# microsoft/maro

Hardware: AMD Instinct MI355X
Metric: env-steps/sec (decision events/sec), CIM global_trade.22p (higher is better)
Workload: dtype int32+f64

## Files before the change

maro_amd/cim/engine.py:

```python
from __future__ import annotations

import contextlib
import ctypes
import os
from typing import Optional, Sequence, Union

import numpy as np
import torch

from .. import _lib
from .topology import CimTopology, load_topology

PORT_ATTRS = ["capacity", "empty", "full", "on_shipper", "on_consignee", "shortage", "acc_shortage", "booking",
              "acc_booking", "fulfillment", "acc_fulfillment", "transfer_cost"]
VESSEL_ATTRS = ["capacity", "empty", "full", "remaining_space", "early_discharge", "is_parking", "loc_port_idx",
                "route_idx", "last_loc_idx", "next_loc_idx", "past_stop_list", "past_stop_tick_list",
                "future_stop_list", "future_stop_tick_list"]
MATRIX_ATTRS = ["full_on_ports", "full_on_vessels", "vessel_plans"]
NODE_ATTRS = {"ports": PORT_ATTRS, "vessels": VESSEL_ATTRS, "matrices": MATRIX_ATTRS}
NODE_TYPE = {"ports": 0, "vessels": 1, "matrices": 2}

SEED_KEEP = -1
SEED_REDRAW = -2


class CimBatchEngine:

    def __init__(self, topology: Union[str, CimTopology], n_envs: int, start_tick: int = 0, durations: int = 100,
                 snapshot_resolution: int = 1, max_snapshots: Optional[int] = None, max_actions: int = 1,
                 device: Union[str, torch.device] = "cuda:0", seeds: Optional[Sequence[int]] = None, order_table: int = 0,
                 decision_mode: int = 0, specialize: Union[bool, str, None] = None, step_mode: int = 0):
        if specialize is None:
            specialize = {"1": True, "cached": "cached"}.get(os.environ.get("MARO_AMD_SPECIALIZE", "0"), False)
        self._L = _lib.load()
        if not torch.cuda.is_available():
            raise RuntimeError("maro_amd needs a ROCm GPU (torch.cuda.is_available() is False); there is no CPU path")
        self.topo = topology if isinstance(topology, CimTopology) else load_topology(topology)
        self.device = torch.device(device)
        dev_index = self.device.index if self.device.index is not None else torch.cuda.current_device()
        self.n_envs, self.max_actions = int(n_envs), int(max_actions)
        self.start_tick, self.durations = int(start_tick), int(durations)
        self.max_tick = self.start_tick + self.durations
        self.snapshot_resolution = int(snapshot_resolution)
        self._cs = self.topo.c_struct()
        self._cfg = _lib.MrxCimConfig(self.n_envs, dev_index, self.start_tick, self.durations,
                                      self.snapshot_resolution, int(max_snapshots or 0), self.max_actions, 0, int(decision_mode),
                                      int(order_table))
        self.decision_mode = int(decision_mode)
        nbytes = self._L.mrx_cim_workspace_bytes(ctypes.byref(self._cs), ctypes.byref(self._cfg))
        _lib.check(nbytes, "mrx_cim_workspace_bytes")
        self.workspace = torch.empty(nbytes, dtype=torch.uint8, device=self.device)
        h = ctypes.c_void_p()
        with torch.cuda.device(self.device):
            torch.cuda.synchronize()
            _lib.check(self._L.mrx_cim_create(ctypes.byref(self._cs), ctypes.byref(self._cfg),
                                              self.workspace.data_ptr(), nbytes, ctypes.byref(h)), "mrx_cim_create")
        self._h = h
        self._bound_stream, self._bound_handle = None, None
        self.specialized = False
        self._specialize, self._obs_ids = specialize, ((), ())
        self._step_mode = int(step_mode)
        self._load_specialized()
        self.layout = _lib.MrxCimLayout()
        _lib.check(self._L.mrx_cim_get_layout(self._h, ctypes.byref(self.layout)), "mrx_cim_get_layout")
        lay = self.layout
        self.live = self._view(lay.off_live, torch.int32, (self.n_envs, lay.frame_words))
        self.ring = self._view(lay.off_ring, torch.int32, (self.n_envs, lay.ring_slots, lay.frame_words))
        self.ring_fi = self._view(lay.off_ring_fi, torch.int32, (self.n_envs, lay.ring_slots))
        self.status = self._view(lay.off_status, torch.int32, (self.n_envs,))
        self.ticks = self._view(lay.off_tick, torch.int32, (self.n_envs,))
        self.seeds = self._view(lay.off_seed, torch.int64, (self.n_envs,))
        dshape = (self.n_envs, 8) if self.decision_mode == 0 else (self.n_envs, lay.n_vessels, 8)
        self.decisions = torch.zeros(dshape, dtype=torch.int32, device=self.device)
        self.metrics = torch.zeros((self.n_envs, 3), dtype=torch.int64, device=self.device)
        self.done = torch.zeros((self.n_envs,), dtype=torch.uint8, device=self.device)
        if seeds is not None:
            self.reset(seeds)

    def __del__(self):
        h = getattr(self, "_h", None)
        if h:
            self._L.mrx_cim_destroy(h)
            self._h = None

    def _view(self, off: int, dtype: torch.dtype, shape) -> torch.Tensor:
        n = int(np.prod(shape)) * torch.empty((), dtype=dtype).element_size()
        return self.workspace[off:off + n].view(dtype).view(*shape)

    def _load_specialized(self) -> None:
        self.specialized = False
        if self._specialize:
            from . import specialize as spec
            try:
                spec.load_into(self, spec.plan_defines(self._cs, self._cfg, obs=self._obs_ids), build=self._specialize != "cached")
                self.specialized = True
            except KeyError:
                pass
        self.set_step_mode(self._step_mode)

    def set_step_mode(self, mode: int) -> int:
        self._step_mode = int(mode)
        self.step_mode = _lib.check(self._L.mrx_cim_set_step_mode(self._h, self._step_mode), "mrx_cim_set_step_mode")
        return self.step_mode

    def use_stream(self, stream: Optional[torch.cuda.Stream]) -> None:
        self._bound_stream = stream
        self._bound_handle = None if stream is None else stream.cuda_stream

    def _stream(self) -> int:
        h = self._bound_handle
        return torch.cuda.current_stream(self.device).cuda_stream if h is None else h

    def _dev(self, x, dtype) -> Optional[torch.Tensor]:
        if x is None:
            return None
        if isinstance(x, torch.Tensor) and x.dtype == dtype and x.device == self.device and x.is_contiguous():
            return x
        if not isinstance(x, torch.Tensor):
            x = torch.as_tensor(np.asarray(x), dtype=dtype)
        if self._bound_stream is None:
            return x.to(device=self.device, dtype=dtype).contiguous()
        if x.is_cuda:
            self._bound_stream.wait_stream(torch.cuda.current_stream(self.device))
        with torch.cuda.stream(self._bound_stream):
            return x.to(device=self.device, dtype=dtype).contiguous()

    @staticmethod
    def _p(t: Optional[torch.Tensor]):
        return None if t is None else t.data_ptr()

    def reset(self, seed_cmd=None, mask=None) -> None:
        sc = self._dev(seed_cmd, torch.int64)
        mk = self._dev(mask, torch.uint8)
        _lib.check(self._L.mrx_cim_reset(self._h, self._p(sc), self._p(mk), self._stream()), "mrx_cim_reset")
        self._keep = (sc, mk)

    def step(self, actions=None, n_actions=None, mask=None, n_answered=None):
        a = self._dev(actions, torch.int32)
        na = self._dev(n_actions, torch.int32)
        mk = self._dev(mask, torch.uint8)
        if a is not None:
            assert a.numel() == self.n_envs * self.max_actions * 4, "actions must be [n_envs, max_actions, 4]"
            if na is None:
                na = torch.full((self.n_envs,), self.max_actions, dtype=torch.int32, device=self.device)
        if self.decision_mode == 0:
            _lib.check(self._L.mrx_cim_step(self._h, self._p(a), self._p(na), self._p(mk), self.decisions.data_ptr(),
                                            self.metrics.data_ptr(), self.done.data_ptr(), self._stream()), "mrx_cim_step")
            self._keep = (a, na, mk)
        else:
            nans = self._dev(n_answered, torch.int32)
            _lib.check(self._L.mrx_cim_step_joint(self._h, self._p(a), self._p(na), self._p(nans), self._p(mk), self.decisions.data_ptr(),
                                                  self.metrics.data_ptr(), self.done.data_ptr(), self._stream()), "mrx_cim_step_joint")
            self._keep = (a, na, mk, nans)
        return self.decisions, self.metrics, self.done

    def clear_status_bits(self, envs, bits: int) -> None:
        st = self._bound_stream
        with (torch.cuda.stream(st) if st is not None else contextlib.nullcontext()):
            idx = torch.as_tensor(list(envs), dtype=torch.int64, device=self.status.device)
            self.status[idx] = self.status[idx] & ~int(bits)

    def random_policy(self, step: int, actions: torch.Tensor, n_actions: torch.Tensor,
                      counter: Optional[torch.Tensor] = None) -> None:
        _lib.check(self._L.mrx_cim_random_policy(self._h, self.decisions.data_ptr(), int(step), actions.data_ptr(),
                                                 n_actions.data_ptr(), self._p(counter), self._stream()),
                   "mrx_cim_random_policy")
# ... 75 lines not shown
```

maro_amd/csrc/cim_device.h:

```cpp
#pragma once
#include <math.h>
#include <stdint.h>

#include "cim_params.h"

#ifdef MRX_SPECIALIZED
#define KD(f) (MRXC_##f)
#define OD(f) (MRXC_obs_##f)
#define ODA(f, i) (MRXC_obs_##f(i))
#else
#define KD(f) (K.f)
#define OD(f) (O.f)
#define ODA(f, i) (O.f[i])
#endif

namespace cim {

#ifndef MRX_PROFILE_PHASES
struct Prof {
  MRX_DEV void mark(int) {}
  MRX_DEV void mark(int, long long) {}
  MRX_DEV void flush() {}
};
#endif
// ... 15 lines not shown
  uint32_t* mt_ord;
  uint32_t* mt_buf;
  double* dsrc;
  double* dtgt;
  int32_t* oq;
  int32_t* srcn;
  int32_t* misc;
};

MRX_DEV Lds make_lds(const CimParams& K, int32_t* b) {
  Lds L;
  L.frame = b + KD(l_frame);
  L.priv = b + KD(l_priv);
  L.rfull = b + KD(l_rfull);
  L.mt_ord = (uint32_t*)(b + KD(l_mt0));
  L.mt_buf = (uint32_t*)(b + KD(l_mt1));
  L.dsrc = (double*)(b + KD(l_dsrc));
  L.dtgt = (double*)(b + KD(l_dtgt));
  L.oq = b + KD(l_oq);
  L.srcn = b + KD(l_srcn);
  L.misc = b + KD(l_misc);
  L.tab.tgt_off = K.h_tgt_off; L.tab.route_port = K.h_route_port;
  L.tab.v_route_base = K.h_v_route_base; L.tab.v_route_len = K.h_v_route_len;
  L.tab.leg_off = K.h_leg_off; L.tab.leg_time = K.h_leg_time;
  L.tab.er_delay = K.er_delay; L.tab.fr_delay = K.fr_delay; L.tab.rec_off = K.h_rec_off;
  L.tab.v_cbase = K.h_v_cbase; L.tab.route_cidx = K.h_route_cidx; L.tab.pair_src = K.h_pair_src;
  L.tab.src_base = K.src_base; L.tab.src_noise = K.src_noise; L.tab.er_base = K.er_base; L.tab.er_noise = K.er_noise;
  L.tab.fr_base = K.fr_base; L.tab.fr_noise = K.fr_noise;
  return L;
}

#if defined(MRX_SPECIALIZED)
#if MRXC_lean_ok
#define MRX_LEAN 1
#endif
#endif
#if defined(MRX_LEAN) && !defined(MRX_NO_LEAN2)
#define MRX_LEAN2 1
#endif
#ifdef MRX_LEAN
enum { RR_NB = (MRXC_NT + 63) / 64, RR_H = MRXC_H };
struct RingRegs { int rf[RR_H][RR_NB]; };
#else
struct RingRegs {};
#endif

#ifdef MRX_LEAN2
struct LeanStat {
  int ps[RR_NB];
  int vs0, vs1, vs2;
  int pt;
};
struct VRows {
  int evt, next;
  int w;
};
MRX_DEV int vr_k(const VRows& W) { return W.w & 0xffff; }
MRX_DEV int vr_pos(const VRows& W) { return (W.w >> 16) & 63; }
MRX_DEV int vr_krl(const VRows& W) { return (W.w >> 22) & 63; }
MRX_DEV int vr_park(const VRows& W) { return (W.w >> 28) & 1; }
MRX_DEV void vr_set(VRows& W, int k_, int pos_, int krl_, int park_) { W.w = k_ | (pos_ << 16) | (krl_ << 22) | (park_ << 28); }
struct Lean { LeanStat s; VRows w; };
#else
struct Lean {};
#endif

#define FP(a, p) L.frame[KD(f_ports) + (a) * KD(P) + (p)]
#define FV(a, v) L.frame[KD(f_vessels) + (a) * KD(V) + (v)]
#define FOPK(k) L.frame[KD(f_fop) + (k)]
#define FOVC(v, c) L.frame[KD(f_fov) + T.v_cbase[v] + (c)]
#define PLANC(v, c) L.frame[KD(f_plans) + T.v_cbase[v] + (c)]
#define V_EVT(v) L.priv[KD(pv_evt) + (v)]
#define V_NEXT(v) L.priv[KD(pv_next) + (v)]
#define V_POS(v) L.priv[KD(pv_pos) + (v)]
#define V_KRL(v) L.priv[KD(pv_krl) + (v)]
#define V_PERIOD(v) L.priv[KD(pv_period) + (v)]
#define U(x) wave::uniform(x)
#define MRX_UNALIGNED_FRAMES (KD(resolution) > 1 && KD(start_tick) % KD(resolution) != 0)
#define RING_FULL(slot, k) L.rfull[(slot) * KD(NT) + (k)]
#define RING_EMPTY(slot, p) L.priv[KD(pv_rempty) + (slot) * KD(P) + (p)]

MRX_DEV float bits_f(int32_t x) { union { int32_t i; float f; } u; u.i = x; return u.f; }
MRX_DEV int32_t f_bits(float f) { union { int32_t i; float f; } u; u.f = f; return u.i; }

MRX_DEV void copy_in_async(int32_t* lds_dst, const int32_t* gsrc, int n_words);
MRX_DEV void stage_tables(const CimParams& K, Lds& L, int32_t* c) {
  copy_in_async(c, K.ctab, KD(ctab_words));
#define MRX_HTAB(f) L.tab.f = (const uint16_t*)c + (K.h_##f - (const uint16_t*)K.ctab)
  MRX_HTAB(tgt_off); MRX_HTAB(route_port); MRX_HTAB(v_route_base); MRX_HTAB(v_route_len);
  MRX_HTAB(leg_off); MRX_HTAB(leg_time); MRX_HTAB(rec_off); MRX_HTAB(v_cbase); MRX_HTAB(route_cidx); MRX_HTAB(pair_src);
#undef MRX_HTAB
  L.tab.er_delay = c + (K.er_delay - K.ctab); L.tab.fr_delay = c + (K.fr_delay - K.ctab);
#define MRX_DTAB(f) L.tab.f = (const double*)(c + ((const int32_t*)K.f - K.ctab))
  if (!KD(pregen)) { MRX_DTAB(src_base); MRX_DTAB(src_noise); }
  MRX_DTAB(er_base); MRX_DTAB(er_noise); MRX_DTAB(fr_base); MRX_DTAB(fr_noise);
#undef MRX_DTAB
}

MRX_DEV uint32_t mt_temper(uint32_t y) {
  y ^= (y >> 11);
  y ^= (y << 7) & 0x9d2c5680U;
  y ^= (y << 15) & 0xefc60000U;
  y ^= (y >> 18);
  return y;
}

MRX_DEV void mt_twist(uint32_t* mt) {
  const int l = wave::lane();
  static_assert(MT_WORDS == 3 * 208, "round size");
  for (int k0 = 0; k0 < MT_WORDS; k0 += 208) {
    uint32_t x[4];
#pragma unroll
    for (int j = 0; j < 4; j++) {
      const bool on = j * 64 + l < 208;
      const int k = on ? k0 + j * 64 + l : k0;
      const int k1 = (k + 1 == MT_WORDS) ? 0 : k + 1;
      const int km = (k + 397 >= MT_WORDS) ? k + 397 - MT_WORDS : k + 397;
      const uint32_t y = (mt[k] & 0x80000000U) | (mt[k1] & 0x7fffffffU);
      x[j] = mt[km] ^ (y >> 1) ^ ((y & 1U) ? 0x9908b0dfU : 0U);
    }
    wave::sync();
#pragma unroll
    for (int j = 0; j < 4; j++)
      if (j * 64 + l < 208) mt[k0 + j * 64 + l] = x[j];
    wave::sync();
  }
}

MRX_DEV double mt_draw_batch(uint32_t* mt, int& idx, int rank, int n, bool& twisted) {
  uint32_t a = 0, b = 0;
  const bool has = rank >= 0;
  const int w0 = idx + 2 * rank, w1 = w0 + 1;
  if (has && w0 < MT_WORDS) a = mt_temper(mt[w0]);
  if (has && w1 < MT_WORDS) b = mt_temper(mt[w1]);
  if (idx + 2 * n > MT_WORDS) {
    wave::sync();
    mt_twist(mt);
    twisted = true;
    if (has && w0 >= MT_WORDS) a = mt_temper(mt[w0 - MT_WORDS]);
    if (has && w1 >= MT_WORDS) b = mt_temper(mt[w1 - MT_WORDS]);
    idx = idx + 2 * n - MT_WORDS;
  } else {
    idx += 2 * n;
  }
  return ((double)(a >> 5) * 67108864.0 + (double)(b >> 6)) * (1.0 / 9007199254740992.0);
}

template <int NB>
MRX_DEV void mt_draw_multi(uint32_t* mt, int& idx, const int (&rank)[NB], int n, bool& twisted, double (&r)[NB]) {
  uint32_t a[NB], b[NB];
#pragma unroll
  for (int i = 0; i < NB; i++) {
    const int w0 = idx + 2 * rank[i], w1 = w0 + 1;
    const uint32_t ra = mt[(rank[i] >= 0 && w0 < MT_WORDS) ? w0 : 0], rb = mt[(rank[i] >= 0 && w1 < MT_WORDS) ? w1 : 0];
    a[i] = (rank[i] >= 0 && w0 < MT_WORDS) ? mt_temper(ra) : 0u;
    b[i] = (rank[i] >= 0 && w1 < MT_WORDS) ? mt_temper(rb) : 0u;
  }
  if (idx + 2 * n > MT_WORDS) {
    wave::sync();
    mt_twist(mt);
    twisted = true;
#pragma unroll
    for (int i = 0; i < NB; i++) {
      const int w0 = idx + 2 * rank[i], w1 = w0 + 1;
      const uint32_t ra = mt[(rank[i] >= 0 && w0 >= MT_WORDS) ? w0 - MT_WORDS : 0], rb = mt[(rank[i] >= 0 && w1 >= MT_WORDS) ? w1 - MT_WORDS : 0];
      if (rank[i] >= 0 && w0 >= MT_WORDS) a[i] = mt_temper(ra);
// ... 279 lines not shown
      long long cur = 0;                                                                          \
      if (n_p > 0) {                                                                              \
        const double ts = L.dsrc[sp], x = L.dtgt[k];                                              \
        cur = (long long)ceil((double)n_p * ((ts == 0.0) ? x : x / ts));                          \
        if (cur > 0x7fffffffll) cur = 0x7fffffffll;                                               \
        if (cur < -0x7fffffffll) cur = -0x7fffffffll;                                             \
      }                                                                                           \
      L.oq[k] = (int32_t)cur;                                                                     \
    }                                                                                             \
  }
  if (NTb > 0) MRX_PAIR_BATCH(0, pf.src[0])
  if (NTb > 64) MRX_PAIR_BATCH(64, pf.src[1])
  if (NTb > 128) MRX_PAIR_BATCH(128, pf.src[2])
  for (int k0 = 192; k0 < NTb; k0 += 64) MRX_PAIR_BATCH(k0, K.pair_src[k0 + lane < NT ? k0 + lane : 0])
#undef MRX_PAIR_BATCH
  wave::sync();
  uint64_t negq = 0;
  for (int k0 = 0; k0 < NTb; k0 += 64) negq |= wave::ballot(k0 + lane < NTb && L.oq[k0 + lane] < 0);
  if (!negq) {
    uint32_t* pre = (uint32_t*)L.dtgt;
    uint32_t carry = 0;
#define MRX_HAND_SCAN(k0, SRC)                                                 \
    {                                                                          \
      const int k = (k0) + lane;                                               \
      int v = 0;                                                               \
      if (k < NTb) {                                                           \
        const int n_p = L.srcn[(SRC)];                                         \
        const int q = L.oq[k];                                                 \
        v = q < n_p ? q : (n_p > 0 ? n_p : 0);  \
      }                                                                        \
      const uint32_t incl = (uint32_t)wave::scan_incl_add(v) + carry;          \
      carry = (uint32_t)wave::bcast((int)incl, 63);                            \
      if (k < NTb) pre[k] = incl;                                              \
    }
    if (NTb > 0) MRX_HAND_SCAN(0, pf.src[0])
    if (NTb > 64) MRX_HAND_SCAN(64, pf.src[1])
    if (NTb > 128) MRX_HAND_SCAN(128, pf.src[2])
    for (int k0 = 192; k0 < NTb; k0 += 64) MRX_HAND_SCAN(k0, K.pair_src[k0 + lane < NT ? k0 + lane : 0])
#undef MRX_HAND_SCAN
    wave::sync();
#define MRX_HAND_OUT(k0, SRC)                                                                   \
    {                                                                                           \
      const int k = (k0) + lane;                                                                \
      if (k < NTb) {                                                                            \
        const int sp = (SRC);                                                                   \
        const int n_p = L.srcn[sp], q = L.oq[k], off = T.tgt_off[sp];                           \
        const int v = q < n_p ? q : (n_p > 0 ? n_p : 0);                                        \
        const int before = (int)(pre[k] - (uint32_t)v - (off > 0 ? pre[off - 1] : 0u));         \
        const int rem = n_p - before;                                                           \
        const int cur = rem <= 0 ? 0 : (q < rem ? q : rem);                                     \
        L.oq[k] = cur > 0 ? cur : 0;                                                            \
      }                                                                                         \
    }
    if (NTb > 0) MRX_HAND_OUT(0, pf.src[0])
    if (NTb > 64) MRX_HAND_OUT(64, pf.src[1])
    if (NTb > 128) MRX_HAND_OUT(128, pf.src[2])
    for (int k0 = 192; k0 < NTb; k0 += 64) MRX_HAND_OUT(k0, K.pair_src[k0 + lane < NT ? k0 + lane : 0])
#undef MRX_HAND_OUT
  } else if (lane < brk) {
    const long long n_p = L.srcn[lane];
    if (n_p > 0) {
      const int off = T.tgt_off[lane], cnt = T.tgt_off[lane + 1] - off;
      long long rem = n_p;
      for (int j = 0; j < cnt; j++) {
        long long cur = L.oq[off + j];
        if (cur > rem) cur = rem;
        rem -= cur;
        L.oq[off + j] = cur > 0 ? (int32_t)cur : 0;
      }
    }
  }
}

MRX_DEV void reset_env(const CimParams& K, int env, int32_t* lds, long long cmd) {
  Lds L = make_lds(K, lds);
  uint32_t* mt_route = (uint32_t*)(lds + KD(l_mt2));
  uint32_t* mt_oinit = (uint32_t*)(lds + KD(l_mt3));
  L.mt_ord = (uint32_t*)(lds + KD(r_mt0));
  L.mt_buf = (uint32_t*)(lds + KD(r_mt1));
  const int lane = wave::lane();
  const int P = KD(P), V = KD(V), TT = KD(T);
  uint32_t* g_mt = K.mt + (size_t)env * MTS_COUNT * MT_WORDS;
  int32_t* g_priv = K.priv + (size_t)env * KD(PW);
  int32_t* g_live = K.live + (size_t)env * KD(FW);
  const Tabs& T = L.tab;

  long long base;
  if (KD(data_mode)) {
    base = K.data_seed;
  } else if (cmd >= 0) {
    base = cmd;
  } else if (cmd == -1) {
    base = K.seed[env];
  } else {
    int idx = g_priv[PH_IDX_ROUTE];
    copy_words((int32_t*)mt_route, (const int32_t*)(g_mt + MTS_ROUTE * MT_WORDS), MT_WORDS);
    wave::sync();
    uint32_t r = mt_next_u32(mt_route, idx) >> (32 - 13);
    while (r >= 4096u) r = mt_next_u32(mt_route, idx) >> (32 - 13);
    base = (long long)r;
    wave::sync();
  }

  {
    uint32_t* arr = lane == 0 ? L.mt_ord : lane == 1 ? L.mt_buf : lane == 2 ? mt_route : mt_oinit;
    const int sidx = lane == 0 ? KD(idx_order_num) : lane == 1 ? KD(idx_buffer) : lane == 2 ? KD(idx_route) : KD(idx_order_init);
    if (lane < 3 || (lane == 3 && KD(has_order_init))) mt_seed_serial(arr, base + sidx);
  }
  wave::sync();
  int idx_route = MT_WORDS, idx_oi = MT_WORDS;

  int32_t* g_prop = K.order_prop + (size_t)env * TT;
  int status = 0;
  uint32_t* g_stops = K.stops + (size_t)env * V * KD(SMAX);
  if (KD(data_mode)) {
    for (int t = lane; t < TT; t += 64) g_prop[t] = (KD(data_mode) == 1 && t < KD(data_T)) ? K.fx_order_prop[t] : 0;
    for (int i = lane; i < V * KD(SMAX); i += 64) g_stops[i] = K.fx_stops[i];
    if (lane < V) { K.nstops[(size_t)env * V + lane] = K.fx_nstops[lane]; K.vperiod[(size_t)env * V + lane] = K.fx_vperiod[lane]; }
    __atomic_thread_fence(__ATOMIC_SEQ_CST);
    wave::sync();
  } else {
  for (int t0 = 0; t0 < TT; t0 += 64) {
    const int t = t0 + lane;
    double orders = t < TT ? K.order_dist[t % KD(period)] : 0.0;
    const bool nz = t < TT && orders != 0.0;
    if (KD(has_order_init)) {
      const uint64_t m = wave::ballot(nz);
      const int rank = nz ? __builtin_popcountll(m & ((1ull << lane) - 1ull)) : -1;
      bool tw = false;
      const double r = mt_draw_batch(mt_oinit, idx_oi, rank, __builtin_popcountll(m), tw);
      if (nz) orders = apply_noise(orders, K.sample_noise, r);
    }
    if (t < TT) {
      int32_t val = 0;
      if (nz) {
        double c = orders < 1.0 ? orders : 1.0;
        if (c < 0.0) c = 0.0;
        val = (int32_t)floor(c * (double)KD(total_containers));
      }
      g_prop[t] = val;
    }
  }

  for (int v = 0; v < V; v++) {
    const int Lr = K.v_route_len[v], rb = K.v_route_base[v], start = K.v_start[v];
    const double speed = K.v_speed[v], sn = K.v_speed_noise[v], dur = K.v_dur[v], dn = K.v_dur_noise[v];
    union { double d; int w[2]; } my_dist;
    my_dist.d = lane < Lr ? K.route_dist[rb + lane] : 0.0;
    const int my_leg = lane < Lr ? K.leg_time[K.leg_off[v] + lane] : 0;
    int tick = 0, extra = 0, k = 0;
    bool have_park = false, done = false;
    int park_carry = 0;
    while (!done) {
      const int left = (MT_WORDS - idx_route) / 2;
      const int nd = (idx_route >= MT_WORDS - 1 || left > 126) ? 126 : left;
      const int c = have_park ? 1 : 0;
      const int pi = 2 * lane - c, si = pi + 1;
      const int rank[2] = {(pi >= 0 && pi < nd) ? pi : -1, si < nd ? si : -1};
      double r[2];
      bool tw = false;
      mt_draw_multi<2>(mt_route, idx_route, rank, nd, tw, r);
      const int n_full = (nd + c) / 2;
      const bool half = ((nd + c) & 1) != 0;
      int parking = (int)ceil(apply_noise(dur, dn, r[0]));
      if (c && lane == 0) parking = park_carry;
      const double noised_speed = apply_noise(speed, sn, r[1]);
      int loc = start + k + lane;
// ... 12 lines not shown
      if (k + n_run >= 4 * KD(SMAX) + 1) {
        n_run = 4 * KD(SMAX) + 1 - k;
        run = run && lane < n_run;
        status |= 2;
        done = true;
      }
      if (wave::ballot(run && (parking <= 0 || parking > 255))) status |= 8;
      if (wave::ballot(run && k + lane >= KD(SMAX))) status |= 2;
      if (run && k + lane < KD(SMAX)) g_stops[(size_t)v * KD(SMAX) + k + lane] = ((uint32_t)t_before << 8) | (uint32_t)(parking & 0xff);
      if (extra + __builtin_popcountll(over & ((1ull << n_run) - 1ull)) > KD(future_n)) done = true;
      if (done) {
        idx_route -= 2 * (nd - (2 * n_run - c));
      } else {
        have_park = half;
        park_carry = wave::bcast(parking, n_full < 64 ? n_full : 0);
        tick += wave::bcast(incl, 63);
        extra += __builtin_popcountll(over);
      }
      k += n_run;
    }
    const int n_per = k < Lr ? k : Lr;
    int ploc = start + lane;
    ploc = ploc % Lr;
    const int leg_l = wave::shfl(my_leg, ploc);
    const int period = wave::bcast(wave::scan_incl_add(lane < n_per ? leg_l : 0), 63);
    if (lane == 0) { K.nstops[(size_t)env * V + v] = k < KD(SMAX) ? k : KD(SMAX); K.vperiod[(size_t)env * V + v] = period; }
  }
  __atomic_thread_fence(__ATOMIC_SEQ_CST);
  }
  wave::sync();

  copy_words((int32_t*)(g_mt + MTS_ORDER * MT_WORDS), (const int32_t*)L.mt_ord, MT_WORDS);
  copy_words((int32_t*)(g_mt + MTS_BUFFER * MT_WORDS), (const int32_t*)L.mt_buf, MT_WORDS);
  copy_words((int32_t*)(g_mt + MTS_ROUTE * MT_WORDS), (const int32_t*)mt_route, MT_WORDS);
  wave::sync();

  for (int i = lane; i < KD(FW); i += 64) L.frame[i] = (i >= KD(f_plans) && i < KD(f_plans) + KD(NC)) ? -1 : 0;
  for (int i = lane; i < KD(PWH); i += 64) L.priv[i] = 0;
  wave::sync();
  if (lane < P) {
    FP(PA_CAPACITY, lane) = K.p_cap[lane];
    FP(PA_EMPTY, lane) = K.p_init_empty[lane];
  }
  if (lane < V) {
    const int v = lane;
    FV(VA_CAPACITY, v) = K.v_cap[v];
    FV(VA_ROUTE_IDX, v) = K.v_route[v];
    FV(VA_EMPTY, v) = K.v_init_empty[v];
    FV(VA_REMAINING_SPACE, v) = K.v_total_space[v] - K.v_init_empty[v];
    FV(VA_IS_PARKING, v) = 1;
    FV(VA_LOC_PORT_IDX, v) = K.route_port[K.v_route_base[v] + K.v_start[v]];
    write_plans(K, L, v, K.v_start[v], 0);
    V_EVT(v) = stop_parking(g_stops[(size_t)v * KD(SMAX)]);
    V_POS(v) = K.v_start[v];
    V_KRL(v) = 0;
    V_PERIOD(v) = K.vperiod[(size_t)env * V + v];
    V_NEXT(v) = K.nstops[(size_t)env * V + v] > 1 ? stop_arrival(g_stops[(size_t)v * KD(SMAX) + 1]) : 0x7fffffff;
  }
  bool zombie = false;
  if (KD(start_tick) > 0 && lane < V) {
    const int v = lane, ns = K.nstops[(size_t)env * V + v];
    int ks = 0;
    while (ks < ns && stop_arrival(g_stops[(size_t)v * KD(SMAX) + ks]) + stop_parking(g_stops[(size_t)v * KD(SMAX) + ks]) < KD(start_tick)) ks++;
    if (ks > 0) {
      zombie = true;
      const uint32_t st = g_stops[(size_t)v * KD(SMAX) + (ks < ns ? ks : 0)];
      V_EVT(v) = ks < ns ? stop_arrival(st) + stop_parking(st) : 0x7fffffff;
      V_NEXT(v) = ks;
    }
  }
  const uint64_t zm = wave::ballot(zombie);
  if (lane == 0) {
    L.priv[PH_TICK] = KD(start_tick);
    L.priv[PH_FLAGS] = FL_FRESH;
    L.priv[PH_IDX_ORDER] = MT_WORDS;
    L.priv[PH_IDX_BUFFER] = MT_WORDS;
    L.priv[PH_IDX_ROUTE] = idx_route;
    L.priv[PH_ZOMBIE_LO] = (int32_t)(uint32_t)(zm & 0xffffffffull);
    L.priv[PH_ZOMBIE_HI] = (int32_t)(uint32_t)(zm >> 32);
    K.seed[env] = base;
    K.status[env] = status;
    K.tick[env] = KD(start_tick);
    K.hint[env] = 1;
  }
  wave::sync();
  copy_words(g_live, L.frame, KD(FW));
  copy_words(g_priv, L.priv, KD(PWH));
  for (int i = KD(PWH) + lane; i < KD(PW); i += 64) g_priv[i] = 0;
  for (int i = lane; i < KD(S); i += 64) K.ring_fi[(size_t)env * KD(S) + i] = -1;
  int32_t* g_rec0 = K.rec + (size_t)env * KD(REC_W);
  for (int i = lane; i < KD(REC_W); i += 64) g_rec0[i] = 0;
}

MRX_DEV double of_recip(double d) {
#if defined(__HIP_DEVICE_COMPILE__)
  double y = __builtin_amdgcn_rcp(d);
  y = fma(y, fma(-d, y, 1.0), y);
  y = fma(y, fma(-d, y, 1.0), y);
  return y;
#else
  return d;
#endif
}
MRX_DEV double of_div(double n, double d, double y) {
#if defined(__HIP_DEVICE_COMPILE__)
  const double q0 = n * y;
  return fma(fma(-d, q0, n), y, q0);
#else
  (void)y;
  return n / d;
#endif
}

MRX_DEV void of_next_block(uint32_t* win, int cur, int nxt) {
  const int l = wave::lane();
#define MRX_OF_ROUND(K0, N)                                                                                  \
  _Pragma("unroll") for (int j = 0; j < ((N) + 63) / 64; j++) {                                              \
    const int k = (K0) + j * 64 + l;                                                                         \
    const bool on = (j + 1) * 64 <= (N) || l < (N) - j * 64;         \
    const int kc = on ? k : (K0);                                                                            \
    const uint32_t a = win[cur + kc], b = win[kc + 1 == MT_WORDS ? nxt : cur + kc + 1];                      \
    const uint32_t m = win[kc < 227 ? cur + kc + 397 : nxt + kc - 227];                                      \
    const uint32_t y = (a & 0x80000000U) | (b & 0x7fffffffU);                                                \
    x[j] = m ^ (y >> 1) ^ ((uint32_t)(-(int32_t)(y & 1U)) & 0x9908b0dfU);                                    \
  }                                                                                                          \
  wave::sync();                                                                                              \
  _Pragma("unroll") for (int j = 0; j < ((N) + 63) / 64; j++)                                                \
    if ((j + 1) * 64 <= (N) || l < (N) - j * 64) win[nxt + (K0) + j * 64 + l] = x[j];                        \
  wave::sync();
  uint32_t x[3];
  MRX_OF_ROUND(0, 192)
  MRX_OF_ROUND(192, 192)
  MRX_OF_ROUND(384, 192)
  MRX_OF_ROUND(576, 48)
#undef MRX_OF_ROUND
}

MRX_DEV void gen_order_table_fast(const CimParams& K, int env, int32_t* lds) {
  const int lane = wave::lane();
  const int P = KD(P), NT = KD(NT), ND = P + NT;
  uint32_t* win = (uint32_t*)(lds + KD(gf_win));
  double* val = (double*)(lds + KD(gf_val));
  int32_t* rec = lds + KD(gf_rec);
  int32_t* pre1 = lds + KD(gf_pre);
  uint16_t* row16 = (uint16_t*)(lds + KD(gf_row));
  int32_t* seg = lds + KD(gf_seg);
  const int ZERO = KD(gf_slots), TRASH = KD(gf_slots) + 4;
  copy_in_async((int32_t*)win, (const int32_t*)(K.mt + ((size_t)env * MTS_COUNT + MTS_ORDER) * MT_WORDS), MT_WORDS);

  const int cnt_p = lane < P ? K.tgt_off[lane + 1] - K.tgt_off[lane] : 0;
  const int pad_p = (cnt_p + 3) & ~3;
  const int Ppad = (P + 3) & ~3;
  const int incl_p = wave::scan_incl_add(pad_p);
  const int sum_seg = lane < P ? Ppad + incl_p - pad_p : 0;
  const int sum_len = lane < P ? pad_p : lane == P ? Ppad : 0;
  const int toff_l = K.tgt_off[lane <= P ? lane : P];
  int max_len = 4;
  for (int len = 8; len <= 64; len += 4)
    if (wave::ballot(sum_len >= len)) max_len = len;
  if (lane < P) seg[lane] = sum_seg;
  for (int i = lane; i < KD(gf_slots) + 6; i += 64) val[i] = 0.0;
  for (int i = lane; i < KD(NTP) / 2; i += 64) ((uint32_t*)row16)[i] = 0u;
  if (lane == 0) {
    pre1[0] = 0;
    double* r = (double*)(rec + P * 8);
    r[0] = 1.0; r[1] = 1.0;
// ... 820 lines not shown
      tick_prefetch_arrivals(K, env, L, arr_mask, pf);
      tick_prefetch_land(pf);
    }
    const int lvv = lane < V ? lane : 0;
    const int r_k = FV(VA_NEXT_LOC_IDX, lvv), r_pos = V_POS(lvv), r_krl = V_KRL(lvv), r_cap = FV(VA_CAPACITY, lvv),
              r_full = FV(VA_FULL, lvv), r_empty = FV(VA_EMPTY, lvv), r_len = T.v_route_len[lvv], r_rb = T.v_route_base[lvv];
    for (uint64_t m = arr_mask; m; m &= m - 1, a_idx++) {
      if (a_idx == 4) {
        tick_prefetch_arrivals(K, env, L, m, pf);
        tick_prefetch_land(pf);
        a_idx = 0;
      }
      const int v = __builtin_ctzll(m);
      const int k = wave::readlane(r_k, v), pos = wave::readlane(r_pos, v), krl = wave::readlane(r_krl, v),
                cap = wave::readlane(r_cap, v);
      int full = wave::readlane(r_full, v), empty = wave::readlane(r_empty, v);
      const int full0 = full, empty0 = empty;
      const int Lr = wave::readlane(r_len, v), rb = wave::readlane(r_rb, v), RL = Lr + 1;
      const int p = T.route_port[rb + pos];
      const int ns = wave::bcast(pf.ns, a_idx);
      const uint32_t st_k = (uint32_t)wave::bcast((int)pf.stk, a_idx);
      const uint32_t st_k1 = (uint32_t)wave::bcast((int)pf.stk1, a_idx);
      prof.mark(10);
      const bool act = lane < Lr;
      int xi = pos + lane, xn = pos + 1 + lane;
      xi = act ? (xi >= Lr ? xi - Lr : xi) : 0;
      xn = act ? (xn >= Lr ? xn - Lr : xn) : 0;
      const int leg = act ? T.leg_time[T.leg_off[v] + xi] : 0;
      const int tick_i = t + wave::scan_incl_add(leg);
      const int port_i = T.route_port[rb + xn], c_i = T.route_cidx[rb + xn];
      bool dup_later = false, dup_earlier = false;
      const int n_distinct = (v + 1 < V ? (int)T.v_cbase[v + 1] : KD(NC)) - (int)T.v_cbase[v];
      if (n_distinct != Lr) {
        for (int j = 0; j < Lr; j++) {
          const int cj = wave::bcast(c_i, j);
          dup_later = dup_later || (j > lane && cj == c_i);
          dup_earlier = dup_earlier || (j < lane && cj == c_i);
        }
      }
      if (lane < Lr && !dup_later) PLANC(v, c_i) = tick_i;
      prof.mark(11);
      const int acceptable = (int)floor((double)(cap - full * KD(vol)) / (double)KD(vol));
      const bool lv = lane < Lr && (k + 1 + lane) < ns && !dup_earlier;
      const int kk = a_idx == 0 ? pf.kk[0] : a_idx == 1 ? pf.kk[1] : a_idx == 2 ? pf.kk[2] : pf.kk[3];
      const int pend = (lv && kk >= 0) ? FOPK(kk) : 0;
      const int incl = wave::scan_incl_add(pend);
      int l = 0;
      if (acceptable > 0 && pend > 0) { const int room = acceptable - (incl - pend); l = room <= 0 ? 0 : (pend < room ? pend : room); }
      const int loaded_total = wave::bcast(incl < acceptable ? incl : (acceptable > 0 ? acceptable : 0), 63);
      if (l > 0) {
        FOPK(kk) = pend - l;
        FOVC(v, c_i) += l;
        int row = krl + 1 + lane;
        if (row >= RL) row -= RL;
        g_rec[T.rec_off[v] + row * RL + krl] = l;
      }
      full += loaded_total;
      int early = 0;
      if ((long long)(full + empty) * KD(vol) > (long long)cap) {
        early = (full + empty) - (int)ceil((double)cap / (double)KD(vol));
        empty -= early;
      }
      wave::sync();
      if (lane == 0) {
        FV(VA_LAST_LOC_IDX, v) = k;
        FV(VA_IS_PARKING, v) = 1;
        FV(VA_LOC_PORT_IDX, v) = p;
        FP(PA_FULL, p) -= loaded_total;
        FP(PA_EMPTY, p) += early;
        FV(VA_FULL, v) = full;
        FV(VA_EMPTY, v) = empty;
        FV(VA_EARLY_DISCHARGE, v) = early;
        FV(VA_REMAINING_SPACE, v) += (full0 + empty0) - (full + empty);
        V_EVT(v) = t + stop_parking(st_k);
        V_NEXT(v) = k + 1 < ns ? stop_arrival(st_k1) : 0x7fffffff;
      }
      wave::sync();
    }
  }
  prof.mark(PF_ARRIVALS);
  return arr_mask;
}

MRX_DEV void take_snapshot(const CimParams& K, const CimObs& O, int env, Lds& L, int fi) {
  const int s = fi % KD(S);
  copy_words(K.ring + ((size_t)env * KD(S) + s) * KD(FW), L.frame, KD(FW));
  if (wave::lane() == 0) K.ring_fi[(size_t)env * KD(S) + s] = fi;
  if (O.hist_n > 0 && fi < O.hist_frames) {
    int32_t* row = O.hist + ((size_t)env * O.hist_frames + fi) * O.hist_n * KD(P);
    for (int a = 0; a < O.hist_n; a++)
      if (wave::lane() < KD(P)) row[a * KD(P) + wave::lane()] = FP(O.hist_attr[a], wave::lane());
  }
}

MRX_DEV unsigned long long mix64(unsigned long long seed, unsigned long long step) {
  unsigned long long x = seed * 0x9E3779B97F4A7C15ull + step * 0xBF58476D1CE4E5B9ull + 0x94D049BB133111EBull;
  x ^= x >> 30; x *= 0xBF58476D1CE4E5B9ull;
  x ^= x >> 27; x *= 0x94D049BB133111EBull;
  x ^= x >> 31;
  return x;
}
MRX_DEV void agent_answer(const CimParams& K, const CimObs& O, int env, long long seed, int t, int port, int vessel, int load, int dis) {
  const unsigned long long key = O.agent_key >= 0 ? (unsigned long long)O.agent_key : (((unsigned long long)(unsigned)t << 8) | (unsigned)vessel) + 0x100000000ull;
  const unsigned long long x = mix64((unsigned long long)seed, key), r = x >> 1;
  int32_t* a = O.agent_actions + (size_t)env * KD(max_actions) * 4;
  a[0] = vessel; a[1] = port;
  if ((x & 1ull) == 0 && load > 0) { a[2] = (int)(r % (unsigned long long)(load + 1)); a[3] = 0; }
  else { a[2] = (int)(r % (unsigned long long)(dis + 1)); a[3] = 1; }
  O.agent_n_actions[env] = 1;
  if (O.agent_count) wave::global_add_nr(&O.agent_count[env], 1);
}
MRX_DEV void agent_none(const CimObs& O, int env) { O.agent_n_actions[env] = 0; }

struct FastRows {
  int hdr;
  int pe, tc;
  int ve, rs, ed, lp, per;
  int pl[4];
  int vo[8];
};

template <bool OBS>
MRX_DEV void fast_rows_request(const CimParams& K, const CimObs& O, int env, FastRows& R) {
  const int lane = wave::lane();
  const int32_t* g_live = K.live + (size_t)env * KD(FW);
  const int32_t* g_priv = K.priv + (size_t)env * KD(PW);
  const int p = lane < KD(P) ? lane : 0, v = lane < KD(V) ? lane : 0;
  R.hdr = lane < PH_COUNT ? g_priv[lane] : 0;
  R.pe = g_live[KD(f_ports) + PA_EMPTY * KD(P) + p];
  R.tc = g_live[KD(f_ports) + PA_TRANSFER_COST * KD(P) + p];
  R.ve = g_live[KD(f_vessels) + VA_EMPTY * KD(V) + v];
  R.rs = g_live[KD(f_vessels) + VA_REMAINING_SPACE * KD(V) + v];
  R.ed = g_live[KD(f_vessels) + VA_EARLY_DISCHARGE * KD(V) + v];
  R.lp = g_live[KD(f_vessels) + VA_LOC_PORT_IDX * KD(V) + v];
  R.per = g_priv[KD(pv_period) + v];
  for (int k = 0; k < 4; k++) R.pl[k] = (KD(NC) <= 256 && lane + 64 * k < KD(NC)) ? g_live[KD(f_plans) + lane + 64 * k] : 0;
  if constexpr (OBS) {
#pragma unroll
    for (int a = 0; a < 8; a++) R.vo[a] = a < OD(nv) ? g_live[KD(f_vessels) + ODA(va, a) * KD(V) + v] : 0;
  }
}

MRX_DEV double port_attr_value(int attr, int raw) { return attr == PA_TRANSFER_COST ? (double)bits_f(raw) : (double)raw; }

template <bool OBS>
MRX_DEV bool fast_step(const CimParams& K, const CimObs& O, int env, const FastRows& R, int n_act, int a0v, int a0p, int a0q, int a0t,
                       int32_t* dec_out, long long* met_out, uint8_t* done_out) {
  const int lane = wave::lane();
  const int P = KD(P), V = KD(V);
  const int hdr = R.hdr;
  const int flags = wave::bcast(hdr, PH_FLAGS);
  if (flags & FL_FINISHED) {
    if (lane < 8) dec_out[lane] = lane == 7 ? -1 : 0;
    if (lane < 3) met_out[lane] = 0;
    if (lane == 0) { *done_out = 1; if (O.agent_mode) agent_none(O, env); }
    return true;
  }
  if ((flags & FL_FRESH) || MRX_UNALIGNED_FRAMES) return false;
  const long long agent_seed = O.agent_mode ? K.seed[env] : 0;
  const uint64_t pend = ((uint64_t)(uint32_t)wave::bcast(hdr, PH_PEND_HI) << 32) | (uint32_t)wave::bcast(hdr, PH_PEND_LO);
  const int cur = wave::bcast(hdr, PH_CUR_VESSEL);
  const uint64_t pend_after = pend & ~(1ull << (cur & 63));
  if (!pend_after || n_act > 1) return false;
  int32_t* g_live = K.live + (size_t)env * KD(FW);
  int32_t* g_priv = K.priv + (size_t)env * KD(PW);
  const int t = wave::bcast(hdr, PH_TICK);
  long long opnum = ((long long)wave::bcast(hdr, PH_OPNUM_HI) << 32) | (uint32_t)wave::bcast(hdr, PH_OPNUM_LO);
  const long long acc_b = ((long long)wave::bcast(hdr, PH_ACCB_HI) << 32) | (uint32_t)wave::bcast(hdr, PH_ACCB_LO);
  const long long acc_s = ((long long)wave::bcast(hdr, PH_ACCS_HI) << 32) | (uint32_t)wave::bcast(hdr, PH_ACCS_LO);
  int status = 0;
  const int v2 = __builtin_ctzll(pend_after);
#define GP(a, p) g_live[KD(f_ports) + (a) * P + (p)]
#define GV(a, v) g_live[KD(f_vessels) + (a) * V + (v)]
  bool act = n_act == 1;
  const int av = a0v, ap = a0p, q = a0q, ty = a0t;
  if (act && (av < 0 || av >= V || ap < 0 || ap >= P || q < 0 || (ty != 0 && ty != 1))) { status |= 1; act = false; }
  const int sv = act ? av : 0, sp = act ? ap : 0;
  const int c = act ? K.cidx_dense[sv * P + sp] : -1;
  const int pe = wave::bcast(R.pe, sp), tc = wave::bcast(R.tc, sp);
  const int ve = wave::bcast(R.ve, sv), rs = wave::bcast(R.rs, sv);
  const int period = wave::bcast(R.per, sv);
  const int lp2 = wave::bcast(R.lp, v2);
  int ve2 = wave::bcast(R.ve, v2), rs2 = wave::bcast(R.rs, v2);
  const int ed2 = wave::bcast(R.ed, v2);
  int pe2 = wave::bcast(R.pe, lp2);
  int pl;
  {
    const int cc = c >= 0 ? c : 0;
    const int p0 = wave::bcast(R.pl[0], cc & 63), p1 = wave::bcast(R.pl[1], cc & 63), p2 = wave::bcast(R.pl[2], cc & 63),
              p3 = wave::bcast(R.pl[3], cc & 63);
    pl = cc < 64 ? p0 : cc < 128 ? p1 : cc < 192 ? p2 : p3;
    if (KD(NC) > 256) pl = g_live[KD(f_plans) + cc];
  }
  bool applied = false;
  int o_pe = 0, o_tc = 0, o_ve = 0, o_rs = 0;
  if (act) {
    int npe = pe, nve = ve;
    bool ok = true;
    if (ty == 1) { if (q > ve) ok = false; else { npe = pe + q; nve = ve - q; } }
    else { if (q > (pe < rs ? pe : rs)) ok = false; else { npe = pe - q; nve = ve + q; } }
    if (!ok) status |= 1;
    else {
      const int nrs = rs - (nve - ve);
      applied = true; o_pe = npe; o_tc = f_bits((float)((double)bits_f(tc) + (double)q)); o_ve = nve; o_rs = nrs;
      if (lane == 0) {
        GP(PA_EMPTY, ap) = npe;
        GP(PA_TRANSFER_COST, ap) = f_bits((float)((double)bits_f(tc) + (double)q));
        GV(VA_EMPTY, av) = nve;
        GV(VA_REMAINING_SPACE, av) = nrs;
        if (c >= 0) g_live[KD(f_plans) + c] = pl + period;
      }
      if (c < 0) status |= 32;
      opnum += q;
      if (ap == lp2) pe2 = npe;
      if (av == v2) { ve2 = nve; rs2 = nrs; }
    }
  }
#undef GP
#undef GV
  if constexpr (OBS) {
    if (applied && lane == 0) {
      if (OD(i_empty) >= 0) O.ports[((size_t)env * P + ap) * OD(np) + OD(i_empty)] = (double)o_pe;
      if (OD(i_tc) >= 0) O.ports[((size_t)env * P + ap) * OD(np) + OD(i_tc)] = (double)bits_f(o_tc);
    }
#pragma unroll
    for (int a = 0; a < 8; a++) {
      if (a < OD(nv)) {
        int raw = wave::bcast(R.vo[a], v2);
        if (applied && av == v2) { if (ODA(va, a) == VA_EMPTY) raw = o_ve; else if (ODA(va, a) == VA_REMAINING_SPACE) raw = o_rs; }
        if (lane == 0) O.vessel[(size_t)env * OD(nv) + a] = (double)raw;
      }
    }
  }
  if (lane == 0) {
    dec_out[0] = t; dec_out[1] = lp2; dec_out[2] = v2;
    dec_out[3] = pe2 < rs2 ? pe2 : rs2;
    dec_out[4] = ve2; dec_out[5] = ed2;
    dec_out[6] = (t - KD(start_tick)) / KD(resolution); dec_out[7] = 1;
    if (O.agent_mode) agent_answer(K, O, env, agent_seed, t, lp2, v2, pe2 < rs2 ? pe2 : rs2, ve2);
    met_out[0] = acc_b; met_out[1] = acc_s; met_out[2] = opnum;
    *done_out = 0;
    g_priv[PH_PEND_LO] = (int32_t)(uint32_t)(pend_after & 0xffffffffull);
    g_priv[PH_PEND_HI] = (int32_t)(uint32_t)(pend_after >> 32);
    g_priv[PH_CUR_VESSEL] = v2;
    g_priv[PH_OPNUM_LO] = (int32_t)(uint32_t)((unsigned long long)opnum & 0xffffffffull);
    g_priv[PH_OPNUM_HI] = (int32_t)(opnum >> 32);
    K.hint[env] = (pend_after & ~(1ull << v2)) ? 0 : ((flags & FL_LONG) ? 2 : 1);
    if (status) wave::global_or(&K.status[env], status);
  }
  return true;
}

template <bool OBS>
MRX_DEV bool fast_step_lane(const CimParams& K, const CimObs& O, int env, const int32_t* act, int n_act, int32_t* dec_out,
                            long long* met_out, uint8_t* done_out) {
  const int P = KD(P), V = KD(V);
  int32_t* g_live = K.live + (size_t)env * KD(FW);
  int32_t* g_priv = K.priv + (size_t)env * KD(PW);
  const wave::v4i h0 = wave::ld16(g_priv), h1 = wave::ld16(g_priv + 4), h3 = wave::ld16(g_priv + 12);
  wave::v4i a4 = {0, 0, 0, 0};
  if (act) a4 = wave::ld16(act);
  const int flags = h0.y;
  if (flags & FL_FINISHED) {
    for (int j = 0; j < 8; j++) dec_out[j] = j == 7 ? -1 : 0;
    for (int j = 0; j < 3; j++) met_out[j] = 0;
    *done_out = 1;
    if (O.agent_mode) agent_none(O, env);
    return true;
  }
  if ((flags & FL_FRESH) || MRX_UNALIGNED_FRAMES) return false;
  const long long agent_seed = O.agent_mode ? K.seed[env] : 0;
  const uint64_t pend = ((uint64_t)(uint32_t)h0.w << 32) | (uint32_t)h0.z;
  const int cur = h1.x;
  const uint64_t pend_after = pend & ~(1ull << (cur & 63));
  if (!pend_after || n_act > 1) return false;
  const int t = h0.x;
  long long opnum = ((long long)h1.z << 32) | (uint32_t)h1.y;
  const long long acc_b = ((long long)h3.y << 32) | (uint32_t)h3.x, acc_s = ((long long)h3.w << 32) | (uint32_t)h3.z;
  int status = 0;
  const int v2 = __builtin_ctzll(pend_after);
#define GP(a, p) g_live[KD(f_ports) + (a) * P + (p)]
#define GV(a, v) g_live[KD(f_vessels) + (a) * V + (v)]
  bool do_act = n_act == 1;
  const int av = a4.x, ap = a4.y, q = a4.z, ty = a4.w;
  if (do_act && (av < 0 || av >= V || ap < 0 || ap >= P || q < 0 || (ty != 0 && ty != 1))) { status |= 1; do_act = false; }
  const int sv = do_act ? av : 0, sp = do_act ? ap : 0;
  const int c = do_act ? K.cidx_dense[sv * P + sp] : -1;
  const int pe = GP(PA_EMPTY, sp), tc = GP(PA_TRANSFER_COST, sp);
  const int ve = GV(VA_EMPTY, sv), rs = GV(VA_REMAINING_SPACE, sv);
  const int period = g_priv[KD(pv_period) + sv];
  const int lp2 = GV(VA_LOC_PORT_IDX, v2), ed2 = GV(VA_EARLY_DISCHARGE, v2);
  int ve2 = GV(VA_EMPTY, v2), rs2 = GV(VA_REMAINING_SPACE, v2);
  int vo[8];
  if constexpr (OBS) {
#pragma unroll
    for (int a = 0; a < 8; a++) vo[a] = a < OD(nv) ? GV(ODA(va, a), v2) : 0;
  }
  int pe2 = GP(PA_EMPTY, lp2 >= 0 ? lp2 : 0);
  const int pl = c >= 0 ? g_live[KD(f_plans) + c] : 0;
  bool applied = false;
  int o_pe = 0, o_tc = 0, o_ve = 0, o_rs = 0;
  if (do_act) {
    int npe = pe, nve = ve;
    bool ok = true;
    if (ty == 1) { if (q > ve) ok = false; else { npe = pe + q; nve = ve - q; } }
    else { if (q > (pe < rs ? pe : rs)) ok = false; else { npe = pe - q; nve = ve + q; } }
    if (!ok) status |= 1;
    else {
      const int nrs = rs - (nve - ve);
      applied = true; o_pe = npe; o_tc = f_bits((float)((double)bits_f(tc) + (double)q)); o_ve = nve; o_rs = nrs;
      GP(PA_EMPTY, ap) = npe;
      GP(PA_TRANSFER_COST, ap) = o_tc;
      GV(VA_EMPTY, av) = nve;
      GV(VA_REMAINING_SPACE, av) = nrs;
      if (c >= 0) g_live[KD(f_plans) + c] = pl + period;
      else status |= 32;
      opnum += q;
      if (ap == lp2) pe2 = npe;
      if (av == v2) { ve2 = nve; rs2 = nrs; }
    }
  }
#undef GP
#undef GV
  if constexpr (OBS) {
    if (applied) {
      if (OD(i_empty) >= 0) O.ports[((size_t)env * P + ap) * OD(np) + OD(i_empty)] = (double)o_pe;
      if (OD(i_tc) >= 0) O.ports[((size_t)env * P + ap) * OD(np) + OD(i_tc)] = (double)bits_f(o_tc);
    }
#pragma unroll
    for (int a = 0; a < 8; a++) {
      if (a < OD(nv)) {
        int raw = vo[a];
        if (applied && av == v2) { if (ODA(va, a) == VA_EMPTY) raw = o_ve; else if (ODA(va, a) == VA_REMAINING_SPACE) raw = o_rs; }
        O.vessel[(size_t)env * OD(nv) + a] = (double)raw;
      }
    }
  }
  dec_out[0] = t; dec_out[1] = lp2; dec_out[2] = v2;
  dec_out[3] = pe2 < rs2 ? pe2 : rs2;
  dec_out[4] = ve2; dec_out[5] = ed2;
  dec_out[6] = (t - KD(start_tick)) / KD(resolution); dec_out[7] = 1;
  if (O.agent_mode) agent_answer(K, O, env, agent_seed, t, lp2, v2, pe2 < rs2 ? pe2 : rs2, ve2);
  met_out[0] = acc_b; met_out[1] = acc_s; met_out[2] = opnum;
  *done_out = 0;
  g_priv[PH_PEND_LO] = (int32_t)(uint32_t)(pend_after & 0xffffffffull);
  g_priv[PH_PEND_HI] = (int32_t)(uint32_t)(pend_after >> 32);
  g_priv[PH_CUR_VESSEL] = v2;
  g_priv[PH_OPNUM_LO] = (int32_t)(uint32_t)((unsigned long long)opnum & 0xffffffffull);
  g_priv[PH_OPNUM_HI] = (int32_t)(opnum >> 32);
  K.hint[env] = (pend_after & ~(1ull << v2)) ? 0 : ((flags & FL_LONG) ? 2 : 1);
  if (status) wave::global_or(&K.status[env], status);
  return true;
}

MRX_DEV uint64_t consume_decisions(const CimParams& K, uint64_t pend, int cur, int n_answered) {
  if (KD(decision_mode) == 0) return pend & ~(1ull << (cur & 63));
  if (KD(decision_mode) == 1 || n_answered < 0) return 0ull;
  for (int k = 0; k < n_answered && pend; k++) pend &= pend - 1;
  return pend;
}

struct StepIO {
  const int32_t* actions;
  int n_act, n_answered;
  int32_t* dec_out;
  long long* met_out;
  uint8_t* done_out;
};
struct StepBatch {
  const int32_t *actions, *n_actions, *n_answered;
  int32_t* decisions;
  long long* metrics;
  uint8_t* done;
};
MRX_DEV StepIO step_io(const CimParams& K, const StepBatch& B, int env, bool counts = true) {
  StepIO io;
  io.actions = B.actions ? B.actions + (size_t)env * KD(max_actions) * 4 : nullptr;
  io.n_act = (counts && B.actions && B.n_actions) ? B.n_actions[env] : 0;
  io.n_answered = (counts && B.n_answered) ? B.n_answered[env] : -1;
  io.dec_out = B.decisions + (size_t)env * (KD(decision_mode) ? (size_t)KD(V) * 8 : 8);
  io.met_out = B.metrics + (size_t)env * 3;
  io.done_out = B.done + env;
  return io;
}
struct StepEnd { bool store, ord_dirty, buf_dirty; };

template <bool PG>
MRX_DEV void state_load_async(const CimParams& K, Lds& L, int env) {
  const uint32_t* g_mt = K.mt + (size_t)env * MTS_COUNT * MT_WORDS;
  copy_in_async(L.frame, K.live + (size_t)env * KD(FW), KD(FW));
  copy_in_async(L.priv, K.priv + (size_t)env * KD(PW), KD(PWH));
#ifndef MRX_LEAN
  copy_in_async(L.rfull, K.priv + (size_t)env * KD(PW) + KD(pv_rfull), KD(PW) - KD(pv_rfull));
#endif
  if (!PG && KD(use_order_rng)) copy_in_async((int32_t*)L.mt_ord, (const int32_t*)(g_mt + MTS_ORDER * MT_WORDS), MT_WORDS);
  if (KD(use_buffer_rng)) copy_in_async((int32_t*)L.mt_buf, (const int32_t*)(g_mt + MTS_BUFFER * MT_WORDS), MT_WORDS);
}
template <bool PG>
MRX_DEV void state_store(const CimParams& K, Lds& L, int env, const StepEnd& e) {
  uint32_t* g_mt = K.mt + (size_t)env * MTS_COUNT * MT_WORDS;
  copy_words(K.live + (size_t)env * KD(FW), L.frame, KD(FW));
  copy_words(K.priv + (size_t)env * KD(PW), L.priv, KD(PWH));
#ifndef MRX_LEAN
  copy_words(K.priv + (size_t)env * KD(PW) + KD(pv_rfull), L.rfull, KD(PW) - KD(pv_rfull));
#endif
  if (!PG && KD(use_order_rng) && e.ord_dirty) copy_words((int32_t*)(g_mt + MTS_ORDER * MT_WORDS), (const int32_t*)L.mt_ord, MT_WORDS);
  if (KD(use_buffer_rng) && e.buf_dirty) copy_words((int32_t*)(g_mt + MTS_BUFFER * MT_WORDS), (const int32_t*)L.mt_buf, MT_WORDS);
}

MRX_DEV void ring_load(const CimParams& K, int env, RingRegs& rr) {
#ifdef MRX_LEAN
  const int lane = wave::lane();
  const int32_t* g = K.priv + (size_t)env * KD(PW) + KD(pv_rfull);
#pragma unroll
  for (int h = 0; h < RR_H; h++)
#pragma unroll
    for (int b = 0; b < RR_NB; b++) {
      const int k = b * 64 + lane;
      const int x = g[h * KD(NT) + (k < KD(NT) ? k : 0)];
      rr.rf[h][b] = k < KD(NT) ? x : 0;
    }
#endif
}
MRX_DEV void ring_store(const CimParams& K, int env, const RingRegs& rr) {
#ifdef MRX_LEAN
  const int lane = wave::lane();
  int32_t* g = K.priv + (size_t)env * KD(PW) + KD(pv_rfull);
#pragma unroll
  for (int h = 0; h < RR_H; h++)
#pragma unroll
    for (int b = 0; b < RR_NB; b++) {
      const int k = b * 64 + lane;
      if (k < KD(NT)) g[h * KD(NT) + k] = rr.rf[h][b];
    }
#endif
}

struct StepCtx {
  int t;
  bool fresh;
  uint64_t pend;
  int idx_ord, idx_buf;
  long long opnum;
  int status;
  int a0v, a0p, a0q, a0t, n_act, n_answered;
  TickPf pf;
};
struct StepOut {
  int kind;
  int dec[8];
  long long met[3];
  int done, hint, tick, status;
  bool obs_on;
  double obs[8];
  double vobs[8];
};

MRX_DEV int plan_cell(const Lds& L, int v, int p) {
  const Tabs& T = L.tab;
  const int lane = wave::lane();
  const int Lr = T.v_route_len[v], rb = T.v_route_base[v];
  const bool hit = lane < Lr && (int)T.route_port[rb + (lane < Lr ? lane : 0)] == p;
  const uint64_t m = wave::ballot(hit);
  if (!m) return -1;
  return (int)T.v_cbase[v] + (int)T.route_cidx[rb + __builtin_ctzll(m)];
}

template <bool PG>
MRX_DEV bool body_open(const CimParams& K, int env, Lds& L, StepCtx& c, StepOut& out, Lean& Z) {
#ifdef MRX_LEAN2
  vrows_load(K, L, Z.w);
#endif
  const int flags0 = U(L.priv[PH_FLAGS]);
  out.kind = 0;
  out.obs_on = false;
  c.pf = TickPf{};
  if (flags0 & FL_FINISHED) {
    out.kind = 2;
    return false;
  }
  if (c.n_act > KD(max_actions)) c.n_act = KD(max_actions);
  c.t = L.priv[PH_TICK];
  c.fresh = (flags0 & FL_FRESH) != 0;
  c.pend = ((uint64_t)(uint32_t)L.priv[PH_PEND_HI] << 32) | (uint32_t)L.priv[PH_PEND_LO];
  c.idx_ord = L.priv[PH_IDX_ORDER];
  c.idx_buf = L.priv[PH_IDX_BUFFER];
  c.opnum = ((long long)L.priv[PH_OPNUM_HI] << 32) | (uint32_t)L.priv[PH_OPNUM_LO];
  c.status = 0;
  const uint64_t pend_after = c.fresh ? 0ull : consume_decisions(K, c.pend, L.priv[PH_CUR_VESSEL], c.n_answered);
  const int tn = c.fresh ? c.t : c.t + 1;
  if (!pend_after && tn < KD(T)) {
#ifdef MRX_LEAN2
    tick_prefetch_lean(K, env, L, tn, c.pf, Z);
#else
    if constexpr (!PG) tick_prefetch_static(K, c.pf, true);
    tick_prefetch<PG>(K, env, L, tn, c.pf);
#endif
  }
  return true;
}

MRX_DEV void body_act(const CimParams& K, Lds& L, const int32_t* actions, StepCtx& c, const Lean& Z) {
  const int P = KD(P), V = KD(V);
  if (c.fresh) return;
  for (int i = 0; i < c.n_act; i++) {
    const int32_t* a = actions + 4 * i;
    const int v = U(i == 0 ? c.a0v : a[0]), p = U(i == 0 ? c.a0p : a[1]), q = U(i == 0 ? c.a0q : a[2]), ty = U(i == 0 ? c.a0t : a[3]);
    if (v < 0 || v >= V || p < 0 || p >= P || q < 0 || (ty != 0 && ty != 1)) { c.status |= 1; continue; }
#ifdef MRX_LEAN2
    const Tabs& T = L.tab;
    const int a_vs0 = wave::readlane(Z.s.vs0, v), a_Lr = a_vs0 & 63, a_rb = (int)((unsigned)a_vs0 >> 12), a_cb = wave::readlane(Z.s.vs2, v);
    const int a_lr = wave::lane() < a_Lr ? wave::lane() : 0;
    const int a_rp = T.route_port[a_rb + a_lr], a_rc = T.route_cidx[a_rb + a_lr], a_per = V_PERIOD(v);
#endif
    const int pe_v = FP(PA_EMPTY, p), ve_v = FV(VA_EMPTY, v), rs_v = FV(VA_REMAINING_SPACE, v), tc_v = FP(PA_TRANSFER_COST, p);
    const int pe = U(pe_v), ve = U(ve_v), rs = U(rs_v), tc = U(tc_v);
    int npe, nve;
    if (ty == 1) {
      if (q > ve) { c.status |= 1; continue; }
      npe = pe + q; nve = ve - q;
    } else {
      if (q > (pe < rs ? pe : rs)) { c.status |= 1; continue; }
      npe = pe - q; nve = ve + q;
    }
    FP(PA_EMPTY, p) = npe;
    FV(VA_EMPTY, v) = nve;
    FV(VA_REMAINING_SPACE, v) = rs - (nve - ve);
    c.opnum += q;
    FP(PA_TRANSFER_COST, p) = f_bits((float)((double)bits_f(tc) + (double)q));
    {
#ifdef MRX_LEAN2
      const uint64_t hit = wave::ballot(wave::lane() < a_Lr && a_rp == p);
      const int cc = hit ? a_cb + wave::readlane(a_rc, __builtin_ctzll(hit)) : -1;
      if (cc >= 0) { const int pl = U(L.frame[KD(f_plans) + cc]); L.frame[KD(f_plans) + cc] = pl + U(a_per); }
#else
      const int cc = plan_cell(L, v, p);
      if (cc >= 0) { const int pl = U(L.frame[KD(f_plans) + cc]); L.frame[KD(f_plans) + cc] = pl + U(V_PERIOD(v)); }
#endif
      else c.status |= 32;
    }
  }
  c.pend = consume_decisions(K, c.pend, L.priv[PH_CUR_VESSEL], c.n_answered);
  wave::sync();
}

template <bool PG, bool OBS>
MRX_DEV StepEnd body_run(const CimParams& K, const CimObs& O, int env, Lds& L, const StepIO& io, StepCtx& c, StepOut& out, Prof& prof, RingRegs& rr, Lean& Z) {
  const int lane = wave::lane();
  const int P = KD(P), V = KD(V);
  StepEnd end = {true, false, false};
  int t = c.t;
  bool fresh = c.fresh, finished = false;
  uint64_t pend = c.pend;
  int dec_v = -1;
  for (;;) {
    if (pend) {
      dec_v = __builtin_ctzll(pend);
      break;
    }
    if (!fresh) {
      if ((t + 1) % KD(resolution) == 0) {
        if (lane < P) FP(PA_ACC_FULFILLMENT, lane) = FP(PA_ACC_BOOKING, lane) - FP(PA_ACC_SHORTAGE, lane);
        wave::sync();
        take_snapshot(K, O, env, L, (t - KD(start_tick)) / KD(resolution));
        wave::sync();
        if (lane < P) { FP(PA_SHORTAGE, lane) = 0; FP(PA_BOOKING, lane) = 0; FP(PA_FULFILLMENT, lane) = 0; FP(PA_TRANSFER_COST, lane) = 0; }
        wave::sync();
      }
      if (t + 1 == KD(T)) {
        if ((t + 1) % KD(resolution) != 0) take_snapshot(K, O, env, L, (t - KD(start_tick)) / KD(resolution));
        finished = true;
        break;
      }
      t += 1;
    }
    prof.mark(PF_POST_STEP);
    fresh = false;
#ifdef MRX_LEAN2
    pend = run_tick_lean(K, env, L, t, c.pf, c.idx_buf, c.status, prof, end.buf_dirty, rr, Z);
#else
    pend = run_tick<PG>(K, env, L, t, c.pf, c.idx_ord, c.idx_buf, c.status, prof, end.ord_dirty, end.buf_dirty, rr);
#endif
    if (!pend && t + 1 < KD(T)) {
#ifdef MRX_LEAN2
      tick_prefetch_lean(K, env, L, t + 1, c.pf, Z);
#else
      tick_prefetch<PG>(K, env, L, t + 1, c.pf);
#endif
      tick_prefetch_land(c.pf);
    }
  }

  if (MRX_UNALIGNED_FRAMES && !finished) {
    const int fi0 = (t - KD(start_tick)) / KD(resolution), lo = KD(start_tick) + fi0 * KD(resolution);
    if (t > lo + (KD(resolution) - 1 - lo % KD(resolution))) {
      wave::sync();
      take_snapshot(K, O, env, L, fi0);
      wave::sync();
    }
  }
  long long acc_b = 0, acc_s = 0;
  if (lane < P) { acc_b = FP(PA_ACC_BOOKING, lane); acc_s = FP(PA_ACC_SHORTAGE, lane); }
  acc_b = wave::reduce_add(acc_b);
  acc_s = wave::reduce_add(acc_s);
  const int fi = (t - KD(start_tick)) / KD(resolution);
  out.kind = 1;
  if (KD(decision_mode) != 0) {
    int32_t* dec_out = io.dec_out;
    const uint64_t pm = finished ? 0ull : pend;
    const bool mine = lane < V && ((pm >> lane) & 1ull);
    if (mine) {
      const int r = __builtin_popcountll(pm & ((1ull << lane) - 1ull));
      const int v = lane, p = FV(VA_LOC_PORT_IDX, v);
      const int pe = FP(PA_EMPTY, p), rs = FV(VA_REMAINING_SPACE, v);
      int32_t* d = dec_out + 8 * r;
      d[0] = t; d[1] = p; d[2] = v; d[3] = pe < rs ? pe : rs; d[4] = FV(VA_EMPTY, v); d[5] = FV(VA_EARLY_DISCHARGE, v);
      d[6] = fi; d[7] = 1;
    }
    const int cnt = __builtin_popcountll(pm);
    if (lane < V && lane >= cnt) {
      int32_t* d = dec_out + 8 * lane;
      for (int j = 0; j < 8; j++) d[j] = 0;
      if (lane == 0) { d[0] = t; d[6] = fi; }
    }
  } else if (!finished) {
    {
      const int v = dec_v, p = FV(VA_LOC_PORT_IDX, v);
      const int pe = FP(PA_EMPTY, p), rs = FV(VA_REMAINING_SPACE, v);
      out.dec[0] = t; out.dec[1] = p; out.dec[2] = v;
      out.dec[3] = pe < rs ? pe : rs;
      out.dec[4] = FV(VA_EMPTY, v);
      out.dec[5] = FV(VA_EARLY_DISCHARGE, v);
      out.dec[6] = fi; out.dec[7] = 1;
    }
    if constexpr (OBS) {
      out.obs_on = true;
      const int tot = P * OD(np), npd = OD(np) > 0 ? OD(np) : 1;
#pragma unroll
      for (int j = 0; j < 8; j++) {
        const int i = lane + 64 * j;
        out.obs[j] = 0.0;
        if (i < tot) {
          const int p = i / npd, a = i - p * npd;
          const int attr = (int)((OD(pa_packed) >> (4 * a)) & 15u);
          out.obs[j] = port_attr_value(attr, FP(attr, p));
        }
      }
#pragma unroll
      for (int a = 0; a < 8; a++) out.vobs[a] = a < OD(nv) ? (double)FV(ODA(va, a), dec_v) : 0.0;
    }
  } else {
    out.dec[0] = t; out.dec[1] = 0; out.dec[2] = 0; out.dec[3] = 0; out.dec[4] = 0; out.dec[5] = 0;
    out.dec[6] = fi; out.dec[7] = 0;
  }
  out.met[0] = acc_b; out.met[1] = acc_s; out.met[2] = c.opnum;
  out.done = finished ? 1 : 0;
  out.tick = t;
  out.status = c.status;
  out.hint = (KD(decision_mode) == 0 && !MRX_UNALIGNED_FRAMES && (finished || (pend & ~(1ull << (dec_v & 63))))) ? 0 : 1;
  bool long_next = false;
  if (KD(start_tick) == 0 && !finished) {
#ifdef MRX_LEAN2
    const bool soon = lane < V && (vr_park(Z.w) ? Z.w.next : Z.w.evt) <= t + 1;
#else
    const bool soon = lane < V && (FV(VA_IS_PARKING, lane) ? V_NEXT(lane) : V_EVT(lane)) <= t + 1;
#endif
    long_next = wave::ballot(soon) == 0ull;
  }
  if (long_next && out.hint) out.hint = 2;
  if (lane == 0) {
    L.priv[PH_TICK] = t;
    L.priv[PH_FLAGS] = finished ? FL_FINISHED : (long_next ? FL_LONG : 0);
    L.priv[PH_PEND_LO] = (int32_t)(uint32_t)(pend & 0xffffffffull);
    L.priv[PH_PEND_HI] = (int32_t)(uint32_t)(pend >> 32);
    L.priv[PH_CUR_VESSEL] = dec_v;
    L.priv[PH_OPNUM_LO] = (int32_t)(uint32_t)((unsigned long long)c.opnum & 0xffffffffull);
    L.priv[PH_OPNUM_HI] = (int32_t)(c.opnum >> 32);
    L.priv[PH_IDX_ORDER] = c.idx_ord;
    L.priv[PH_IDX_BUFFER] = c.idx_buf;
    L.priv[PH_ACCB_LO] = (int32_t)(uint32_t)((unsigned long long)acc_b & 0xffffffffull); L.priv[PH_ACCB_HI] = (int32_t)(acc_b >> 32);
    L.priv[PH_ACCS_LO] = (int32_t)(uint32_t)((unsigned long long)acc_s & 0xffffffffull); L.priv[PH_ACCS_HI] = (int32_t)(acc_s >> 32);
  }
  wave::sync();
  prof.mark(PF_OUTPUT);
  return end;
}

template <bool OBS>
MRX_DEV void body_emit(const CimParams& K, const CimObs& O, int env, const StepIO& io, const StepOut& out, long long agent_seed) {
  const int lane = wave::lane();
  if (out.kind == 0) return;
  if (out.kind == 2) {
    if (lane < 8) io.dec_out[lane] = lane == 7 ? -1 : 0;
    if (lane < 3) io.met_out[lane] = 0;
    if (lane == 0) { *io.done_out = 1; if (O.agent_mode) agent_none(O, env); }
    return;
  }
  if (O.agent_mode && KD(decision_mode) == 0 && lane == 0) {
    if (out.dec[7] == 1 && !out.done) agent_answer(K, O, env, agent_seed, out.dec[0], out.dec[1], out.dec[2], out.dec[3], out.dec[4]);
    else agent_none(O, env);
  }
  if (KD(decision_mode) == 0) {
    if (lane == 0) {
#pragma unroll
      for (int j = 0; j < 8; j++) io.dec_out[j] = out.dec[j];
    }
    if constexpr (OBS) {
      if (out.obs_on) {
        const int tot = KD(P) * OD(np);
        double* op = O.ports + (size_t)env * tot;
#pragma unroll
        for (int j = 0; j < 8; j++) {
          const int i = lane + 64 * j;
          if (i < tot) op[i] = out.obs[j];
        }
#pragma unroll
        for (int a = 0; a < 8; a++)
          if (a < OD(nv) && lane == 0) O.vessel[(size_t)env * OD(nv) + a] = out.vobs[a];
      }
    }
  }
  if (lane == 0) {
    io.met_out[0] = out.met[0]; io.met_out[1] = out.met[1]; io.met_out[2] = out.met[2];
    *io.done_out = (uint8_t)out.done;
    K.tick[env] = out.tick;
    K.hint[env] = (uint8_t)out.hint;
    if (out.status) wave::global_or(&K.status[env], out.status);
  }
}

template <bool PG, bool OBS>
MRX_DEV StepEnd full_body(const CimParams& K, const CimObs& O, int env, Lds& L, const StepIO& io, int a0v, int a0p, int a0q, int a0t, Prof& prof, RingRegs& rr, Lean& Z) {
  StepCtx c;
  StepOut out;
  c.a0v = a0v; c.a0p = a0p; c.a0q = a0q; c.a0t = a0t;
  c.n_act = io.n_act; c.n_answered = io.n_answered;
  StepEnd end = {false, false, false};
  const long long agent_seed = O.agent_mode ? K.seed[env] : 0;
  if (body_open<PG>(K, env, L, c, out, Z)) {
    prof.mark(PF_LOAD);
    body_act(K, L, io.actions, c, Z);
    prof.mark(PF_ACTION);
    tick_prefetch_land(c.pf);
    prof.mark(PF_MT_LOAD);
    end = body_run<PG, OBS>(K, O, env, L, io, c, out, prof, rr, Z);
  }
  body_emit<OBS>(K, O, env, io, out, agent_seed);
  return end;
}

enum { PATH_PROBE = 0,
       PATH_FAST = 1,
       PATH_FULL = 2 };

template <bool PG, bool OBS>
MRX_DEV void step_env(const CimParams& K, const CimObs& O, int env, int32_t* lds, const StepIO& io, int path, int32_t* lds_ctab = nullptr) {
  Lds L = make_lds(K, lds);
  Prof prof;
  if (KD(decision_mode) == 0 && path != PATH_FULL) {
    FastRows rows;
    fast_rows_request<OBS>(K, O, env, rows);
    int hint = 0;
    if (path == PATH_PROBE) hint = K.hint[env];
    int f0v = 0, f0p = 0, f0q = 0, f0t = 0;
    if (io.actions) { f0v = io.actions[0]; f0p = io.actions[1]; f0q = io.actions[2]; f0t = io.actions[3]; }
    if (!U(hint) && fast_step<OBS>(K, O, env, rows, io.n_act > KD(max_actions) ? KD(max_actions) : io.n_act, f0v, f0p, f0q, f0t, io.dec_out,
                                   io.met_out, io.done_out)) {
#ifdef MRX_PROFILE_FAST_PATH
      prof.mark(13); prof.mark(14, 1);
      prof.flush();
#endif
      return;
    }
    prof.mark(12);
  }
  state_load_async<PG>(K, L, env);
  stage_tables(K, L, lds_ctab ? lds_ctab : lds + KD(l_ctab));
  RingRegs rr;
  ring_load(K, env, rr);
  Lean Z;
#ifdef MRX_LEAN2
  lean_stat_load(K, Z.s);
#endif
  int a0v = 0, a0p = 0, a0q = 0, a0t = 0;
  if (io.actions) { a0v = io.actions[0]; a0p = io.actions[1]; a0q = io.actions[2]; a0t = io.actions[3]; }
  wave::lds_dma_wait();
  const StepEnd e = full_body<PG, OBS>(K, O, env, L, io, a0v, a0p, a0q, a0t, prof, rr, Z);
  if (e.store) { state_store<PG>(K, L, env, e); ring_store(K, env, rr); }
  prof.mark(PF_STORE);
  prof.flush();
}

template <bool OBS>
MRX_DEV void fast_lanes_env(const CimParams& K, const CimObs& O, const StepBatch& B, const uint8_t* mask, int env) {
  if (env >= K.n_envs || (mask && !mask[env]) || K.hint[env]) return;
  const StepIO io = step_io(K, B, env);
  const int n_act = io.n_act > KD(max_actions) ? KD(max_actions) : io.n_act;
  if (KD(decision_mode) == 0 && fast_step_lane<OBS>(K, O, env, io.actions, n_act, io.dec_out, io.met_out, io.done_out)) return;
  K.order[wave::global_add(&K.sched[0], 1)] = env | MRX_ORDER_TICK;
}

template <bool PG, bool OBS>
MRX_DEV void step_loop(const CimParams& K, const CimObs& O, int32_t* lds, int w, int W, const StepBatch& B) {
  const int n_tick = U(wave::ld_uniform_v(K.sched + 0));
  for (int i = w; i < n_tick; i += W) {
    const int env = U(wave::ld_uniform_v(K.order + i)) & (MRX_ORDER_TICK - 1);
    step_env<PG, OBS>(K, O, env, lds, step_io(K, B, env), PATH_FULL);
    wave::sync();
  }
}

MRX_DEV int attr_slots(const CimParams& K, int node_type, int a) {
  if (node_type == 0) return 1;
  if (node_type == 1) {
    if (a == VA_PAST_STOP_LIST || a == VA_PAST_STOP_TICK_LIST) return KD(past_n);
    if (a == VA_FUTURE_STOP_LIST || a == VA_FUTURE_STOP_TICK_LIST) return KD(future_n);
    return 1;
  }
  return a == MA_FULL_ON_PORTS ? KD(P) * KD(P) : KD(V) * KD(P);
}

MRX_DEV int frame_word(const CimParams& K, int node_type, int a, int node, int s) {
  if (node_type == 0) return KD(f_ports) + a * KD(P) + node;
  if (node_type == 1) return KD(f_vessels) + a * KD(V) + node;
  if (a == MA_FULL_ON_PORTS) {
    const int k = K.pair_dense[s];
    return k < 0 ? -1 : KD(f_fop) + k;
  }
  const int c = K.cidx_dense[s];
  if (c < 0) return -1;
  return (a == MA_FULL_ON_VESSELS ? KD(f_fov) : KD(f_plans)) + c;
}

MRX_DEV int stop_list_value(const CimParams& K, int env, const int32_t* frame, int a, int v, int s) {
  const int Lr = K.v_route_len[v], rb = K.v_route_base[v], start = K.v_start[v];
  const uint32_t* srow = K.stops + ((size_t)env * KD(V) + v) * KD(SMAX);
  if (a == VA_PAST_STOP_LIST || a == VA_PAST_STOP_TICK_LIST) {
    const int j = frame[KD(f_vessels) + VA_NEXT_LOC_IDX * KD(V) + v] - KD(past_n) + s;
    if (j < 0) return -1;
    if (a == VA_PAST_STOP_LIST) return K.route_port[rb + (start + j) % Lr];
    if (j == 0) {
      const int32_t* hdr = K.priv + (size_t)env * KD(PW);
      const uint64_t zm = ((uint64_t)(uint32_t)hdr[PH_ZOMBIE_HI] << 32) | (uint32_t)hdr[PH_ZOMBIE_LO];
      if (!((zm >> v) & 1ull)) return 0;
    }
    return stop_arrival(srow[j < KD(SMAX) ? j : KD(SMAX) - 1]);
  }
  const int k = frame[KD(f_vessels) + VA_LAST_LOC_IDX * KD(V) + v];
  int tick = k == 0 ? 0 : stop_arrival(srow[k < KD(SMAX) ? k : KD(SMAX) - 1]);
  int x = (start + k) % Lr;
  const int lo = K.leg_off[v];
  for (int i = 0; i <= s; i++) {
    tick += K.leg_time[lo + x];
    x = (x + 1 == Lr) ? 0 : x + 1;
  }
  return a == VA_FUTURE_STOP_LIST ? K.route_port[rb + x] : tick;
}

MRX_DEV const int32_t* frame_of(const CimParams& K, int env, int fi) {
  const int s = (fi < 0 ? 0 : fi) % KD(S);
  const int32_t* hdr = K.priv + (size_t)env * KD(PW);
  const int flags = hdr[PH_FLAGS], tick = hdr[PH_TICK], held = K.ring_fi[(size_t)env * KD(S) + s];
  const bool paused = (flags & (FL_FRESH | FL_FINISHED)) == 0;
  const int cur_fi = (tick - KD(start_tick)) / KD(resolution);
  const int32_t* frame = nullptr;
  if (held == fi) frame = K.ring + ((size_t)env * KD(S) + s) * KD(FW);
  if (paused && s == cur_fi % KD(S)) frame = fi == cur_fi ? K.live + (size_t)env * KD(FW) : nullptr;
  return fi < 0 ? nullptr : frame;
}

MRX_DEV double query_elem(const CimParams& K, int node_type, const int32_t* ticks, int nt, int ticks_per_env,
                          const int32_t* nodes, int nn, int nodes_per_env, const int32_t* attrs, int na, long long row, int col) {
  const int ni = (int)(row % nn);
  const int ti = (int)((row / nn) % nt);
  const int env = (int)(row / ((long long)nn * nt));
  const int fi = ticks[(size_t)env * ticks_per_env + ti];
  const int32_t* frame = frame_of(K, env, fi);
  if (!frame) return 0.0;
  int a = 0, slot = col;
  for (int i = 0; i < na; i++) {
    const int ns = attr_slots(K, node_type, attrs[i]);
    if (slot < ns) { a = attrs[i]; break; }
    slot -= ns;
  }
  const int node = nodes[(size_t)env * nodes_per_env + ni];
  const int n_nodes = node_type == 0 ? KD(P) : node_type == 1 ? KD(V) : 1;
  if (node < 0 || node >= n_nodes) return 0.0;
  if (node_type == 1 && a >= VA_PAST_STOP_LIST) return (double)stop_list_value(K, env, frame, a, node, slot);
  const int w = frame_word(K, node_type, a, node, slot);
  if (w < 0) return a == MA_VESSEL_PLANS ? -1.0 : 0.0;
  const int32_t raw = frame[w];
  return (node_type == 0 && a == PA_TRANSFER_COST) ? (double)bits_f(raw) : (double)raw;
}

#undef FP
#undef FV
#undef FOPK
#undef FOVC
#undef PLANC
#undef V_EVT
#undef V_NEXT
#undef V_POS
#undef V_KRL
#undef V_PERIOD
#undef U
#undef RING_FULL
#undef RING_EMPTY

}
```

maro_amd/csrc/cim_dqn.h:

```cpp
#pragma once
#include <hip/hip_runtime.h>

#include "cim_device.h"

namespace cim {

enum { DQ_MAX_LAYERS = 8, DQ_MAX_WIDTH = 256, DQ_TILE_MAX = 32, DQ_LD = DQ_MAX_WIDTH + 4, DQ_MAX_TICKS = 16, DQ_MAX_NODES = 8,
       DQ_PASS = 8 ,
       DQ_SLOTS = 2 * DQ_PASS  };

struct DqnParams {
  int n_layers, dueling, state_dim, look_back, n_nodes, n_pa, n_va, n_actions;
  int xcd_runs;
  int pa[8], va[8];
  int kpad[DQ_MAX_LAYERS], npad[DQ_MAX_LAYERS], n_out[DQ_MAX_LAYERS];
  long long s_off[4][DQ_MAX_LAYERS];
  long long b_off[DQ_MAX_LAYERS], net_floats;
  float slope, epsilon;
  const float* weights;
  double action_space[32];
};

struct SamplerRec {
  int on, cap, D, f64, A, P;
// ... 40 lines not shown
__device__ __forceinline__ dq_f4 dq_ldw(__amdgpu_buffer_rsrc_t rs, int soff_bytes, unsigned lane_off) {
  return __builtin_bit_cast(dq_f4, __builtin_amdgcn_raw_buffer_load_b128(rs, (int)lane_off, soff_bytes, 0));
}

__device__ __forceinline__ void dq_barrier() { asm volatile("s_waitcnt lgkmcnt(0)\n\ts_barrier" ::: "memory"); }

template <int MT, int NT, int H, bool FULL>
__device__ __forceinline__ void dq_pass(dq_f4 (&ring)[DQ_SLOTS], dq_f4 (&acc)[DQ_TILE_MAX / 16][4], dq_f4 (&acur)[DQ_TILE_MAX / 16], const float* xk, int nvalid,
                                        __amdgpu_buffer_rsrc_t rs, int refill, unsigned lane_off) {
  dq_f4 an_[MT];
#pragma unroll
  for (int p = 0; p < DQ_PASS; p++) {
    const int kbl = p / NT, nt = p % NT;
    if (nt == 0) {
#pragma unroll
      for (int mt = 0; mt < MT; mt++) an_[mt] = *(const dq_f4*)(xk + mt * 16 * DQ_LD + (kbl + 1) * 16);
    }
    const dq_f4 b_ = ring[H * DQ_PASS + p];
    ring[H * DQ_PASS + p] = dq_ldw(rs, refill + p * 1024, lane_off);
    if (FULL || p < nvalid) {
#pragma unroll
      for (int s = 0; s < 4; s++)
#pragma unroll
        for (int mt = 0; mt < MT; mt++) acc[mt][nt] = __builtin_amdgcn_mfma_f32_16x16x4f32(b_[s], acur[mt][s], acc[mt][nt], 0, 0, 0);
    }
    if (nt == NT - 1) {
#pragma unroll
      for (int mt = 0; mt < MT; mt++) acur[mt] = an_[mt];
    }
  }
}

template <int MT, int NT, int H>
__device__ __forceinline__ void dq_pass_any(dq_f4 (&ring)[DQ_SLOTS], dq_f4 (&acc)[DQ_TILE_MAX / 16][4], dq_f4 (&acur)[DQ_TILE_MAX / 16], const float* xk, int nvalid,
                                            __amdgpu_buffer_rsrc_t rs, int refill, unsigned lane_off) {
  if (nvalid >= DQ_PASS) dq_pass<MT, NT, H, true>(ring, acc, acur, xk, nvalid, rs, refill, lane_off);
  else dq_pass<MT, NT, H, false>(ring, acc, acur, xk, nvalid, rs, refill, lane_off);
}

template <int MT, int NT>
__device__ __forceinline__ void dq_epilogue(dq_f4 (&acc)[DQ_TILE_MAX / 16][4], const dq_f4 (&bv)[4], float* __restrict__ Xout, int col0, int colstep, bool act, float slope) {
  const int lane = threadIdx.x & 63, r = lane & 15, g = lane >> 4;
#pragma unroll
  for (int nt = 0; nt < NT; nt++) {
    const int col = col0 + nt * colstep + g * 4;
#pragma unroll
    for (int mt = 0; mt < MT; mt++) {
      dq_f4 v = acc[mt][nt] + bv[nt];
      if (act) {
#pragma unroll
        for (int e = 0; e < 4; e++) v[e] = v[e] > 0.f ? v[e] : v[e] * slope;
      }
      *(dq_f4*)(Xout + (mt * 16 + r) * DQ_LD + col) = v;
      acc[mt][nt] = dq_f4{0.f, 0.f, 0.f, 0.f};
    }
  }
}

__device__ __forceinline__ void dq_bias(dq_f4 (&bv)[4], const float* bias, int Npad, int w, int g) {
  const int sh = dq_sh(Npad), col0 = (Npad == 16 ? 0 : Npad == 32 ? (w & 1) : w) * 16, colstep = Npad <= 32 ? 16 : 64;
#pragma unroll
  for (int nt = 0; nt < 4; nt++) bv[nt] = *(const dq_f4*)(bias + col0 + min(nt, (1 << sh) - 1) * colstep + g * 4);
}

__device__ __forceinline__ unsigned long long dq_mix64(unsigned long long seed, unsigned long long key) {
  unsigned long long x = seed * 0x9E3779B97F4A7C15ull + key * 0xBF58476D1CE4E5B9ull + 0x94D049BB133111EBull;
  x ^= x >> 30; x *= 0xBF58476D1CE4E5B9ull;
  x ^= x >> 27; x *= 0x94D049BB133111EBull;
  x ^= x >> 31;
  return x;
}

__device__ __forceinline__ const int32_t* dq_shfl_ptr(const int32_t* p, int src) {
  const unsigned long long u = (unsigned long long)p;
  const unsigned lo = (unsigned)__shfl((int)(unsigned)u, src), hi = (unsigned)__shfl((int)(unsigned)(u >> 32), src);
  return (const int32_t*)(((unsigned long long)hi << 32) | lo);
}

__device__ __forceinline__ void dq_state_wave(const CimParams& K, const DqnParams& M, int env, const int32_t* __restrict__ decisions,
                                              const int* c_info, float* __restrict__ xrows, float* __restrict__ state_out, const SamplerRec& R) {
  const int lane = threadIdx.x & 63;
  const int dl = lane < 8 ? decisions[(size_t)env * 8 + lane] : 0;
  const int32_t* hdr = K.priv + (size_t)env * K.PW;
  const int flags = hdr[PH_FLAGS], htick = hdr[PH_TICK];
  int over = 0, pact = 0, pj = 0;
  long long head = 0;
  if (R.on) {
    over = (int)R.eoe[env] | (int)R.done[env];
    head = R.head[env];
    pact = R.prev_active[env];
    pj = (int)R.prev_j[env];
  }
  const int tick = __builtin_amdgcn_readlane(dl, 0), port = __builtin_amdgcn_readlane(dl, 1), vessel = __builtin_amdgcn_readlane(dl, 2);
  if (over || __builtin_amdgcn_readlane(dl, 7) != 1 || (unsigned)port >= (unsigned)K.P) return;
  const int32_t* livef = K.live + (size_t)env * K.FW;
  const int vv = (unsigned)vessel < (unsigned)K.V ? vessel : 0;
  const int kw = K.f_vessels + VA_LAST_LOC_IDX * K.V + vv;
  const int k_live = livef[kw];
  const int Lr = K.v_route_len[vv], rb = K.v_route_base[vv], start = K.v_start[vv];
  long long last = -1;
  if (R.on) last = R.last[(size_t)env * R.P + port];
  const int n_ticks = M.look_back - 1;
  const int fi = max(0, tick - lane);
  const int slot = fi % K.S;
  const int held = lane < n_ticks ? K.ring_fi[(size_t)env * K.S + slot] : -1;
  const bool paused = (flags & (FL_FRESH | FL_FINISHED)) == 0;
  const int cur_fi = (htick - K.start_tick) / K.resolution;
  const int32_t* fptr = nullptr;
  if (held == fi) fptr = K.ring + ((size_t)env * K.S + slot) * K.FW;
  if (paused && slot == cur_fi % K.S) fptr = fi == cur_fi ? livef : nullptr;
  if (lane >= n_ticks) fptr = nullptr;
  const int32_t* now = dq_shfl_ptr(fptr, 0);
  now = (const int32_t*)(((unsigned long long)(unsigned)__builtin_amdgcn_readfirstlane((int)((unsigned long long)now >> 32)) << 32) |
                         (unsigned)__builtin_amdgcn_readfirstlane((int)(unsigned long long)now));
  const int k = now == livef ? k_live : now ? now[kw] : 0;
  const int x0 = (start + k) % Lr;
  int node = port;
  if (lane >= 1 && lane < M.n_nodes) node = now ? (int)K.route_port[rb + (x0 + lane) % Lr] : 0;
  const int kp0 = M.kpad[0];
  const size_t cbase = (size_t)env * R.cap;
  const int s0 = (int)(head & ((long long)R.cap - 1)), s1 = pact ? pj : -1, s2 = last >= 0 ? (int)(last & ((long long)R.cap - 1)) : -1;
  int32_t raw[4];
  int inf[4];
  unsigned okm = 0;
#pragma unroll
  for (int i = 0; i < 4; i++) {
    const int c = lane + 64 * i;
    const int info = c < kp0 ? c_info[c] : -1;
    inf[i] = info;
    const int ti = info & 0xff, ni = (info >> 8) & 0x7f, word = info >> 16;
    const bool vessel_col = ni == 0x7f;
    const int32_t* f = dq_shfl_ptr(fptr, ti & 63);
    const int nd = vessel_col ? vessel : __shfl(node, ni & 63);
    const bool ok = info >= 0 && f != nullptr && (unsigned)nd < (unsigned)(vessel_col ? K.V : K.P);
    const int w = vessel_col ? K.f_vessels + word * K.V + nd : word + nd;
    raw[i] = *(ok ? f + w : K.live);
    okm |= (unsigned)ok << i;
  }
#pragma unroll
  for (int i = 0; i < 4; i++) {
    const int c = lane + 64 * i;
    if (c < kp0) {
      const float v = !((okm >> i) & 1) ? 0.f : ((inf[i] >> 15) & 1) ? bits_f(raw[i]) : (float)raw[i];
      xrows[(size_t)env * kp0 + c] = v;
      if (inf[i] >= 0) {
        if (state_out) state_out[(size_t)env * M.state_dim + c] = v;
        if (R.on) {
          rec_store(R.c_state, (cbase + s0) * R.D + c, v, R.f64);
          if (s1 >= 0) rec_store(R.c_next_state, (cbase + s1) * R.D + c, v, R.f64);
          if (s2 >= 0) rec_store(R.c_nas, (cbase + s2) * R.D + c, v, R.f64);
        }
      }
    }
  }
}

}

extern "C" __global__ void __launch_bounds__(256)
mrx_k_cim_dqn_prep(CimParams K, cim::DqnParams M, int n_bin, const int32_t* __restrict__ decisions, int32_t* __restrict__ cnt,
                   int32_t* __restrict__ lists, int32_t* __restrict__ n_actions, unsigned long long* __restrict__ counter, int sched_per,
                   float* __restrict__ xrows, float* __restrict__ state_out, cim::SamplerRec R) {
  using namespace cim;
  const int n_envs = K.n_envs, P = K.P;
  const int first_state = n_bin + (sched_per > 0 ? 1 : 0);
  if ((int)blockIdx.x >= first_state) {
    __shared__ int c_info[DQ_MAX_WIDTH];
    const int t = threadIdx.x, kp0 = M.kpad[0];
    const int per_tick = M.n_nodes * M.n_pa, n_port_feats = (M.look_back - 1) * per_tick;
    if (t < kp0) {
      int info = -1;
      if (t < n_port_feats) {
        const int ti = t / per_tick, rem = t - ti * per_tick, ni = rem / M.n_pa, a = M.pa[rem - ni * M.n_pa];
        info = ti | (ni << 8) | ((a == PA_TRANSFER_COST ? 1 : 0) << 15) | ((K.f_ports + a * K.P) << 16);
      } else if (t < M.state_dim) {
        info = 0 | (0x7f << 8) | (M.va[t - n_port_feats] << 16);
      }
      c_info[t] = info;
    }
    __syncthreads();
    const int env = __builtin_amdgcn_readfirstlane(((int)blockIdx.x - first_state) * 4 + (t >> 6));
    if (env < n_envs) dq_state_wave(K, M, env, decisions, c_info, xrows, state_out, R);
    return;
  }
  if (sched_per > 0 && (int)blockIdx.x == n_bin) {
    mrx_schedule_block((const uint8_t*)K.hint, nullptr, 0, n_envs, sched_per & 0xffffff, K.order, K.sched, sched_per >> 24);
    return;
  }
  __shared__ int lcnt[64], base[64];
  const int t = threadIdx.x, e = blockIdx.x * blockDim.x + t;
  if (t < 64) lcnt[t] = 0;
  __syncthreads();
  int port = -1, rank = 0;
  if (e < n_envs) {
    const int32_t* d = decisions + (size_t)e * 8;
    bool over = false;
    if (R.on) {
      const bool was_over = R.eoe[e] != 0;
      over = was_over || R.done[e] != 0;
      if (over) {
        if (!was_over) R.eoe[e] = 1;
        if (R.prev_active[e]) {
          const size_t row = ((size_t)e * R.cap + (size_t)R.prev_j[e]) * R.D;
          if (R.f64) for (int k = 0; k < R.D; k++) ((double*)R.c_next_state)[row + k] = ((const double*)R.c_state)[row + k];
          else for (int k = 0; k < R.D; k++) ((float*)R.c_next_state)[row + k] = ((const float*)R.c_state)[row + k];
          R.prev_active[e] = 0;
        }
      }
    }
    if (!over && d[7] == 1 && (unsigned)d[1] < (unsigned)P) {
      port = d[1];
      rank = atomicAdd(&lcnt[port], 1);
    }
    n_actions[e] = port >= 0 ? 1 : 0;
  }
  __syncthreads();
  if (t < P && lcnt[t] > 0) {
    base[t] = atomicAdd(&cnt[t], lcnt[t]);
    if (counter) atomicAdd(counter, (unsigned long long)lcnt[t]);
  }
  __syncthreads();
  if (port >= 0) lists[(size_t)port * n_envs + base[port] + rank] = e;
}

template <int DQ_TILE>
__device__ __forceinline__ void mrx_dqn_mlp_body(const CimParams& K, const cim::DqnParams& M, const int32_t* __restrict__ decisions, int32_t* __restrict__ cnt,
                                                 const int32_t* __restrict__ lists, const float* __restrict__ xrows, int32_t* __restrict__ actions,
                                                 float* __restrict__ q_out, int32_t* __restrict__ choice_out, const cim::SamplerRec& R) {
  using namespace cim;
  __shared__ __attribute__((aligned(16))) float X[2][DQ_TILE * DQ_LD + 16];
  const int t = threadIdx.x, lane = t & 63;
  const int w = __builtin_amdgcn_readfirstlane(t >> 6);

  int port, rows, first;
  {
    const int c = lane < K.P ? cnt[lane] : 0;
    const int nt = (c + DQ_TILE - 1) / DQ_TILE;
    int incl = nt;
    for (int o = 1; o < 64; o <<= 1) {
      const int up = __shfl_up(incl, o);
      if (lane >= o) incl += up;
    }
    const int total = __builtin_amdgcn_readlane(incl, 63);
    int tile_idx = (int)blockIdx.x;
    if (M.xcd_runs) {
      const int run = (total + 7) >> 3, x = (int)blockIdx.x & 7, slot = (int)blockIdx.x >> 3;
      tile_idx = slot < run ? x * run + slot : total;
    }
    const int b = tile_idx - (incl - nt);
    const unsigned long long hit = __ballot(tile_idx < total && b >= 0 && b < nt);
    port = hit ? __builtin_amdgcn_readfirstlane((int)__builtin_ctzll(hit)) : -1;
    const int src = port < 0 ? 0 : port;
    first = __builtin_amdgcn_readfirstlane(__shfl(b * DQ_TILE, src));
    rows = __builtin_amdgcn_readfirstlane(__shfl(min(DQ_TILE, c - b * DQ_TILE), src));
  }
  if (port < 0) {
    dq_barrier();
    if (t == 0) {
      int32_t* done = cnt + 64;
      if (atomicAdd(done, 1) == (int)gridDim.x - 1) {
        for (int p = 0; p < 64; p++) cnt[p] = 0;
        *done = 0;
      }
    }
    return;
  }
  const int32_t* list = lists + (size_t)port * K.n_envs + first;
  const float* net = M.weights + (size_t)port * M.net_floats;
  constexpr int MT = DQ_TILE / 16;
  const int r16 = lane & 15, g4 = lane >> 4;
  const unsigned lane_off = (unsigned)lane * 16;
  dq_f4 ring[DQ_SLOTS], bv[4], bvn[4];
  const __amdgpu_buffer_rsrc_t rs = dq_rsrc(net);
  int soff = (int)M.s_off[w][0] * 4;
#pragma unroll
  for (int p = 0; p < DQ_SLOTS; p++) ring[p] = dq_ldw(rs, soff + p * 1024, lane_off);
  int lw = 0;
  while (lw < M.n_layers && dq_idle(M.npad[lw], w)) lw++;
  dq_bias(bv, net + M.b_off[lw < M.n_layers ? lw : 0], M.npad[lw < M.n_layers ? lw : 0], w, g4);
#ifdef MRX_DQN_PROFILE
  long long tm[12]; int tmi = 0;
  const long long rt0 = (long long)__builtin_amdgcn_s_memrealtime();
#define DQ_MARK() do { dq_barrier(); tm[tmi++] = (long long)__builtin_amdgcn_s_memtime(); } while (0)
  __shared__ long long dq_tl[4][64];
  int tli = 0;
#ifdef MRX_DQN_PROFILE_T
#define DQ_T() do { if (lane == 0 && tli < 64) dq_tl[w][tli] = (long long)__builtin_amdgcn_s_memtime(); tli++; } while (0)
#else
#define DQ_T() do {} while (0)
#endif
#else
#define DQ_MARK() do {} while (0)
#define DQ_T() do {} while (0)
#endif
  DQ_MARK();

  int32_t dq_d[5] = {0, 0, 0, 0, 0};
  int32_t dq_space = 0, dq_early = 0, dq_env = -1;
  long long dq_head = 0, dq_seed = 0, dq_last = -1;
  if (t < rows) {
    const int env = list[t];
    dq_env = env;
    const int32_t* d = decisions + (size_t)env * 8;
#pragma unroll
    for (int i = 0; i < 5; i++) dq_d[i] = d[i];
    const int32_t* live = K.live + (size_t)env * K.FW;
    const int v = (unsigned)dq_d[2] < (unsigned)K.V ? dq_d[2] : 0;
    dq_space = live[K.f_vessels + VA_REMAINING_SPACE * K.V + v];
    dq_early = live[K.f_vessels + VA_EARLY_DISCHARGE * K.V + v];
    if (R.on) {
      dq_head = R.head[env];
      const int agent = dq_d[1] < 0 ? 0 : (dq_d[1] >= R.P ? R.P - 1 : dq_d[1]);
      dq_last = R.last[(size_t)env * R.P + agent];
    }
    if (M.epsilon > 0.f) dq_seed = K.seed[env];
  }
  {
    const int kp0 = M.kpad[0], q4 = kp0 >> 2;
    for (int i = t; i < DQ_TILE * q4; i += 256) {
      const int r = i / q4, c4 = i - r * q4;
      dq_f4 v = dq_f4{0.f, 0.f, 0.f, 0.f};
      if (r < rows) v = *(const dq_f4*)(xrows + (size_t)list[r] * kp0 + c4 * 4);
      *(dq_f4*)(&X[0][r * DQ_LD + c4 * 4]) = v;
    }
  }
  dq_barrier();
  DQ_MARK();

  int cur = 0, half = 0;
  dq_f4 acc[DQ_TILE_MAX / 16][4], acur[DQ_TILE_MAX / 16];
#pragma unroll
  for (int mt = 0; mt < DQ_TILE_MAX / 16; mt++) {
    acur[mt] = dq_f4{0.f, 0.f, 0.f, 0.f};
#pragma unroll
    for (int nt = 0; nt < 4; nt++) acc[mt][nt] = dq_f4{0.f, 0.f, 0.f, 0.f};
  }
  for (int l = 0; l < M.n_layers; l++) {
    DQ_T();
    if (l == lw) {
      const int Npad = M.npad[l], sh = dq_sh(Npad), F = (M.kpad[l] >> 4) << sh;
      int ln = l + 1;
      while (ln < M.n_layers && dq_idle(M.npad[ln], w)) ln++;
      const int lb = ln < M.n_layers ? ln : l;
      dq_bias(bvn, net + M.b_off[lb], M.npad[lb], w, g4);
      const float* xlane = X[cur] + r16 * DQ_LD + g4 * 4;
#pragma unroll
      for (int mt = 0; mt < MT; mt++) acur[mt] = *(const dq_f4*)(xlane + mt * 16 * DQ_LD);
      DQ_T();
      for (int f0 = 0; f0 < F; f0 += DQ_PASS) {
        const int nvalid = F - f0;
        const float* xk = xlane + (f0 >> sh) * 16;
        const int refill = soff + DQ_SLOTS * 1024;
        if (half == 0) {
          if (sh == 0) dq_pass_any<MT, 1, 0>(ring, acc, acur, xk, nvalid, rs, refill, lane_off);
          else if (sh == 1) dq_pass_any<MT, 2, 0>(ring, acc, acur, xk, nvalid, rs, refill, lane_off);
          else dq_pass_any<MT, 4, 0>(ring, acc, acur, xk, nvalid, rs, refill, lane_off);
        } else {
          if (sh == 0) dq_pass_any<MT, 1, 1>(ring, acc, acur, xk, nvalid, rs, refill, lane_off);
          else if (sh == 1) dq_pass_any<MT, 2, 1>(ring, acc, acur, xk, nvalid, rs, refill, lane_off);
          else dq_pass_any<MT, 4, 1>(ring, acc, acur, xk, nvalid, rs, refill, lane_off);
        }
        half ^= 1;
        soff += DQ_PASS * 1024;
        DQ_T();
      }
      const bool act = l + 1 < M.n_layers;
      const int col0 = (Npad == 16 ? 0 : Npad == 32 ? (w & 1) : w) * 16, colstep = Npad <= 32 ? 16 : 64;
      if (sh == 0) dq_epilogue<MT, 1>(acc, bv, X[cur ^ 1], col0, colstep, act, M.slope);
      else if (sh == 1) dq_epilogue<MT, 2>(acc, bv, X[cur ^ 1], col0, colstep, act, M.slope);
      else dq_epilogue<MT, 4>(acc, bv, X[cur ^ 1], col0, colstep, act, M.slope);
      DQ_T();
      lw = ln;
#pragma unroll
      for (int nt = 0; nt < 4; nt++) bv[nt] = bvn[nt];
    }
    dq_barrier();
    DQ_T();
    cur ^= 1;
    DQ_MARK();
  }
  if (t == 0) {
    int32_t* done = cnt + 64;
    if (atomicAdd(done, 1) == (int)gridDim.x - 1) {
      for (int p = 0; p < 64; p++) cnt[p] = 0;
      *done = 0;
    }
  }

  if (t < rows) {
// ... 88 lines not shown
```

maro_amd/csrc/cim_engine.hip:

```cpp
#include <hip/hip_runtime.h>
#include <stdio.h>
#include <stdlib.h>
#include <string.h>

#include <mutex>
#include <new>
#include <string>
#include <vector>

#include "wave.h"
#include "cim_prof.h"
#include "cim_device.h"
#include "cim_layout.h"

#include "cim_step_kernels.h"


__device__ __forceinline__ unsigned mrx_nz16(uint4 v, unsigned m = 0xffffffffu) {
  auto nib = [m](unsigned w) { w &= m; return ((((w | ((w & 0x7f7f7f7fu) + 0x7f7f7f7fu)) >> 7) & 0x01010101u) * 0x01020408u) >> 24; };
  return nib(v.x) | (nib(v.y) << 4) | (nib(v.z) << 8) | (nib(v.w) << 12);
}

__device__ __forceinline__ void mrx_schedule_block(const uint8_t* __restrict__ hint, const uint8_t* __restrict__ mask, int mask_vec, int n, int per,
                                                   int32_t* __restrict__ order, int32_t* __restrict__ sched, int lpt) {
  __shared__ int s_l[16], s_t[16], s_f[16];
  const int tid = threadIdx.x, lane = tid & 63, wid = tid >> 6;
  const int lo = tid * per, hi = lo + per < n ? lo + per : n;
  auto piece = [&](int p0, unsigned& l, unsigned& t, unsigned& f) {
    const unsigned valid = p0 + 16 <= n ? 0xffffu : ((1u << (n - p0)) - 1u);
    const uint4 hv = *(const uint4*)(hint + p0);
    const unsigned tk = mrx_nz16(hv), lg = lpt ? mrx_nz16(hv, 0x02020202u) : 0u;
    unsigned on = 0xffffu;
    if (mask) {
      if (mask_vec && p0 + 16 <= n) on = mrx_nz16(*(const uint4*)(mask + p0));
      else { on = 0; for (int b = 0; b < 16 && p0 + b < n; b++) on |= mask[p0 + b] ? (1u << b) : 0u; }
    }
    l = lg & on & valid;
    t = tk & ~lg & on & valid;
    f = ~tk & on & valid;
  };
  int cl = 0, ct = 0, cf = 0;
  unsigned long long bl = 0, bt = 0, bf = 0;
  const bool small = per <= 64;
  for (int p0 = lo; p0 < hi; p0 += 16) {
    unsigned l, t, f;
    piece(p0, l, t, f);
    cl += __builtin_popcount(l); ct += __builtin_popcount(t); cf += __builtin_popcount(f);
    if (small) { bl |= (unsigned long long)l << (p0 - lo); bt |= (unsigned long long)t << (p0 - lo); bf |= (unsigned long long)f << (p0 - lo); }
  }
  int il = cl, it = ct, jf = cf;
  for (int d = 1; d < 64; d <<= 1) {
    const int w = __shfl_up(il, d, 64), u = __shfl_up(it, d, 64), v = __shfl_up(jf, d, 64);
    if (lane >= d) { il += w; it += u; jf += v; }
  }
  if (lane == 63) { s_l[wid] = il; s_t[wid] = it; s_f[wid] = jf; }
  __syncthreads();
  int base_l = 0, base_t = 0, base_f = 0, tot_l = 0, tot_t = 0, tot_f = 0;
  const int n_waves = (int)(blockDim.x >> 6);
  for (int w = 0; w < n_waves; w++) {
    if (w < wid) { base_l += s_l[w]; base_t += s_t[w]; base_f += s_f[w]; }
    tot_l += s_l[w]; tot_t += s_t[w]; tot_f += s_f[w];
  }
  int ol = base_l + il - cl, ot = tot_l + base_t + it - ct, of = tot_l + tot_t + base_f + jf - cf;
  if (small) {
    for (unsigned long long m = bl; m; m &= m - 1) order[ol++] = (lo + __builtin_ctzll(m)) | MRX_ORDER_TICK;
    for (unsigned long long m = bt; m; m &= m - 1) order[ot++] = (lo + __builtin_ctzll(m)) | MRX_ORDER_TICK;
    for (unsigned long long m = bf; m; m &= m - 1) order[of++] = lo + __builtin_ctzll(m);
  } else {
    for (int p0 = lo; p0 < hi; p0 += 16) {
      unsigned l, t, f;
      piece(p0, l, t, f);
      for (; l; l &= l - 1) order[ol++] = (p0 + __builtin_ctz(l)) | MRX_ORDER_TICK;
      for (; t; t &= t - 1) order[ot++] = (p0 + __builtin_ctz(t)) | MRX_ORDER_TICK;
      for (; f; f &= f - 1) order[of++] = p0 + __builtin_ctz(f);
    }
  }
  const int n_full = tot_l + tot_t;
  for (int i = n_full + tot_f + tid; i < n; i += (int)blockDim.x) order[i] = -1;
  if (tid < 16) sched[tid] = tid == 0 ? n_full : tid == 1 ? n_full + tot_f : tid >= 8 ? -1 : 0;
}

extern "C" __global__ void __launch_bounds__(1024)
mrx_k_cim_schedule(const uint8_t* __restrict__ hint, const uint8_t* __restrict__ mask, int mask_vec, int n, int per, int32_t* __restrict__ order,
                   int32_t* __restrict__ sched, int lpt) {
  mrx_schedule_block(hint, mask, mask_vec, n, per, order, sched, lpt);
}

#ifndef MRX_DQN_TILE_DEFAULT
#define MRX_DQN_TILE_DEFAULT 16
#endif
#include "cim_dqn.h"
#include "cim_sampler.h"

struct AttrList { int n; int32_t id[16]; };

extern "C" __global__ void __launch_bounds__(256)
mrx_k_cim_query(CimParams K, int node_type, const int32_t* __restrict__ ticks, int nt, int ticks_per_env,
                const int32_t* __restrict__ nodes, int nn, int nodes_per_env, AttrList al, int row_slots, long long total,
                double* __restrict__ out) {
  const long long rt = blockIdx.x;
  const int per_row = nn * row_slots;
  for (int j = threadIdx.x; j < per_row; j += blockDim.x) {
    const int ni = j / row_slots;
    out[rt * per_row + j] = cim::query_elem(K, node_type, ticks, nt, ticks_per_env, nodes, nn, nodes_per_env, al.id, al.n, rt * nn + ni, j - ni * row_slots);
  }
}

__device__ __forceinline__ unsigned long long mrx_mix64(unsigned long long seed, unsigned long long step) {
  unsigned long long x = seed * 0x9E3779B97F4A7C15ull + step * 0xBF58476D1CE4E5B9ull + 0x94D049BB133111EBull;
  x ^= x >> 30; x *= 0xBF58476D1CE4E5B9ull;
  x ^= x >> 27; x *= 0x94D049BB133111EBull;
  x ^= x >> 31;
  return x;
}

extern "C" __global__ void __launch_bounds__(256)
mrx_k_cim_random_policy(CimParams K, const int32_t* __restrict__ decisions, long long step, int32_t* __restrict__ actions,
                        int32_t* __restrict__ n_actions, unsigned long long* __restrict__ counter, int sched_per) {
  if (sched_per > 0 && blockIdx.x == 0) {
    mrx_schedule_block((const uint8_t*)K.hint, nullptr, 0, K.n_envs, sched_per & 0xffffff, K.order, K.sched, sched_per >> 24);
    return;
  }
  const int env = (int)((blockIdx.x - (sched_per > 0 ? 1 : 0)) * blockDim.x + threadIdx.x);
  bool valid = false;
  if (env < K.n_envs) {
    const int32_t* d = decisions + (size_t)env * 8;
    valid = d[7] == 1;
    int32_t* a = actions + (size_t)env * K.max_actions * 4;
    if (valid) {
      const unsigned long long key = step >= 0 ? (unsigned long long)step : (((unsigned long long)(unsigned)d[0] << 8) | (unsigned)d[2]) + 0x100000000ull;
      const unsigned long long x = mrx_mix64((unsigned long long)K.seed[env], key);
      const unsigned long long r = x >> 1;
      const int load = d[3], dis = d[4];
      a[0] = d[2]; a[1] = d[1];
      if ((x & 1ull) == 0 && load > 0) { a[2] = (int)(r % (unsigned long long)(load + 1)); a[3] = MRX_ACTION_LOAD; }
      else { a[2] = (int)(r % (unsigned long long)(dis + 1)); a[3] = MRX_ACTION_DISCHARGE; }
    }
    n_actions[env] = valid ? 1 : 0;
  }
  if (counter) {
    const unsigned long long m = __ballot(valid);
    if ((threadIdx.x & 63) == 0 && m) atomicAdd(counter, (unsigned long long)__builtin_popcountll(m));
  }
}

template <class T>
__global__ void __launch_bounds__(64)
mrx_k_cim_sampler_record(int n, int P, int D, int cap, int A, int first, const int32_t* __restrict__ dec, const float* __restrict__ state,
                         const int32_t* __restrict__ choice, const int32_t* __restrict__ acts, int32_t* __restrict__ nact, uint8_t* __restrict__ eoe,
                         const uint8_t* __restrict__ done, long long* __restrict__ head, long long* __restrict__ last, long long* __restrict__ prev_j, uint8_t* __restrict__ prev_active,
                         int32_t* __restrict__ c_tick, long long* __restrict__ c_agent, T* __restrict__ c_state, long long* __restrict__ c_action,
                         int32_t* __restrict__ c_env_action, uint8_t* __restrict__ c_terminal, T* __restrict__ c_next_state, T* __restrict__ c_nas,
                         long long* __restrict__ steps_env) {
  const int e = (int)blockIdx.x, lane = (int)threadIdx.x;
  const bool was_over = eoe[e] != 0;
  const bool over = was_over || (done && done[e] != 0);
  if (over && !was_over && lane == 0) eoe[e] = 1;
  const float* st = state + (size_t)e * D;
  const long long ring = (long long)cap - 1;
  if (!first && prev_active[e]) {
    const long long pj = prev_j[e];
    T* ns = c_next_state + ((size_t)e * cap + pj) * D;
    const T* own = c_state + ((size_t)e * cap + pj) * D;
    for (int d = lane; d < D; d += 64) ns[d] = over ? own[d] : (T)st[d];
  }
  if (over) {
    if (lane == 0) { nact[e] = 0; prev_active[e] = 0; }
    return;
  }
  const long long q = head[e], j = q & ring;
  int agent = dec[(size_t)e * 8 + 1];
  agent = agent < 0 ? 0 : (agent >= P ? P - 1 : agent);
  const long long prev = last[(size_t)e * P + agent], pslot = prev & ring;
  T* cs = c_state + ((size_t)e * cap + j) * D;
  for (int d = lane; d < D; d += 64) cs[d] = (T)st[d];
  if (prev >= 0) {
    T* na = c_nas + ((size_t)e * cap + pslot) * D;
    for (int d = lane; d < D; d += 64) na[d] = (T)st[d];
  }
  if (lane < 4) c_env_action[((size_t)e * cap + j) * 4 + lane] = acts[(size_t)e * A * 4 + lane];
  if (lane == 0) {
    c_tick[(size_t)e * cap + j] = dec[(size_t)e * 8];
    c_agent[(size_t)e * cap + j] = agent;
    c_action[(size_t)e * cap + j] = choice[e];
    c_terminal[(size_t)e * cap + j] = 0;
    if (prev >= 0) c_terminal[(size_t)e * cap + pslot] = 0;
    last[(size_t)e * P + agent] = q;
    head[e] = q + 1;
    prev_j[e] = j;
    prev_active[e] = 1;
    steps_env[e] += 1;
  }
}

template <class T>
__global__ void __launch_bounds__(256)
mrx_k_cim_sampler_emit(int P, int D, int cap, int frames, int window, double ff, double sf, const double* __restrict__ decay,
                       const long long* __restrict__ rows, const long long* __restrict__ tail, const long long* __restrict__ n_emit,
                       const long long* __restrict__ out_off, const int32_t* __restrict__ hist, const int32_t* __restrict__ c_tick,
                       const long long* __restrict__ c_agent, const T* __restrict__ c_state, const long long* __restrict__ c_action,
                       const int32_t* __restrict__ c_env_action, const uint8_t* __restrict__ c_terminal, const T* __restrict__ c_next_state,
                       const T* __restrict__ c_nas, T* __restrict__ o_state, long long* __restrict__ o_action, int32_t* __restrict__ o_env_action,
                       float* __restrict__ o_reward, T* __restrict__ o_next_state, T* __restrict__ o_nas, uint8_t* __restrict__ o_terminal,
// ... 227 lines not shown
int mrx_cim_get_layout(mrx_handle h, mrx_cim_layout* out) {
  if (!h || !out) return set_err(MRX_ERR_INVALID_ARG, "null handle/out");
  *out = h->plan.layout;
  return MRX_OK;
}

int mrx_cim_reset(mrx_handle h, const int64_t* d_seed_cmd, const uint8_t* d_env_mask, void* stream) {
  if (!h) return set_err(MRX_ERR_INVALID_ARG, "null handle");
  h->order_ready = false;
  int rc = use_device(h->device);
  if (rc != MRX_OK) return rc;
  const CimParams& K = h->plan.kp;
  const bool table = K.pregen && K.orders_stride && d_seed_cmd && !K.data_mode;
  if (h->spec_module) {
    CimParams Kc = K;
    const long long* cmd = (const long long*)d_seed_cmd;
    long long dflt = -1;
    void* params[] = {&Kc, &cmd, &d_env_mask, &dflt};
    HIP_TRY(hipModuleLaunchKernel(h->spec_reset, (unsigned)K.n_envs, 1, 1, 64, 1, 1, (unsigned)((size_t)K.lds_words_reset * 4), (hipStream_t)stream, params, nullptr));
    if (table)
      HIP_TRY(hipModuleLaunchKernel(h->spec_order_table, (unsigned)K.n_envs, 1, 1, 64, 1, 1, (unsigned)((size_t)K.lds_words_gen * 4), (hipStream_t)stream, params, nullptr));
    return MRX_OK;
  }
  hipLaunchKernelGGL(mrx_k_cim_reset, dim3(K.n_envs), dim3(64), (size_t)K.lds_words_reset * 4, (hipStream_t)stream, K,
                     (const long long*)d_seed_cmd, d_env_mask, (long long)-1);
  if (table)
    hipLaunchKernelGGL(mrx_k_cim_order_table, dim3(K.n_envs), dim3(64), (size_t)K.lds_words_gen * 4, (hipStream_t)stream, K,
                       (const long long*)d_seed_cmd, d_env_mask, (long long)-1);
  HIP_TRY(hipGetLastError());
  return MRX_OK;
}

static int launch_step(mrx_handle h, const int32_t* d_actions, const int32_t* d_n_actions, const int32_t* d_n_answered,
                       const uint8_t* d_env_mask, int32_t* d_decisions, int64_t* d_metrics, uint8_t* d_done, void* stream);

int mrx_cim_step(mrx_handle h, const int32_t* d_actions, const int32_t* d_n_actions, const uint8_t* d_env_mask,
                 int32_t* d_decisions, int64_t* d_metrics, uint8_t* d_done, void* stream) {
  if (h && h->plan.kp.decision_mode != 0) return set_err(MRX_ERR_INVALID_ARG, "engine was created in a Joint decision mode: use mrx_cim_step_joint");
  return launch_step(h, d_actions, d_n_actions, nullptr, d_env_mask, d_decisions, d_metrics, d_done, stream);
}

int mrx_cim_step_joint(mrx_handle h, const int32_t* d_actions, const int32_t* d_n_actions, const int32_t* d_n_answered,
                       const uint8_t* d_env_mask, int32_t* d_decisions, int64_t* d_metrics, uint8_t* d_done, void* stream) {
  if (h && h->plan.kp.decision_mode == 0) return set_err(MRX_ERR_INVALID_ARG, "engine was created in Sequential decision mode: use mrx_cim_step");
  return launch_step(h, d_actions, d_n_actions, d_n_answered, d_env_mask, d_decisions, d_metrics, d_done, stream);
}

static int effective_step_mode(mrx_handle h) {
  static const int env_mode = getenv("MRX_CIM_STEP_MODE") ? atoi(getenv("MRX_CIM_STEP_MODE")) : 0;
  int m = h->step_mode ? h->step_mode : env_mode;
  if (m < 1 || m > 5) m = 2;
  if (m == 3) m = 2;
  if (m == 4 && h->spec_module && !(h->spec_fast && h->spec_loop)) m = 2;
  if (m == 5 && h->spec_module && !h->spec_fast) m = 2;
  return m;
}

static int resident_waves(const void* kern, size_t lds_bytes, int device) {
  int per_cu = 0, cus = 0;
  if (hipOccupancyMaxActiveBlocksPerMultiprocessor(&per_cu, kern, 64, lds_bytes) != hipSuccess || per_cu <= 0) per_cu = 8;
  if (hipDeviceGetAttribute(&cus, hipDeviceAttributeMultiprocessorCount, device) != hipSuccess || cus <= 0) cus = 256;
  if (getenv("MRX_CIM_LOOP_WAVES_PER_CU")) per_cu = atoi(getenv("MRX_CIM_LOOP_WAVES_PER_CU"));
  return per_cu * cus;
}

static int launch_step(mrx_handle h, const int32_t* d_actions, const int32_t* d_n_actions, const int32_t* d_n_answered,
                       const uint8_t* d_env_mask, int32_t* d_decisions, int64_t* d_metrics, uint8_t* d_done, void* stream) {
  if (!h || !d_decisions || !d_metrics || !d_done) return set_err(MRX_ERR_INVALID_ARG, "null handle/output pointer");
  int rc = use_device(h->device);
  if (rc != MRX_OK) return rc;
  const CimParams& K = h->plan.kp;
  static const size_t lds_pad = getenv("MRX_DEBUG_LDS_PAD_BYTES") ? (size_t)atoi(getenv("MRX_DEBUG_LDS_PAD_BYTES")) : 0;
  const bool obs = h->obs.np > 0 || h->obs.nv > 0;
  const int mode = effective_step_mode(h);
  cim::StepBatch B = {d_actions, d_n_actions, d_n_answered, d_decisions, (long long*)d_metrics, d_done};
  if (h->obs.agent_mode) {
    h->obs.agent_key = h->agent_key;
    if (h->agent_key >= 0) h->agent_key++;
  }
  const bool have_order = h->order_ready && !d_env_mask && stream == h->order_stream;
  h->order_ready = false;
  if (mode >= 2 && !have_order) {
    const int per = ((K.n_envs + 1023) / 1024 + 15) / 16 * 16;
    hipLaunchKernelGGL(mrx_k_cim_schedule, dim3(1), dim3(1024), 0, (hipStream_t)stream, (const uint8_t*)K.hint, d_env_mask,
                       ((uintptr_t)d_env_mask & 15) ? 0 : 1, K.n_envs, per, K.order, K.sched, h->lpt);
  }
  const int sorted = mode == 5 ? 2 : mode >= 2 ? 1 : 0;
  const size_t lds_bytes = (size_t)K.lds_words * 4 + lds_pad;
  if (mode == 4) {
    const unsigned fast_blocks = (unsigned)((K.n_envs + 63) / 64);
    if (h->spec_module) {
      CimParams Kc = K;
      CimObs Oc = h->obs;
      void* pf[] = {&Kc, &Oc, &B, &d_env_mask};
      HIP_TRY(hipModuleLaunchKernel(h->spec_fast, fast_blocks, 1, 1, 64, 1, 1, 0, (hipStream_t)stream, pf, nullptr));
      void* pl[] = {&Kc, &Oc, &B};
      const int W = h->loop_waves < K.n_envs ? h->loop_waves : K.n_envs;
      HIP_TRY(hipModuleLaunchKernel(h->spec_loop, (unsigned)W, 1, 1, 64, 1, 1, (unsigned)lds_bytes, (hipStream_t)stream, pl, nullptr));
      return MRX_OK;
    }
#define MRX_LAUNCH_SPLIT(SUFFIX)                                                                                                    \
    {                                                                                                                              \
      if (!h->loop_waves) h->loop_waves = resident_waves((const void*)mrx_k_cim_step_loop##SUFFIX, lds_bytes, h->device);                       \
      const int W = h->loop_waves < K.n_envs ? h->loop_waves : K.n_envs;                                                           \
      hipLaunchKernelGGL(mrx_k_cim_fast_lanes##SUFFIX, dim3(fast_blocks), dim3(64), 0, (hipStream_t)stream, K, h->obs, B, d_env_mask); \
      hipLaunchKernelGGL(mrx_k_cim_step_loop##SUFFIX, dim3(W), dim3(64), lds_bytes, (hipStream_t)stream, K, h->obs, B);            \
    }
    if (K.pregen) { if (obs) MRX_LAUNCH_SPLIT(_tab_obs) else MRX_LAUNCH_SPLIT(_tab) }
    else { if (obs) MRX_LAUNCH_SPLIT(_obs) else MRX_LAUNCH_SPLIT() }
#undef MRX_LAUNCH_SPLIT
    HIP_TRY(hipGetLastError());
    return MRX_OK;
  }
  if (mode == 5) {
    const unsigned fast_blocks = (unsigned)((K.n_envs + 63) / 64);
    if (h->spec_module) {
      CimParams Kc = K;
      CimObs Oc = h->obs;
      void* pf[] = {&Kc, &Oc, &B, &d_env_mask};
      HIP_TRY(hipModuleLaunchKernel(h->spec_fast, fast_blocks, 1, 1, 64, 1, 1, 0, (hipStream_t)stream, pf, nullptr));
    } else if (K.pregen) {
      if (obs) hipLaunchKernelGGL(mrx_k_cim_fast_lanes_tab_obs, dim3(fast_blocks), dim3(64), 0, (hipStream_t)stream, K, h->obs, B, d_env_mask);
      else hipLaunchKernelGGL(mrx_k_cim_fast_lanes_tab, dim3(fast_blocks), dim3(64), 0, (hipStream_t)stream, K, h->obs, B, d_env_mask);
    } else {
      if (obs) hipLaunchKernelGGL(mrx_k_cim_fast_lanes_obs, dim3(fast_blocks), dim3(64), 0, (hipStream_t)stream, K, h->obs, B, d_env_mask);
      else hipLaunchKernelGGL(mrx_k_cim_fast_lanes, dim3(fast_blocks), dim3(64), 0, (hipStream_t)stream, K, h->obs, B, d_env_mask);
    }
  }
  if (h->spec_module) {
    CimParams Kc = K;
    CimObs Oc = h->obs;
    int srt = sorted;
    void* params[] = {&Kc, &Oc, &B, &d_env_mask, &srt};
    const int kw = K.wg_waves > 0 ? K.wg_waves : 1;
    HIP_TRY(hipModuleLaunchKernel(h->spec_fn[(K.pregen ? 2 : 0) + (obs ? 1 : 0)], (unsigned)((K.n_envs + kw - 1) / kw), 1, 1, (unsigned)(64 * kw), 1, 1,
                                  (unsigned)((K.lean_ok ? ((size_t)kw * K.l_ctab + K.ctab_words + 3) / 4 * 16 : (size_t)K.lds_words * 4) + lds_pad), (hipStream_t)stream, params, nullptr));
    return MRX_OK;
  }
  auto kern = K.pregen ? (obs ? mrx_k_cim_step_tab_obs : mrx_k_cim_step_tab) : (obs ? mrx_k_cim_step_obs : mrx_k_cim_step);
  hipLaunchKernelGGL(kern, dim3(K.n_envs), dim3(64), (size_t)K.lds_words * 4 + lds_pad, (hipStream_t)stream, K, h->obs, B, d_env_mask, sorted);
  HIP_TRY(hipGetLastError());
  return MRX_OK;
}

int mrx_cim_set_device_agent(mrx_handle h, int mode, int32_t* d_actions, int32_t* d_n_actions, int32_t* d_counts, int64_t next_key) {
  if (!h) return set_err(MRX_ERR_INVALID_ARG, "null handle");
  if (mode != 0 && mode != 1) return set_err(MRX_ERR_INVALID_ARG, "device agent mode must be 0 (off) or 1 (random legal)");
  if (mode && (!d_actions || !d_n_actions)) return set_err(MRX_ERR_INVALID_ARG, "null action buffers");
  if (mode && h->plan.kp.decision_mode != 0) return set_err(MRX_ERR_UNSUPPORTED, "the device agent answers Sequential decisions only");
  h->obs.agent_mode = mode;
  h->obs.agent_actions = mode ? d_actions : nullptr;
  h->obs.agent_n_actions = mode ? d_n_actions : nullptr;
  h->obs.agent_count = mode ? d_counts : nullptr;
  h->agent_key = next_key;
  return MRX_OK;
}

int mrx_cim_set_step_mode(mrx_handle h, int mode) {
  if (!h) return set_err(MRX_ERR_INVALID_ARG, "null handle");
  if (mode < 0 || mode > 5) return set_err(MRX_ERR_INVALID_ARG, "step mode must be 0 (automatic), 1, 2, 4 or 5");
  h->step_mode = mode;
  return effective_step_mode(h);
}

static std::string plan_defines(const CimParams& K, const CimObs& O);
static int make_obs(const int32_t* port_attrs, int n_port_attrs, const int32_t* vessel_attrs, int n_vessel_attrs, CimObs* out);

// ... 512 lines not shown
```

maro_amd/csrc/cim_layout.h:

```cpp
#pragma once
#include <math.h>
#include <stdint.h>
#include <stdlib.h>
#include <string.h>

#include <string>
#include <utility>
#include <vector>

#include "../../include/maro_amd.h"
#include "cim_params.h"

struct CimHostPlan {
  CimParams kp;
  mrx_cim_layout layout;
  std::vector<uint8_t> const_blob;
  int64_t const_off = 0;
  int64_t workspace_bytes = 0;
  int64_t o_live, o_ring, o_ring_fi, o_priv, o_rec, o_status, o_tick, o_nstops, o_order_prop, o_mt, o_stops, o_seed, o_vperiod, o_orders, o_hint, o_order, o_sched;
  std::vector<std::pair<size_t, int64_t>> binds;
  int64_t ctab_rel = 0;
  int64_t shared_orders_rel = -1;
};

namespace cim_layout_detail {
inline int64_t align_up(int64_t x, int64_t a) { return (x + a - 1) / a * a; }
struct Arena {
  int64_t top = 0;
  int64_t take(int64_t bytes) { int64_t o = align_up(top, 256); top = o + bytes; return o; }
};
template <class T>
inline int64_t blob_put(std::vector<uint8_t>& blob, const T* src, size_t n, size_t align = 64) {
  size_t off = (blob.size() + align - 1) / align * align;
  blob.resize(off + sizeof(T) * (n ? n : 1), 0);
  if (n) memcpy(blob.data() + off, src, sizeof(T) * n);
  return (int64_t)off;
}
}

inline int cim_stop_bound(const mrx_cim_topology* t, int v, int max_tick) {
  int r = t->vessel_route[v];
  int L = t->route_offset[r + 1] - t->route_offset[r];
  double cyc = 0;
  for (int i = 0; i < L; i++) {
    double park = ceil(t->vessel_duration[v] - t->vessel_duration_noise[v]);
    if (park < 1) park = 1;
    double sp = t->vessel_speed[v] + t->vessel_speed_noise[v];
    double sail = sp > 0 ? ceil(t->route_dist[t->route_offset[r] + i] / sp) : 1;
    if (sail < 0) sail = 0;
    cyc += park + sail;
  }
  if (cyc < 1) cyc = 1;
  double cycles = ceil((double)(max_tick + 1) / cyc) + 1;
  return (int)(cycles * L) + t->future_stop_number + 2;
}

typedef int (*order_fast_probe_fn)();
inline order_fast_probe_fn& order_fast_probe() {
  static order_fast_probe_fn f = nullptr;
  return f;
}

inline int cim_plan(const mrx_cim_topology* t, const mrx_cim_config* c, CimHostPlan* pl, std::string* err) {
  using namespace cim_layout_detail;
  auto fail = [&](const char* m) { if (err) *err = m; return (int)MRX_ERR_UNSUPPORTED; };
  if (!t || !c) { if (err) *err = "null topology/config"; return MRX_ERR_INVALID_ARG; }
  if (c->n_envs <= 0 || c->durations <= 0 || c->snapshot_resolution <= 0) { if (err) *err = "n_envs, durations and snapshot_resolution must be positive"; return MRX_ERR_INVALID_ARG; }
  if (t->n_ports <= 0 || t->n_ports > 64) return fail("engine limit: 1..64 ports (one lane per port)");
  if (t->n_vessels <= 0 || t->n_vessels > 64) return fail("engine limit: 1..64 vessels (one lane per vessel)");
  if (t->container_volume <= 0) return fail("container_volume must be positive");
  if (c->n_envs >= (1 << 30)) return fail("engine limit: n_envs < 2^30");
  {
    auto bad = [&](const char* m) { if (err) *err = m; return (int)MRX_ERR_INVALID_ARG; };
    if (t->period < 1 || !t->order_dist) return bad("topology: period must be >= 1 (order_dist[period])");
    if (t->n_routes <= 0 || t->n_targets < 0 || t->n_route_points <= 0) return bad("topology: n_routes / n_route_points must be positive, n_targets >= 0");
    if (!t->route_offset || !t->route_port || !t->target_offset || !t->vessel_route || !t->vessel_start_offset) return bad("topology: null index array");
    if (t->n_targets > 0 && !t->target_port) return bad("topology: null target_port");
    if (t->route_offset[0] != 0 || t->route_offset[t->n_routes] != t->n_route_points) return bad("topology: route_offset must run from 0 to n_route_points");
    for (int r = 0; r < t->n_routes; r++) if (t->route_offset[r + 1] < t->route_offset[r]) return bad("topology: route_offset must be non-decreasing");
    for (int i = 0; i < t->n_route_points; i++) if (t->route_port[i] < 0 || t->route_port[i] >= t->n_ports) return bad("topology: route_port out of range");
    if (t->target_offset[0] != 0 || t->target_offset[t->n_ports] != t->n_targets) return bad("topology: target_offset must run from 0 to n_targets");
    for (int p = 0; p < t->n_ports; p++) if (t->target_offset[p + 1] < t->target_offset[p]) return bad("topology: target_offset must be non-decreasing");
    for (int i = 0; i < t->n_targets; i++) if (t->target_port[i] < 0 || t->target_port[i] >= t->n_ports) return bad("topology: target_port out of range");
    for (int v = 0; v < t->n_vessels; v++) {
      const int r = t->vessel_route[v];
      if (r < 0 || r >= t->n_routes) return bad("topology: vessel_route out of range");
      const int L = t->route_offset[r + 1] - t->route_offset[r];
      if (t->vessel_start_offset[v] < 0 || t->vessel_start_offset[v] >= (L > 0 ? L : 1)) return bad("topology: vessel_start_offset out of range");
    }
  }
  CimParams& k = pl->kp;
  memset(&k, 0, sizeof(k));
  const int P = t->n_ports, V = t->n_vessels, R = t->n_routes, NT = t->n_targets, NRP = t->n_route_points;
  k.n_envs = c->n_envs; k.P = P; k.V = V; k.R = R; k.NT = NT; k.NRP = NRP;
  k.past_n = t->past_stop_number; k.future_n = t->future_stop_number;
  if (k.past_n < 0 || k.future_n < 0 || k.past_n > 16 || k.future_n > 16) return fail("stop_number out of range (0..16)");
  k.vrows = 10;
  k.start_tick = c->start_tick; k.T = c->start_tick + c->durations; k.resolution = c->snapshot_resolution;
  k.max_actions = c->max_actions > 0 ? c->max_actions : 1;
  if (c->decision_mode < 0 || c->decision_mode > 2) { if (err) *err = "decision_mode must be 0, 1 or 2"; return MRX_ERR_INVALID_ARG; }
  k.decision_mode = c->decision_mode;
  k.period = t->period; k.vol = t->container_volume; k.total_containers = t->total_containers; k.order_mode = t->order_mode;
// ... 235 lines not shown
  k.l_ctab = (k.lds_words + 3) / 4 * 4;
  k.lds_words_lean = (k.l_ctab + k.ctab_words + 3) / 4 * 4;
  k.l_rfull = k.lds_words_lean;
  k.l_oq = k.l_rfull + (H * NT + 3) / 4 * 4;
  k.l_odelay = k.l_oq;
  k.lds_words = (k.l_oq + NT + 1 + 3) / 4 * 4;
  k.lean_ok = (k.pregen && NT <= 192 && H <= 4) ? 1 : 0;
  if (NRP >= (1 << 19) || rec_w >= (1 << 15)) k.lean_ok = 0;
  if (k.SMAX >= (1 << 16)) k.lean_ok = 0;
  {
    int best_k = 1, best_waves = 0;
    for (int kk = 1; kk <= 4; kk++) {
      const long long bytes = ((long long)kk * k.l_ctab + k.ctab_words + 3) / 4 * 4 * 4;
      const long long gran = (bytes + 1279) / 1280;
      const int waves = gran > 128 ? 0 : (int)(128 / gran) * kk;
      if (waves > best_waves) { best_waves = waves; best_k = kk; }
    }
    best_k = 1;
    if (const char* ev = getenv("MRX_CIM_WG_WAVES")) { const int v = atoi(ev); if (v >= 1 && v <= 16 && k.lean_ok) best_k = v; }
    k.wg_waves = best_k;
  }
  k.l_mt2 = 0; k.l_mt3 = MT_WORDS; k.r_mt0 = 2 * MT_WORDS; k.r_mt1 = 3 * MT_WORDS;
  k.lds_words_reset = 4 * MT_WORDS > k.FW + k.PWH ? 4 * MT_WORDS : (k.FW + k.PWH + 3) / 4 * 4;
  if (k.pregen) {
    int g = 0;
    k.g_mt0 = g; g += MT_WORDS;
    k.g_dsrc = g; g += dsrc_w;
    k.g_dtgt = g; g += dtgt_w;
    k.g_oq = g; g += NT + 1;
    k.g_srcn = g; g += P;
    g = (g + 1) / 2 * 2;
    k.g_srctab = g; g += 4 * P;
    k.g_ctab = (g + 3) / 4 * 4;
    k.lds_words_gen = (k.g_ctab + k.ctab_words + 3) / 4 * 4;
    k.order_fast = 0;
    {
      const char* ev = getenv("MRX_ORDER_FAST");
      bool ok = k.order_half && k.use_order_rng && P <= 63 && P + NT <= 192 && !(ev && atoi(ev) == 0);
      if (ok && order_fast_probe()) {
        static const int veto = order_fast_probe()();
        if (veto) ok = false;
      }
      const double margin = 9.094947017729282e-13, cap = 1048576.0;
      auto entry_ok = [&](double b, double n) { return (b == 0.0 && n == 0.0) || b - fabs(n) >= margin; };
      double tot = 0, tot_min = 0;
      for (int p = 0; p < P && ok; p++) {
        if (!entry_ok(t->source_base[p], t->source_noise[p])) ok = false;
        tot += t->source_base[p] + fabs(t->source_noise[p]);
        tot_min += t->source_base[p] - fabs(t->source_noise[p]);
      }
      if (!(tot <= cap && tot_min >= margin)) ok = false;
      for (int p = 0; p < P && ok; p++) {
        double ts = 0, ts_min = 0;
        for (int i = t->target_offset[p]; i < t->target_offset[p + 1]; i++) {
          if (!entry_ok(t->target_base[i], t->target_noise[i])) ok = false;
          ts += t->target_base[i] + fabs(t->target_noise[i]);
          ts_min += t->target_base[i] - fabs(t->target_noise[i]);
        }
        if (t->target_offset[p + 1] > t->target_offset[p] && !(ts <= cap && ts_min >= margin)) ok = false;
      }
      if (ok) {
        int slots = (P + 3) / 4 * 4;
        for (int p = 0; p < P; p++) slots += (t->target_offset[p + 1] - t->target_offset[p] + 3) / 4 * 4;
        k.gf_slots = slots;
        int f = 0;
        k.gf_win = f; f += 2 * MT_WORDS;
        k.gf_val = f; f += 2 * (slots + 6);
        f = (f + 3) / 4 * 4;
        k.gf_rec = f; f += 8 * (P + 1);
        k.gf_pre = f; f += NT + 2;
        f = (f + 3) / 4 * 4;
        k.gf_row = f; f += k.NTP / 2;
        k.gf_seg = f; f += P + 1;
        k.order_fast = 1;
        k.lds_words_gen = (f + 3) / 4 * 4;
      }
    }
  }
  if ((int64_t)k.lds_words_reset * 4 > 160 * 1024 || (int64_t)k.lds_words * 4 > 160 * 1024) return fail("engine limit: per-env state exceeds 160 KiB of LDS");

  Arena A;
  const int64_t N = c->n_envs;
  pl->const_off = A.take((int64_t)B.size());
  pl->o_live = A.take(N * k.FW * 4);
  pl->o_ring = A.take(N * (int64_t)k.S * k.FW * 4);
  pl->o_ring_fi = A.take(N * k.S * 4);
  pl->o_priv = A.take(N * k.PW * 4);
  pl->o_rec = A.take(N * (int64_t)k.REC_W * 4);
  pl->o_status = A.take(N * 4);
  pl->o_tick = A.take(N * 4);
  pl->o_nstops = A.take(N * V * 4);
  pl->o_order_prop = A.take(N * (int64_t)k.T * 4);
  pl->o_mt = A.take(N * MTS_COUNT * MT_WORDS * 4);
  pl->o_stops = A.take(N * (int64_t)V * k.SMAX * 4);
  pl->o_seed = A.take(N * 8);
  pl->o_vperiod = A.take(N * V * 4);
  pl->o_hint = A.take(N + 64);
  pl->o_order = A.take(N * 4);
  pl->o_sched = A.take(64 + 64 * MRX_PIPE_MAX_WAVES);
  pl->shared_orders_rel = shared_orders_rel;
  k.orders_stride = shared_orders_rel >= 0 ? 0 : (long long)c->durations * k.NTP;
  pl->o_orders = (k.pregen && shared_orders_rel < 0) ? A.take(N * (int64_t)c->durations * k.NTP * (k.order_half ? 2 : 4)) : 0;
  pl->workspace_bytes = align_up(A.top, 256);

  mrx_cim_layout& Lo = pl->layout;
  memset(&Lo, 0, sizeof(Lo));
  Lo.n_envs = c->n_envs; Lo.n_ports = P; Lo.n_vessels = V; Lo.frame_words = k.FW; Lo.ring_slots = k.S;
  Lo.max_stops = k.SMAX; Lo.horizon = k.H;
  Lo.frame_off_ports = k.f_ports; Lo.frame_off_vessels = k.f_vessels; Lo.frame_off_full_on_ports = k.f_fop;
  Lo.frame_off_full_on_vessels = k.f_fov; Lo.frame_off_vessel_plans = k.f_plans;
  Lo.off_live = pl->o_live; Lo.off_ring = pl->o_ring; Lo.off_ring_fi = pl->o_ring_fi; Lo.off_status = pl->o_status;
  Lo.off_tick = pl->o_tick; Lo.off_seed = pl->o_seed; Lo.off_stops = pl->o_stops; Lo.off_nstops = pl->o_nstops;
  Lo.off_order_prop = pl->o_order_prop; Lo.off_vessel_period = pl->o_vperiod;
  Lo.off_orders = shared_orders_rel >= 0 ? pl->const_off + shared_orders_rel : pl->o_orders; Lo.order_row_words = k.NTP; Lo.order_table_on = k.pregen; Lo.order_elem_bytes = k.pregen ? (k.order_half ? 2 : 4) : 0;
  Lo.workspace_bytes = pl->workspace_bytes;
  return MRX_OK;
}

inline void cim_plan_bind(CimHostPlan* pl, void* base_) {
  uint8_t* base = (uint8_t*)base_;
  CimParams& k = pl->kp;
  uint8_t* cb = base + pl->const_off;
  for (auto& bd : pl->binds) *(const void**)((char*)&k + bd.first) = cb + bd.second;
  k.ctab = (const int32_t*)(cb + pl->ctab_rel);
  k.live = (int32_t*)(base + pl->o_live); k.ring = (int32_t*)(base + pl->o_ring); k.ring_fi = (int32_t*)(base + pl->o_ring_fi);
  k.priv = (int32_t*)(base + pl->o_priv); k.rec = (int32_t*)(base + pl->o_rec); k.status = (int32_t*)(base + pl->o_status);
  k.tick = (int32_t*)(base + pl->o_tick); k.nstops = (int32_t*)(base + pl->o_nstops);
  k.order_prop = (int32_t*)(base + pl->o_order_prop); k.mt = (uint32_t*)(base + pl->o_mt);
  k.stops = (uint32_t*)(base + pl->o_stops); k.seed = (int64_t*)(base + pl->o_seed);
  k.vperiod = (int32_t*)(base + pl->o_vperiod);
  k.hint = base + pl->o_hint; k.order = (int32_t*)(base + pl->o_order); k.sched = (int32_t*)(base + pl->o_sched);
  k.orders = !k.pregen ? nullptr : pl->shared_orders_rel >= 0 ? (int32_t*)(cb + pl->shared_orders_rel) : (int32_t*)(base + pl->o_orders);
}
```

maro_amd/csrc/cim_params.h:

```cpp
#pragma once
#include <stdint.h>

enum { PA_CAPACITY, PA_EMPTY, PA_FULL, PA_ON_SHIPPER, PA_ON_CONSIGNEE, PA_SHORTAGE, PA_ACC_SHORTAGE,
       PA_BOOKING, PA_ACC_BOOKING, PA_FULFILLMENT, PA_ACC_FULFILLMENT, PA_TRANSFER_COST, PA_COUNT };
enum { VA_CAPACITY, VA_EMPTY, VA_FULL, VA_REMAINING_SPACE, VA_EARLY_DISCHARGE, VA_IS_PARKING, VA_LOC_PORT_IDX,
       VA_ROUTE_IDX, VA_LAST_LOC_IDX, VA_NEXT_LOC_IDX, VA_PAST_STOP_LIST, VA_PAST_STOP_TICK_LIST,
       VA_FUTURE_STOP_LIST, VA_FUTURE_STOP_TICK_LIST, VA_COUNT };
enum { MA_FULL_ON_PORTS, MA_FULL_ON_VESSELS, MA_VESSEL_PLANS, MA_COUNT };

enum { PH_TICK, PH_FLAGS, PH_PEND_LO, PH_PEND_HI, PH_CUR_VESSEL, PH_OPNUM_LO, PH_OPNUM_HI, PH_IDX_ORDER,
       PH_IDX_BUFFER, PH_IDX_ROUTE, PH_ZOMBIE_LO, PH_ZOMBIE_HI ,
       PH_ACCB_LO, PH_ACCB_HI, PH_ACCS_LO, PH_ACCS_HI , PH_COUNT = 16 };
enum { FL_FRESH = 1, FL_FINISHED = 2, FL_LONG = 4  };

#define MT_WORDS 624
enum { MTS_ORDER = 0, MTS_BUFFER = 1, MTS_ROUTE = 2, MTS_COUNT = 3 };

struct CimParams {
  int n_envs, P, V, R, NT, NRP, past_n, future_n, vrows, FW, S, H, SMAX, T, start_tick, resolution,
      max_actions, period;
  int vol, total_containers, order_mode;
  int use_order_rng, use_buffer_rng, has_order_init;
  int idx_order_init, idx_route, idx_order_num, idx_buffer;
  double sample_noise;
  int f_ports, f_vessels, f_fop, f_fov, f_plans;
  int misc_cap;
  int NC;
  int PW, PWH , pv_evt, pv_next, pv_pos, pv_krl, pv_period, pv_rfull, pv_rempty;
  int REC_W;
  int l_frame, l_priv, l_mt0, l_mt1, l_dsrc, l_dtgt, l_oq, l_odelay, l_srcn, l_misc, lds_words;
  int l_ctab, ctab_words;
  int wg_waves;
  int l_mt2, l_mt3, r_mt0, r_mt1, lds_words_reset;
  int l_rfull, lds_words_lean, lean_ok;
  int decision_mode;
  int data_mode;
  int data_T;
  long long data_seed;
  long long orders_stride;
  int order_half;
  const uint32_t* fx_stops;
  const int32_t *fx_nstops, *fx_vperiod, *fx_order_prop;
  int pregen, NTP;
  int g_mt0, g_dsrc, g_dtgt, g_oq, g_srcn, g_srctab, g_ctab, lds_words_gen;
  int order_fast, gf_win, gf_val, gf_rec, gf_pre, gf_row, gf_seg, gf_slots;
  const double *src_base, *src_noise, *tgt_base, *tgt_noise, *er_base, *er_noise, *fr_base, *fr_noise,
      *v_speed, *v_speed_noise, *v_dur, *v_dur_noise, *route_dist, *order_dist;
  const int32_t *tgt_off, *tgt_port, *pair_src, *route_port, *v_route_base, *v_route_len, *v_start, *v_cap,
      *v_init_empty, *v_total_space, *p_cap, *p_init_empty, *leg_off, *leg_time, *v_period, *er_delay,
      *fr_delay, *rec_off, *v_route, *v_cbase, *route_cidx, *cidx_dense, *pair_dense;
  const int32_t* lean_tab;
  const int32_t* ctab;
  const uint16_t *h_tgt_off, *h_route_port, *h_v_route_base, *h_v_route_len, *h_leg_off, *h_leg_time,
      *h_rec_off, *h_v_cbase, *h_route_cidx, *h_pair_src;
  int32_t *live, *ring, *ring_fi, *priv, *rec, *status, *tick, *nstops, *order_prop, *vperiod, *orders;
  uint32_t *mt, *stops;
  int64_t* seed;
  uint8_t* hint;
  int32_t* order;
  int32_t* sched;
};
#define MRX_ORDER_TICK 0x40000000
#define MRX_PIPE_MAX_WAVES 4096

#define MRX_CIM_DIM_FIELDS(X) \
  X(P) \
  X(V) \
  X(R) \
  X(NT) \
  X(NRP) \
  X(past_n) \
  X(future_n) \
  X(vrows) \
  X(FW) \
  X(S) \
  X(H) \
  X(SMAX) \
  X(T) \
  X(start_tick) \
  X(resolution) \
  X(max_actions) \
  X(period) \
  X(vol) \
  X(total_containers) \
  X(order_mode) \
  X(use_order_rng) \
  X(use_buffer_rng) \
  X(has_order_init) \
  X(idx_order_init) \
  X(idx_route) \
  X(idx_order_num) \
  X(idx_buffer) \
  X(f_ports) \
  X(f_vessels) \
  X(f_fop) \
  X(f_fov) \
  X(f_plans) \
  X(misc_cap) \
  X(NC) \
  X(PW) \
  X(PWH) \
  X(pv_evt) \
  X(pv_next) \
  X(pv_pos) \
  X(pv_krl) \
  X(pv_period) \
  X(pv_rfull) \
  X(pv_rempty) \
  X(REC_W) \
  X(l_frame) \
  X(l_priv) \
  X(l_mt0) \
  X(l_mt1) \
  X(l_dsrc) \
  X(l_dtgt) \
  X(l_oq) \
  X(l_odelay) \
  X(l_srcn) \
  X(l_misc) \
  X(lds_words) \
  X(l_ctab) \
  X(ctab_words) \
  X(wg_waves) \
  X(decision_mode) \
  X(data_mode) \
  X(data_T) \
  X(pregen) \
  X(order_half) \
  X(NTP) \
  X(l_mt2) \
  X(l_mt3) \
  X(r_mt0) \
  X(r_mt1) \
  X(l_rfull) \
  X(lds_words_lean) \
  X(lean_ok) \
  X(lds_words_reset) \
  X(g_mt0) \
  X(g_dsrc) \
  X(g_dtgt) \
  X(g_oq) \
  X(g_srcn) \
  X(g_srctab) \
  X(g_ctab) \
  X(lds_words_gen) \
// ... 24 lines not shown
```

maro_amd/csrc/cim_sampler.h:

```cpp
#pragma once
#include <hip/hip_runtime.h>

#include "cim_dqn.h"

namespace cim {

struct SamplerEnd {
  SamplerRec R;
  long long* tail;
  int window, frames;
  double ff, sf;
  const double* decay;
  int32_t* hist;
};

}

extern "C" __global__ void __launch_bounds__(64)
mrx_k_cim_sampler_finalize(CimParams K, cim::SamplerEnd E, long long* __restrict__ n_emit) {
  const cim::SamplerRec& R = E.R;
  const int e = (int)blockIdx.x, lane = (int)threadIdx.x;
  const bool was_over = R.eoe[e] != 0;
  const bool over = was_over || R.done[e] != 0;
  if (over && !was_over && lane == 0) R.eoe[e] = 1;
  const int tick_now = K.tick[e];
  if (over && R.prev_active[e]) {
    const size_t row = ((size_t)e * R.cap + (size_t)R.prev_j[e]) * R.D;
    if (R.f64) for (int k = lane; k < R.D; k += 64) ((double*)R.c_next_state)[row + k] = ((const double*)R.c_state)[row + k];
    else for (int k = lane; k < R.D; k += 64) ((float*)R.c_next_state)[row + k] = ((const float*)R.c_state)[row + k];
  }
  if (!over && tick_now >= 0 && tick_now < E.frames) {
    const int32_t* live = K.live + (size_t)e * K.FW + K.f_ports;
    int32_t* row = E.hist + ((size_t)e * E.frames + (size_t)tick_now) * 2 * K.P;
    if (lane < K.P) { row[lane] = live[PA_FULFILLMENT * K.P + lane]; row[K.P + lane] = live[PA_SHORTAGE * K.P + lane]; }
  }
  const long long head = R.head[e], tail = E.tail[e], ring = (long long)R.cap - 1;
  const long long bound = (long long)tick_now - E.window;
  long long cnt = 0;
  for (long long q0 = tail; q0 < head; q0 += 64) {
    const long long q = q0 + lane;
    const bool ok = q < head && (long long)R.c_tick[(size_t)e * R.cap + (size_t)(q & ring)] <= bound;
    const unsigned long long m = __ballot(ok);
    if (m == ~0ull) { cnt += 64; continue; }
    cnt += __builtin_ctzll(~m);
    break;
  }
  __syncthreads();
  if (lane == 0) {
    n_emit[e] = cnt;
    if (over) R.prev_active[e] = 0;
  }
}

extern "C" __global__ void __launch_bounds__(1024)
mrx_k_cim_sampler_scan(int n, const long long* __restrict__ n_emit, const long long* __restrict__ head, const long long* __restrict__ tail,
                       const uint8_t* __restrict__ eoe, const uint8_t* __restrict__ prev_active, long long* __restrict__ out_off,
                       long long* __restrict__ info) {
  __shared__ long long part[1024], pmax[1024], pover[1024], ppend[1024];
  const int t = (int)threadIdx.x, per = (n + 1023) / 1024, lo = t * per, hi = min(n, lo + per);
  long long s = 0, mx = 0, ov = 0, pe = 0;
  for (int e = lo; e < hi; e++) {
    s += n_emit[e];
    const long long left = head[e] - tail[e] - n_emit[e];
    mx = left > mx ? left : mx;
    ov += eoe[e] != 0;
    pe += (n_emit[e] > 0 && left == 0 && eoe[e] == 0 && prev_active[e] != 0) ? 1 : 0;
  }
  part[t] = s; pmax[t] = mx; pover[t] = ov; ppend[t] = pe;
  __syncthreads();
  for (int o = 1; o < 1024; o <<= 1) {
    const long long v = t >= o ? part[t - o] : 0;
    const long long m2 = t >= o ? pmax[t - o] : 0, o2 = t >= o ? pover[t - o] : 0, p2 = t >= o ? ppend[t - o] : 0;
    __syncthreads();
    part[t] += v; pmax[t] = m2 > pmax[t] ? m2 : pmax[t]; pover[t] += o2; ppend[t] += p2;
    __syncthreads();
  }
  long long run = part[t] - s;
  for (int e = lo; e < hi; e++) { out_off[e] = run; run += n_emit[e]; }
  if (t == 1023) { info[0] = part[t]; info[1] = pmax[t]; info[2] = pover[t]; info[3] = ppend[t]; }
}

template <class T>
__global__ void __launch_bounds__(256)
mrx_k_cim_sampler_emit_all(cim::SamplerEnd E, int rows_cap, const long long* __restrict__ n_emit, const long long* __restrict__ out_off,
                           T* __restrict__ o_state, long long* __restrict__ o_action, int32_t* __restrict__ o_env_action,
                           float* __restrict__ o_reward, T* __restrict__ o_next_state, T* __restrict__ o_nas, uint8_t* __restrict__ o_terminal,
                           int32_t* __restrict__ o_env_id, int32_t* __restrict__ o_tick, int32_t* __restrict__ o_agent) {
  extern __shared__ int32_t hrows[];
  const cim::SamplerRec& R = E.R;
  const int e = (int)blockIdx.x, t = (int)threadIdx.x, w = t >> 6, lane = t & 63;
  const long long ne = n_emit[e];
  if (ne <= 0) return;
  const long long t0 = E.tail[e], o0 = out_off[e], ring = (long long)R.cap - 1;
  const int P = R.P, D = R.D;
  const size_t base = (size_t)e * R.cap;
  const T* cs = (const T*)R.c_state;
  const T* cn = (const T*)R.c_next_state;
  const T* ca = (const T*)R.c_nas;
  const bool eoe = R.eoe[e] != 0;
  const long long s0 = t0 & ring;
  const long long n1 = (s0 + ne <= (long long)R.cap) ? ne : (long long)R.cap - s0;
  for (int piece = 0; piece < 2; piece++) {
    const long long cnt = piece == 0 ? n1 : ne - n1;
    if (cnt <= 0) continue;
    const size_t src = (base + (size_t)(piece == 0 ? s0 : 0)) * D, dst = (size_t)(o0 + (piece == 0 ? 0 : n1)) * D;
    const size_t words = (size_t)cnt * D;
    for (size_t i = t; i < words; i += 256) {
      o_state[dst + i] = cs[src + i];
      o_next_state[dst + i] = cn[src + i];
      o_nas[dst + i] = ca[src + i];
    }
  }
  long long j = 0;
  while (j < ne) {
    const int tick_first = R.c_tick[base + (size_t)((t0 + j) & ring)];
// ... 47 lines not shown
```

maro_amd/csrc/cim_step_kernels.h:

```cpp
extern "C" __global__ void __launch_bounds__(64)
mrx_k_cim_reset(CimParams K, const long long* __restrict__ seed_cmd, const uint8_t* __restrict__ mask, long long default_cmd) {
  extern __shared__ __attribute__((aligned(16))) int32_t lds[];
  const int env = blockIdx.x;
  if (mask && !mask[env]) return;
  cim::reset_env(K, env, lds, seed_cmd ? seed_cmd[env] : default_cmd);
}

extern "C" __global__ void __launch_bounds__(64)
mrx_k_cim_order_table(CimParams K, const long long* __restrict__ seed_cmd, const uint8_t* __restrict__ mask, long long default_cmd) {
  extern __shared__ __attribute__((aligned(16))) int32_t lds[];
  const int env = blockIdx.x;
  if (mask && !mask[env]) return;
  if ((seed_cmd ? seed_cmd[env] : default_cmd) == -1) return;
  cim::gen_order_table(K, env, lds);
}

#ifndef MRX_STEP_WAVES
#define MRX_STEP_WAVES 2
#endif
#ifdef MRX_SPECIALIZED
#define MRX_WG_WAVES MRXC_wg_waves
#else
#define MRX_WG_WAVES 1
#endif
#define MRX_STEP_KERNEL(NAME, PG, OBS, WAVES)                                                                            \
  extern "C" __global__ void __launch_bounds__(64 * MRX_WG_WAVES, WAVES)                                                 \
  NAME(CimParams K, CimObs O, cim::StepBatch B, const uint8_t* __restrict__ mask, int sorted) {                          \
    extern __shared__ __attribute__((aligned(16))) int32_t lds[];                                                       \
    const int w = MRX_WG_WAVES > 1 ? __builtin_amdgcn_readfirstlane((int)(threadIdx.x >> 6)) : 0;                        \
    const int slot = (int)blockIdx.x * MRX_WG_WAVES + w;                                                                \
    if (MRX_WG_WAVES > 1 && slot >= K.n_envs) return;                                                                   \
    int env = slot, path = cim::PATH_PROBE;                                                                             \
    if (sorted) {                                                                                                       \
      if (sorted == 2 && slot >= K.sched[0]) return;   \
      const int e = K.order[slot];                                                                                      \
      if (e < 0) return;                                                                                                \
      env = e & (MRX_ORDER_TICK - 1);                                                                                   \
      path = (e & MRX_ORDER_TICK) ? cim::PATH_FULL : cim::PATH_FAST;                                                    \
    } else if (mask && !mask[env]) {                                                                                    \
      return;                                                                                                           \
    }                                                                                                                   \
    cim::step_env<PG, OBS>(K, O, env, lds + w * KD(l_ctab), cim::step_io(K, B, env), path,                               \
                           lds + MRX_WG_WAVES * KD(l_ctab));                                                            \
  }
#ifdef MRX_SPECIALIZED
#define MRX_WANT(PG, OBS) ((PG) == (MRXC_pregen != 0) && (OBS) == ((MRXC_obs_np | MRXC_obs_nv) != 0))
#else
#define MRX_WANT(PG, OBS) 1
#endif
#define MRX_SPLIT_KERNELS(SUFFIX, PG, OBS, WAVES)                                                                       \
  extern "C" __global__ void __launch_bounds__(64)                                                                      \
  mrx_k_cim_fast_lanes##SUFFIX(CimParams K, CimObs O, cim::StepBatch B, const uint8_t* __restrict__ mask) {               \
    cim::fast_lanes_env<OBS>(K, O, B, mask, (int)(blockIdx.x * 64 + threadIdx.x));                                      \
  }                                                                                                                     \
  extern "C" __global__ void __launch_bounds__(64, WAVES)                                                               \
  mrx_k_cim_step_loop##SUFFIX(CimParams K, CimObs O, cim::StepBatch B) {                                                 \
    extern __shared__ __attribute__((aligned(16))) int32_t lds[];                                                       \
    cim::step_loop<PG, OBS>(K, O, lds, (int)blockIdx.x, (int)gridDim.x, B);                                             \
  }
#if MRX_WANT(0, 0)
MRX_STEP_KERNEL(mrx_k_cim_step, false, false, MRX_STEP_WAVES)
MRX_SPLIT_KERNELS(, false, false, MRX_STEP_WAVES)
#endif
#if MRX_WANT(0, 1)
MRX_STEP_KERNEL(mrx_k_cim_step_obs, false, true, MRX_STEP_WAVES)
MRX_SPLIT_KERNELS(_obs, false, true, MRX_STEP_WAVES)
#endif
#if MRX_WANT(1, 0)
MRX_STEP_KERNEL(mrx_k_cim_step_tab, true, false, MRX_STEP_WAVES)
MRX_SPLIT_KERNELS(_tab, true, false, MRX_STEP_WAVES)
#endif
#if MRX_WANT(1, 1)
MRX_STEP_KERNEL(mrx_k_cim_step_tab_obs, true, true, MRX_STEP_WAVES)
MRX_SPLIT_KERNELS(_tab_obs, true, true, MRX_STEP_WAVES)
#endif
#undef MRX_WANT
#undef MRX_STEP_KERNEL
#undef MRX_SPLIT_KERNELS
```

Before: 154.3 million.

## Drop separate live frame; use ring slot as live state with partial snapshots

Removes the per-env live frame buffer and makes the current ring slot serve as the live state. Snapshots that land on the same slot now write only the attributes that changed (empty, transfer cost, fulfillment, remaining space, touched plan cells) instead of a full frame copy. The aim is to cut the duplicate full-frame global writes and reads on every step. In exchange it adds slot bookkeeping (a per-env slot byte, slot packing in the order word) and depends on the partial-patch invariants being correct.

```diff
diff --git a/maro_amd/cim/engine.py b/maro_amd/cim/engine.py
--- a/maro_amd/cim/engine.py
+++ b/maro_amd/cim/engine.py
@@ -64,8 +64,7 @@
         self.layout = _lib.MrxCimLayout()
         _lib.check(self._L.mrx_cim_get_layout(self._h, ctypes.byref(self.layout)), "mrx_cim_get_layout")
         lay = self.layout
-        self.live = self._view(lay.off_live, torch.int32, (self.n_envs, lay.frame_words))
-        self.ring = self._view(lay.off_ring, torch.int32, (self.n_envs, lay.ring_slots, lay.frame_words))
+        self.ring =self._view(lay.off_ring, torch.int32, (self.n_envs, lay.ring_slots, lay.frame_words))
         self.ring_fi = self._view(lay.off_ring_fi, torch.int32, (self.n_envs, lay.ring_slots))
         self.status = self._view(lay.off_status, torch.int32, (self.n_envs,))
         self.ticks = self._view(lay.off_tick, torch.int32, (self.n_envs,))
@@ -82,6 +81,12 @@
         if h:
             self._L.mrx_cim_destroy(h)
             self._h = None
+
+    @property
+    def live(self) -> torch.Tensor:
+        fi = torch.clamp(self.ticks.to(torch.int64) - self.start_tick, min=0) // self.snapshot_resolution
+        slot = fi % self.layout.ring_slots
+        return self.ring[torch.arange(self.n_envs, device=self.device), slot]
 
     def _view(self, off: int, dtype: torch.dtype, shape) -> torch.Tensor:
         n = int(np.prod(shape)) * torch.empty((), dtype=dtype).element_size()
diff --git a/maro_amd/csrc/cim_device.h b/maro_amd/csrc/cim_device.h
--- a/maro_amd/csrc/cim_device.h
+++ b/maro_amd/csrc/cim_device.h
@@ -121,6 +121,17 @@
 
 MRX_DEV float bits_f(int32_t x) { union { int32_t i; float f; } u; u.i = x; return u.f; }
 MRX_DEV int32_t f_bits(float f) { union { int32_t i; float f; } u; u.f = f; return u.i; }
+
+MRX_DEV int live_slot(const CimParams& K, int tick) {
+  const int d = tick - KD(start_tick);
+  return (d > 0 ? d / KD(resolution) : 0) % KD(S);
+}
+MRX_DEV int32_t* slot_frame(const CimParams& K, int env, int slot) { return K.ring + ((size_t)env * KD(S) + slot) * KD(FW); }
+MRX_DEV int32_t* live_frame(const CimParams& K, int env, int tick) { return slot_frame(K, env, live_slot(K, tick)); }
+MRX_DEV int order_env(int e, int& slot) {
+  slot = (e & MRX_ORDER_SLOT) ? (e >> MRX_ORDER_SLOT_SHIFT) & 127 : -1;
+  return e & ((e & MRX_ORDER_SLOT) ? MRX_ORDER_ENV_PACKED : MRX_ORDER_ENV_PLAIN);
+}
 
 MRX_DEV void copy_in_async(int32_t* lds_dst, const int32_t* gsrc, int n_words);
 MRX_DEV void stage_tables(const CimParams& K, Lds& L, int32_t* c) {
@@ -566,7 +577,7 @@
   const int P = KD(P), V = KD(V), TT = KD(T);
   uint32_t* g_mt = K.mt + (size_t)env * MTS_COUNT * MT_WORDS;
   int32_t* g_priv = K.priv + (size_t)env * KD(PW);
-  int32_t* g_live = K.live + (size_t)env * KD(FW);
+  int32_t* g_live = live_frame(K, env, KD(start_tick));
   const Tabs& T = L.tab;
 
   long long base;
@@ -745,6 +756,7 @@
     K.status[env] = status;
     K.tick[env] = KD(start_tick);
     K.hint[env] = 1;
+    K.slot[env] = (uint8_t)live_slot(K, KD(start_tick));
   }
   wave::sync();
   copy_words(g_live, L.frame, KD(FW));
@@ -1731,15 +1743,38 @@
   return arr_mask;
 }
 
-MRX_DEV void take_snapshot(const CimParams& K, const CimObs& O, int env, Lds& L, int fi) {
-  const int s = fi % KD(S);
-  copy_words(K.ring + ((size_t)env * KD(S) + s) * KD(FW), L.frame, KD(FW));
-  if (wave::lane() == 0) K.ring_fi[(size_t)env * KD(S) + s] = fi;
+MRX_DEV void snapshot_hist(const CimParams& K, const CimObs& O, int env, Lds& L, int fi) {
   if (O.hist_n > 0 && fi < O.hist_frames) {
     int32_t* row = O.hist + ((size_t)env * O.hist_frames + fi) * O.hist_n * KD(P);
     for (int a = 0; a < O.hist_n; a++)
       if (wave::lane() < KD(P)) row[a * KD(P) + wave::lane()] = FP(O.hist_attr[a], wave::lane());
   }
+}
+
+enum { SNAP_FULL = -3, PLAN_MANY = -2, PLAN_NONE = -1 };
+MRX_DEV void take_snapshot(const CimParams& K, const CimObs& O, int env, Lds& L, int fi, int patch = SNAP_FULL) {
+  const int s = fi % KD(S), lane = wave::lane();
+  int32_t* g = slot_frame(K, env, s);
+#ifdef MRX_SNAPSHOT_FULL_COPY
+  patch = SNAP_FULL;
+#endif
+  if (patch == SNAP_FULL) {
+    copy_words(g, L.frame, KD(FW));
+    if (lane == 0) K.ring_fi[(size_t)env * KD(S) + s] = fi;
+  } else {
+    if (lane < KD(P)) {
+      g[KD(f_ports) + PA_EMPTY * KD(P) + lane] = FP(PA_EMPTY, lane);
+      g[KD(f_ports) + PA_TRANSFER_COST * KD(P) + lane] = FP(PA_TRANSFER_COST, lane);
+      g[KD(f_ports) + PA_ACC_FULFILLMENT * KD(P) + lane] = FP(PA_ACC_FULFILLMENT, lane);
+    }
+    if (lane < KD(V)) {
+      g[KD(f_vessels) + VA_EMPTY * KD(V) + lane] = FV(VA_EMPTY, lane);
+      g[KD(f_vessels) + VA_REMAINING_SPACE * KD(V) + lane] = FV(VA_REMAINING_SPACE, lane);
+    }
+    if (patch >= 0) { if (lane == 0) g[KD(f_plans) + patch] = L.frame[KD(f_plans) + patch]; }
+    else if (patch == PLAN_MANY) for (int i = lane; i < KD(NC); i += 64) g[KD(f_plans) + i] = L.frame[KD(f_plans) + i];
+  }
+  snapshot_hist(K, O, env, L, fi);
 }
 
 MRX_DEV unsigned long long mix64(unsigned long long seed, unsigned long long step) {
@@ -1770,9 +1805,8 @@
 };
 
 template <bool OBS>
-MRX_DEV void fast_rows_request(const CimParams& K, const CimObs& O, int env, FastRows& R) {
+MRX_DEV void fast_rows_request(const CimParams& K, const CimObs& O, int env, const int32_t* g_live, FastRows& R) {
   const int lane = wave::lane();
-  const int32_t* g_live = K.live + (size_t)env * KD(FW);
   const int32_t* g_priv = K.priv + (size_t)env * KD(PW);
   const int p = lane < KD(P) ? lane : 0, v = lane < KD(V) ? lane : 0;
   R.hdr = lane < PH_COUNT ? g_priv[lane] : 0;
@@ -1793,7 +1827,7 @@
 MRX_DEV double port_attr_value(int attr, int raw) { return attr == PA_TRANSFER_COST ? (double)bits_f(raw) : (double)raw; }
 
 template <bool OBS>
-MRX_DEV bool fast_step(const CimParams& K, const CimObs& O, int env, const FastRows& R, int n_act, int a0v, int a0p, int a0q, int a0t,
+MRX_DEV bool fast_step(const CimParams& K, const CimObs& O, int env, int32_t* g_live, const FastRows& R, int n_act, int a0v, int a0p, int a0q, int a0t,
                        int32_t* dec_out, long long* met_out, uint8_t* done_out) {
   const int lane = wave::lane();
   const int P = KD(P), V = KD(V);
@@ -1811,7 +1845,6 @@
   const int cur = wave::bcast(hdr, PH_CUR_VESSEL);
   const uint64_t pend_after = pend & ~(1ull << (cur & 63));
   if (!pend_after || n_act > 1) return false;
-  int32_t* g_live = K.live + (size_t)env * KD(FW);
   int32_t* g_priv = K.priv + (size_t)env * KD(PW);
   const int t = wave::bcast(hdr, PH_TICK);
   long long opnum = ((long long)wave::bcast(hdr, PH_OPNUM_HI) << 32) | (uint32_t)wave::bcast(hdr, PH_OPNUM_LO);
@@ -1904,7 +1937,6 @@
 MRX_DEV bool fast_step_lane(const CimParams& K, const CimObs& O, int env, const int32_t* act, int n_act, int32_t* dec_out,
                             long long* met_out, uint8_t* done_out) {
   const int P = KD(P), V = KD(V);
-  int32_t* g_live = K.live + (size_t)env * KD(FW);
   int32_t* g_priv = K.priv + (size_t)env * KD(PW);
   const wave::v4i h0 = wave::ld16(g_priv), h1 = wave::ld16(g_priv + 4), h3 = wave::ld16(g_priv + 12);
   wave::v4i a4 = {0, 0, 0, 0};
@@ -1924,6 +1956,7 @@
   const uint64_t pend_after = pend & ~(1ull << (cur & 63));
   if (!pend_after || n_act > 1) return false;
   const int t = h0.x;
+  int32_t* g_live = live_frame(K, env, t);
   long long opnum = ((long long)h1.z << 32) | (uint32_t)h1.y;
   const long long acc_b = ((long long)h3.y << 32) | (uint32_t)h3.x, acc_s = ((long long)h3.w << 32) | (uint32_t)h3.z;
   int status = 0;
@@ -2032,12 +2065,12 @@
   io.done_out = B.done + env;
   return io;
 }
-struct StepEnd { bool store, ord_dirty, buf_dirty; };
+struct StepEnd { bool store, ord_dirty, buf_dirty, frame; int tick; };
 
 template <bool PG>
-MRX_DEV void state_load_async(const CimParams& K, Lds& L, int env) {
+MRX_DEV void state_load_async(const CimParams& K, Lds& L, int env, const int32_t* g_frame) {
   const uint32_t* g_mt = K.mt + (size_t)env * MTS_COUNT * MT_WORDS;
-  copy_in_async(L.frame, K.live + (size_t)env * KD(FW), KD(FW));
+  copy_in_async(L.frame, g_frame, KD(FW));
   copy_in_async(L.priv, K.priv + (size_t)env * KD(PW), KD(PWH));
 #ifndef MRX_LEAN
   copy_in_async(L.rfull, K.priv + (size_t)env * KD(PW) + KD(pv_rfull), KD(PW) - KD(pv_rfull));
@@ -2048,7 +2081,11 @@
 template <bool PG>
 MRX_DEV void state_store(const CimParams& K, Lds& L, int env, const StepEnd& e) {
   uint32_t* g_mt = K.mt + (size_t)env * MTS_COUNT * MT_WORDS;
-  copy_words(K.live + (size_t)env * KD(FW), L.frame, KD(FW));
+  if (e.frame) {
+    const int s = live_slot(K, e.tick);
+    copy_words(slot_frame(K, env, s), L.frame, KD(FW));
+    if (wave::lane() == 0) K.ring_fi[(size_t)env * KD(S) + s] = (e.tick - KD(start_tick)) / KD(resolution);
+  }
   copy_words(K.priv + (size_t)env * KD(PW), L.priv, KD(PWH));
 #ifndef MRX_LEAN
   copy_words(K.priv + (size_t)env * KD(PW) + KD(pv_rfull), L.rfull, KD(PW) - KD(pv_rfull));
@@ -2093,6 +2130,7 @@
   long long opnum;
   int status;
   int a0v, a0p, a0q, a0t, n_act, n_answered;
+  int plan_cell;
   TickPf pf;
 };
 struct StepOut {
@@ -2136,6 +2174,7 @@
   c.idx_buf = L.priv[PH_IDX_BUFFER];
   c.opnum = ((long long)L.priv[PH_OPNUM_HI] << 32) | (uint32_t)L.priv[PH_OPNUM_LO];
   c.status = 0;
+  c.plan_cell = PLAN_NONE;
   const uint64_t pend_after = c.fresh ? 0ull : consume_decisions(K, c.pend, L.priv[PH_CUR_VESSEL], c.n_answered);
   const int tn = c.fresh ? c.t : c.t + 1;
   if (!pend_after && tn < KD(T)) {
@@ -2181,10 +2220,10 @@
 #ifdef MRX_LEAN2
       const uint64_t hit = wave::ballot(wave::lane() < a_Lr && a_rp == p);
       const int cc = hit ? a_cb + wave::readlane(a_rc, __builtin_ctzll(hit)) : -1;
-      if (cc >= 0) { const int pl = U(L.frame[KD(f_plans) + cc]); L.frame[KD(f_plans) + cc] = pl + U(a_per); }
+      if (cc >= 0) { const int pl = U(L.frame[KD(f_plans) + cc]); L.frame[KD(f_plans) + cc] = pl + U(a_per); c.plan_cell = (c.plan_cell == PLAN_NONE || c.plan_cell == cc) ? cc : PLAN_MANY; }
 #else
       const int cc = plan_cell(L, v, p);
-      if (cc >= 0) { const int pl = U(L.frame[KD(f_plans) + cc]); L.frame[KD(f_plans) + cc] = pl + U(V_PERIOD(v)); }
+      if (cc >= 0) { const int pl = U(L.frame[KD(f_plans) + cc]); L.frame[KD(f_plans) + cc] = pl + U(V_PERIOD(v)); c.plan_cell = (c.plan_cell == PLAN_NONE || c.plan_cell == cc) ? cc : PLAN_MANY; }
 #endif
       else c.status |= 32;
     }
@@ -2197,9 +2236,10 @@
 MRX_DEV StepEnd body_run(const CimParams& K, const CimObs& O, int env, Lds& L, const StepIO& io, StepCtx& c, StepOut& out, Prof& prof, RingRegs& rr, Lean& Z) {
   const int lane = wave::lane();
   const int P = KD(P), V = KD(V);
-  StepEnd end = {true, false, false};
+  StepEnd end = {true, false, false, true, 0};
   int t = c.t;
   bool fresh = c.fresh, finished = false;
+  int snap = fresh ? SNAP_FULL : c.plan_cell;
   uint64_t pend = c.pend;
   int dec_v = -1;
   for (;;) {
@@ -2211,13 +2251,14 @@
       if ((t + 1) % KD(resolution) == 0) {
         if (lane < P) FP(PA_ACC_FULFILLMENT, lane) = FP(PA_ACC_BOOKING, lane) - FP(PA_ACC_SHORTAGE, lane);
         wave::sync();
-        take_snapshot(K, O, env, L, (t - KD(start_tick)) / KD(resolution));
+        take_snapshot(K, O, env, L, (t - KD(start_tick)) / KD(resolution), snap);
+        snap = SNAP_FULL;
         wave::sync();
         if (lane < P) { FP(PA_SHORTAGE, lane) = 0; FP(PA_BOOKING, lane) = 0; FP(PA_FULFILLMENT, lane) = 0; FP(PA_TRANSFER_COST, lane) = 0; }
         wave::sync();
       }
       if (t + 1 == KD(T)) {
-        if ((t + 1) % KD(resolution) != 0) take_snapshot(K, O, env, L, (t - KD(start_tick)) / KD(resolution));
+        if ((t + 1) % KD(resolution) != 0) take_snapshot(K, O, env, L, (t - KD(start_tick)) / KD(resolution), snap);
         finished = true;
         break;
       }
@@ -2225,6 +2266,7 @@
     }
     prof.mark(PF_POST_STEP);
     fresh = false;
+    snap = SNAP_FULL;
 #ifdef MRX_LEAN2
     pend = run_tick_lean(K, env, L, t, c.pf, c.idx_buf, c.status, prof, end.buf_dirty, rr, Z);
 #else
@@ -2242,12 +2284,10 @@
 
   if (MRX_UNALIGNED_FRAMES && !finished) {
     const int fi0 = (t - KD(start_tick)) / KD(resolution), lo = KD(start_tick) + fi0 * KD(resolution);
-    if (t > lo + (KD(resolution) - 1 - lo % KD(resolution))) {
-      wave::sync();
-      take_snapshot(K, O, env, L, fi0);
-      wave::sync();
-    }
-  }
+    if (t > lo + (KD(resolution) - 1 - lo % KD(resolution))) snapshot_hist(K, O, env, L, fi0);
+  }
+  end.frame = !finished;
+  end.tick = t;
   long long acc_b = 0, acc_s = 0;
   if (lane < P) { acc_b = FP(PA_ACC_BOOKING, lane); acc_s = FP(PA_ACC_SHORTAGE, lane); }
   acc_b = wave::reduce_add(acc_b);
@@ -2374,6 +2414,7 @@
     *io.done_out = (uint8_t)out.done;
     K.tick[env] = out.tick;
     K.hint[env] = (uint8_t)out.hint;
+    K.slot[env] = (uint8_t)live_slot(K, out.tick);
     if (out.status) wave::global_or(&K.status[env], out.status);
   }
 }
@@ -2384,7 +2425,7 @@
   StepOut out;
   c.a0v = a0v; c.a0p = a0p; c.a0q = a0q; c.a0t = a0t;
   c.n_act = io.n_act; c.n_answered = io.n_answered;
-  StepEnd end = {false, false, false};
+  StepEnd end = {false, false, false, false, 0};
   const long long agent_seed = O.agent_mode ? K.seed[env] : 0;
   if (body_open<PG>(K, env, L, c, out, Z)) {
     prof.mark(PF_LOAD);
@@ -2403,17 +2444,25 @@
        PATH_FULL = 2 };
 
 template <bool PG, bool OBS>
-MRX_DEV void step_env(const CimParams& K, const CimObs& O, int env, int32_t* lds, const StepIO& io, int path, int32_t* lds_ctab = nullptr) {
+MRX_DEV void step_env(const CimParams& K, const CimObs& O, int env, int32_t* lds, const StepIO& io, int path, int32_t* lds_ctab = nullptr,
+                      int slot = -1) {
   Lds L = make_lds(K, lds);
   Prof prof;
+  int hint = 0;
+  if (slot < 0) {
+    const int tick_v = K.tick[env], hint_v = (KD(decision_mode) == 0 && path == PATH_PROBE) ? (int)K.hint[env] : 0;
+    slot = live_slot(K, U(tick_v));
+    hint = hint_v;
+  } else if (KD(decision_mode) == 0 && path == PATH_PROBE) {
+    hint = K.hint[env];
+  }
+  int32_t* g_frame = slot_frame(K, env, U(slot));
   if (KD(decision_mode) == 0 && path != PATH_FULL) {
     FastRows rows;
-    fast_rows_request<OBS>(K, O, env, rows);
-    int hint = 0;
-    if (path == PATH_PROBE) hint = K.hint[env];
+    fast_rows_request<OBS>(K, O, env, g_frame, rows);
     int f0v = 0, f0p = 0, f0q = 0, f0t = 0;
     if (io.actions) { f0v = io.actions[0]; f0p = io.actions[1]; f0q = io.actions[2]; f0t = io.actions[3]; }
-    if (!U(hint) && fast_step<OBS>(K, O, env, rows, io.n_act > KD(max_actions) ? KD(max_actions) : io.n_act, f0v, f0p, f0q, f0t, io.dec_out,
+    if (!U(hint) && fast_step<OBS>(K, O, env, g_frame, rows, io.n_act > KD(max_actions) ? KD(max_actions) : io.n_act, f0v, f0p, f0q, f0t, io.dec_out,
                                    io.met_out, io.done_out)) {
 #ifdef MRX_PROFILE_FAST_PATH
       prof.mark(13); prof.mark(14, 1);
@@ -2423,7 +2472,7 @@
     }
     prof.mark(12);
   }
-  state_load_async<PG>(K, L, env);
+  state_load_async<PG>(K, L, env, g_frame);
   stage_tables(K, L, lds_ctab ? lds_ctab : lds + KD(l_ctab));
   RingRegs rr;
   ring_load(K, env, rr);
@@ -2453,8 +2502,9 @@
 MRX_DEV void step_loop(const CimParams& K, const CimObs& O, int32_t* lds, int w, int W, const StepBatch& B) {
   const int n_tick = U(wave::ld_uniform_v(K.sched + 0));
   for (int i = w; i < n_tick; i += W) {
-    const int env = U(wave::ld_uniform_v(K.order + i)) & (MRX_ORDER_TICK - 1);
-    step_env<PG, OBS>(K, O, env, lds, step_io(K, B, env), PATH_FULL);
+    int slot;
+    const int env = order_env(U(wave::ld_uniform_v(K.order + i)), slot);
+    step_env<PG, OBS>(K, O, env, lds, step_io(K, B, env), PATH_FULL, nullptr, slot);
     wave::sync();
   }
 }
@@ -2508,14 +2558,8 @@
 
 MRX_DEV const int32_t* frame_of(const CimParams& K, int env, int fi) {
   const int s = (fi < 0 ? 0 : fi) % KD(S);
-  const int32_t* hdr = K.priv + (size_t)env * KD(PW);
-  const int flags = hdr[PH_FLAGS], tick = hdr[PH_TICK], held = K.ring_fi[(size_t)env * KD(S) + s];
-  const bool paused = (flags & (FL_FRESH | FL_FINISHED)) == 0;
-  const int cur_fi = (tick - KD(start_tick)) / KD(resolution);
-  const int32_t* frame = nullptr;
-  if (held == fi) frame = K.ring + ((size_t)env * KD(S) + s) * KD(FW);
-  if (paused && s == cur_fi % KD(S)) frame = fi == cur_fi ? K.live + (size_t)env * KD(FW) : nullptr;
-  return fi < 0 ? nullptr : frame;
+  const int held = K.ring_fi[(size_t)env * KD(S) + s];
+  return (fi >= 0 && held == fi) ? slot_frame(K, env, s) : nullptr;
 }
 
 MRX_DEV double query_elem(const CimParams& K, int node_type, const int32_t* ticks, int nt, int ticks_per_env,
diff --git a/maro_amd/csrc/cim_dqn.h b/maro_amd/csrc/cim_dqn.h
--- a/maro_amd/csrc/cim_dqn.h
+++ b/maro_amd/csrc/cim_dqn.h
@@ -146,7 +146,7 @@
   const int lane = threadIdx.x & 63;
   const int dl = lane < 8 ? decisions[(size_t)env * 8 + lane] : 0;
   const int32_t* hdr = K.priv + (size_t)env * K.PW;
-  const int flags = hdr[PH_FLAGS], htick = hdr[PH_TICK];
+  const int htick = hdr[PH_TICK];
   int over = 0, pact = 0, pj = 0;
   long long head = 0;
   if (R.on) {
@@ -157,7 +157,7 @@
   }
   const int tick = __builtin_amdgcn_readlane(dl, 0), port = __builtin_amdgcn_readlane(dl, 1), vessel = __builtin_amdgcn_readlane(dl, 2);
   if (over || __builtin_amdgcn_readlane(dl, 7) != 1 || (unsigned)port >= (unsigned)K.P) return;
-  const int32_t* livef = K.live + (size_t)env * K.FW;
+  const int32_t* livef = cim::live_frame(K, env, htick);
   const int vv = (unsigned)vessel < (unsigned)K.V ? vessel : 0;
   const int kw = K.f_vessels + VA_LAST_LOC_IDX * K.V + vv;
   const int k_live = livef[kw];
@@ -168,11 +168,8 @@
   const int fi = max(0, tick - lane);
   const int slot = fi % K.S;
   const int held = lane < n_ticks ? K.ring_fi[(size_t)env * K.S + slot] : -1;
-  const bool paused = (flags & (FL_FRESH | FL_FINISHED)) == 0;
-  const int cur_fi = (htick - K.start_tick) / K.resolution;
   const int32_t* fptr = nullptr;
   if (held == fi) fptr = K.ring + ((size_t)env * K.S + slot) * K.FW;
-  if (paused && slot == cur_fi % K.S) fptr = fi == cur_fi ? livef : nullptr;
   if (lane >= n_ticks) fptr = nullptr;
   const int32_t* now = dq_shfl_ptr(fptr, 0);
   now = (const int32_t*)(((unsigned long long)(unsigned)__builtin_amdgcn_readfirstlane((int)((unsigned long long)now >> 32)) << 32) |
@@ -198,7 +195,7 @@
     const int nd = vessel_col ? vessel : __shfl(node, ni & 63);
     const bool ok = info >= 0 && f != nullptr && (unsigned)nd < (unsigned)(vessel_col ? K.V : K.P);
     const int w = vessel_col ? K.f_vessels + word * K.V + nd : word + nd;
-    raw[i] = *(ok ? f + w : K.live);
+    raw[i] = *(ok ? f + w : K.ring);
     okm |= (unsigned)ok << i;
   }
 #pragma unroll
@@ -248,7 +245,7 @@
     return;
   }
   if (sched_per > 0 && (int)blockIdx.x == n_bin) {
-    mrx_schedule_block((const uint8_t*)K.hint, nullptr, 0, n_envs, sched_per & 0xffffff, K.order, K.sched, sched_per >> 24);
+    mrx_schedule_block((const uint8_t*)K.hint, MRX_SCHED_SLOT(K), nullptr, 0, n_envs, sched_per & 0xffffff, K.order, K.sched, sched_per >> 24);
     return;
   }
   __shared__ int lcnt[64], base[64];
@@ -368,7 +365,7 @@
     const int32_t* d = decisions + (size_t)env * 8;
 #pragma unroll
     for (int i = 0; i < 5; i++) dq_d[i] = d[i];
-    const int32_t* live = K.live + (size_t)env * K.FW;
+    const int32_t* live = cim::live_frame(K, env, K.tick[env]);
     const int v = (unsigned)dq_d[2] < (unsigned)K.V ? dq_d[2] : 0;
     dq_space = live[K.f_vessels + VA_REMAINING_SPACE * K.V + v];
     dq_early = live[K.f_vessels + VA_EARLY_DISCHARGE * K.V + v];
diff --git a/maro_amd/csrc/cim_engine.hip b/maro_amd/csrc/cim_engine.hip
--- a/maro_amd/csrc/cim_engine.hip
+++ b/maro_amd/csrc/cim_engine.hip
@@ -21,11 +21,31 @@
   return nib(v.x) | (nib(v.y) << 4) | (nib(v.z) << 8) | (nib(v.w) << 12);
 }
 
-__device__ __forceinline__ void mrx_schedule_block(const uint8_t* __restrict__ hint, const uint8_t* __restrict__ mask, int mask_vec, int n, int per,
+__device__ __forceinline__ void mrx_emit8(int32_t* __restrict__ order, int& at, int p0, unsigned m, unsigned w0, unsigned w1, bool packed, int flags) {
+  for (; m; m &= m - 1) {
+    const int b = __builtin_ctz(m);
+    int e = (p0 + b) | flags;
+    if (packed) e |= MRX_ORDER_SLOT | (int)(__builtin_amdgcn_perm(w1, w0, 0x0c0c0c00u | (unsigned)b) << MRX_ORDER_SLOT_SHIFT);
+    order[at++] = e;
+  }
+}
+__device__ __forceinline__ void mrx_emit16(int32_t* __restrict__ order, int& ol, int& ot, int& of, int p0, unsigned l, unsigned t, unsigned f, uint4 sv, bool packed) {
+  mrx_emit8(order, ol, p0, l & 0xffu, sv.x, sv.y, packed, MRX_ORDER_TICK); mrx_emit8(order, ol, p0 + 8, l >> 8, sv.z, sv.w, packed, MRX_ORDER_TICK);
+  mrx_emit8(order, ot, p0, t & 0xffu, sv.x, sv.y, packed, MRX_ORDER_TICK); mrx_emit8(order, ot, p0 + 8, t >> 8, sv.z, sv.w, packed, MRX_ORDER_TICK);
+  mrx_emit8(order, of, p0, f & 0xffu, sv.x, sv.y, packed, 0); mrx_emit8(order, of, p0 + 8, f >> 8, sv.z, sv.w, packed, 0);
+}
+#ifdef MRX_ORDER_NO_SLOT
+#define MRX_SCHED_SLOT(K) ((const uint8_t*)nullptr)
+#else
+#define MRX_SCHED_SLOT(K) (((K).n_envs <= (1 << MRX_ORDER_SLOT_SHIFT) && (K).S <= 128) ? (const uint8_t*)(K).slot : (const uint8_t*)nullptr)
+#endif
+
+__device__ __forceinline__ void mrx_schedule_block(const uint8_t* __restrict__ hint, const uint8_t* __restrict__ slot, const uint8_t* __restrict__ mask, int mask_vec, int n, int per,
                                                    int32_t* __restrict__ order, int32_t* __restrict__ sched, int lpt) {
   __shared__ int s_l[16], s_t[16], s_f[16];
   const int tid = threadIdx.x, lane = tid & 63, wid = tid >> 6;
   const int lo = tid * per, hi = lo + per < n ? lo + per : n;
+  const bool packed = slot != nullptr;
   auto piece = [&](int p0, unsigned& l, unsigned& t, unsigned& f) {
     const unsigned valid = p0 + 16 <= n ? 0xffffu : ((1u << (n - p0)) - 1u);
     const uint4 hv = *(const uint4*)(hint + p0);
@@ -42,6 +62,7 @@
   int cl = 0, ct = 0, cf = 0;
   unsigned long long bl = 0, bt = 0, bf = 0;
   const bool small = per <= 64;
+  const uint4 zero4 = {0u, 0u, 0u, 0u};
   for (int p0 = lo; p0 < hi; p0 += 16) {
     unsigned l, t, f;
     piece(p0, l, t, f);
@@ -63,16 +84,18 @@
   }
   int ol = base_l + il - cl, ot = tot_l + base_t + it - ct, of = tot_l + tot_t + base_f + jf - cf;
   if (small) {
-    for (unsigned long long m = bl; m; m &= m - 1) order[ol++] = (lo + __builtin_ctzll(m)) | MRX_ORDER_TICK;
-    for (unsigned long long m = bt; m; m &= m - 1) order[ot++] = (lo + __builtin_ctzll(m)) | MRX_ORDER_TICK;
-    for (unsigned long long m = bf; m; m &= m - 1) order[of++] = lo + __builtin_ctzll(m);
+#pragma unroll 1
+    for (int p0 = lo; p0 < hi; p0 += 16) {
+      const uint4 sv = slot ? *(const uint4*)(slot + p0) : zero4;
+      mrx_emit16(order, ol, ot, of, p0, (unsigned)bl & 0xffffu, (unsigned)bt & 0xffffu, (unsigned)bf & 0xffffu, sv, packed);
+      bl >>= 16; bt >>= 16; bf >>= 16;
+    }
   } else {
     for (int p0 = lo; p0 < hi; p0 += 16) {
       unsigned l, t, f;
+      const uint4 sv = slot ? *(const uint4*)(slot + p0) : zero4;
       piece(p0, l, t, f);
-      for (; l; l &= l - 1) order[ol++] = (p0 + __builtin_ctz(l)) | MRX_ORDER_TICK;
-      for (; t; t &= t - 1) order[ot++] = (p0 + __builtin_ctz(t)) | MRX_ORDER_TICK;
-      for (; f; f &= f - 1) order[of++] = p0 + __builtin_ctz(f);
+      mrx_emit16(order, ol, ot, of, p0, l, t, f, sv, packed);
     }
   }
   const int n_full = tot_l + tot_t;
@@ -81,9 +104,9 @@
 }
 
 extern "C" __global__ void __launch_bounds__(1024)
-mrx_k_cim_schedule(const uint8_t* __restrict__ hint, const uint8_t* __restrict__ mask, int mask_vec, int n, int per, int32_t* __restrict__ order,
-                   int32_t* __restrict__ sched, int lpt) {
-  mrx_schedule_block(hint, mask, mask_vec, n, per, order, sched, lpt);
+mrx_k_cim_schedule(const uint8_t* __restrict__ hint, const uint8_t* __restrict__ slot, const uint8_t* __restrict__ mask, int mask_vec, int n, int per,
+                   int32_t* __restrict__ order, int32_t* __restrict__ sched, int lpt) {
+  mrx_schedule_block(hint, slot, mask, mask_vec, n, per, order, sched, lpt);
 }
 
 #ifndef MRX_DQN_TILE_DEFAULT
@@ -118,7 +141,7 @@
 mrx_k_cim_random_policy(CimParams K, const int32_t* __restrict__ decisions, long long step, int32_t* __restrict__ actions,
                         int32_t* __restrict__ n_actions, unsigned long long* __restrict__ counter, int sched_per) {
   if (sched_per > 0 && blockIdx.x == 0) {
-    mrx_schedule_block((const uint8_t*)K.hint, nullptr, 0, K.n_envs, sched_per & 0xffffff, K.order, K.sched, sched_per >> 24);
+    mrx_schedule_block((const uint8_t*)K.hint, MRX_SCHED_SLOT(K), nullptr, 0, K.n_envs, sched_per & 0xffffff, K.order, K.sched, sched_per >> 24);
     return;
   }
   const int env = (int)((blockIdx.x - (sched_per > 0 ? 1 : 0)) * blockDim.x + threadIdx.x);
@@ -512,7 +535,7 @@
   h->order_ready = false;
   if (mode >= 2 && !have_order) {
     const int per = ((K.n_envs + 1023) / 1024 + 15) / 16 * 16;
-    hipLaunchKernelGGL(mrx_k_cim_schedule, dim3(1), dim3(1024), 0, (hipStream_t)stream, (const uint8_t*)K.hint, d_env_mask,
+    hipLaunchKernelGGL(mrx_k_cim_schedule, dim3(1), dim3(1024), 0, (hipStream_t)stream, (const uint8_t*)K.hint, MRX_SCHED_SLOT(K), d_env_mask,
                        ((uintptr_t)d_env_mask & 15) ? 0 : 1, K.n_envs, per, K.order, K.sched, h->lpt);
   }
   const int sorted = mode == 5 ? 2 : mode >= 2 ? 1 : 0;
diff --git a/maro_amd/csrc/cim_layout.h b/maro_amd/csrc/cim_layout.h
--- a/maro_amd/csrc/cim_layout.h
+++ b/maro_amd/csrc/cim_layout.h
@@ -17,7 +17,7 @@
   std::vector<uint8_t> const_blob;
   int64_t const_off = 0;
   int64_t workspace_bytes = 0;
-  int64_t o_live, o_ring, o_ring_fi, o_priv, o_rec, o_status, o_tick, o_nstops, o_order_prop, o_mt, o_stops, o_seed, o_vperiod, o_orders, o_hint, o_order, o_sched;
+  int64_t o_ring, o_ring_fi, o_priv, o_rec, o_status, o_tick, o_nstops, o_order_prop, o_mt, o_stops, o_seed, o_vperiod, o_orders, o_hint, o_slot, o_order, o_sched;
   std::vector<std::pair<size_t, int64_t>> binds;
   int64_t ctab_rel = 0;
   int64_t shared_orders_rel = -1;
@@ -419,7 +419,6 @@
   Arena A;
   const int64_t N = c->n_envs;
   pl->const_off = A.take((int64_t)B.size());
-  pl->o_live = A.take(N * k.FW * 4);
   pl->o_ring = A.take(N * (int64_t)k.S * k.FW * 4);
   pl->o_ring_fi = A.take(N * k.S * 4);
   pl->o_priv = A.take(N * k.PW * 4);
@@ -433,6 +432,7 @@
   pl->o_seed = A.take(N * 8);
   pl->o_vperiod = A.take(N * V * 4);
   pl->o_hint = A.take(N + 64);
+  pl->o_slot = A.take(N + 64);
   pl->o_order = A.take(N * 4);
   pl->o_sched = A.take(64 + 64 * MRX_PIPE_MAX_WAVES);
   pl->shared_orders_rel = shared_orders_rel;
@@ -446,7 +446,8 @@
   Lo.max_stops = k.SMAX; Lo.horizon = k.H;
   Lo.frame_off_ports = k.f_ports; Lo.frame_off_vessels = k.f_vessels; Lo.frame_off_full_on_ports = k.f_fop;
   Lo.frame_off_full_on_vessels = k.f_fov; Lo.frame_off_vessel_plans = k.f_plans;
-  Lo.off_live = pl->o_live; Lo.off_ring = pl->o_ring; Lo.off_ring_fi = pl->o_ring_fi; Lo.off_status = pl->o_status;
+  Lo.off_live = pl->o_ring;
+  Lo.off_ring = pl->o_ring; Lo.off_ring_fi = pl->o_ring_fi; Lo.off_status = pl->o_status;
   Lo.off_tick = pl->o_tick; Lo.off_seed = pl->o_seed; Lo.off_stops = pl->o_stops; Lo.off_nstops = pl->o_nstops;
   Lo.off_order_prop = pl->o_order_prop; Lo.off_vessel_period = pl->o_vperiod;
   Lo.off_orders = shared_orders_rel >= 0 ? pl->const_off + shared_orders_rel : pl->o_orders; Lo.order_row_words = k.NTP; Lo.order_table_on = k.pregen; Lo.order_elem_bytes = k.pregen ? (k.order_half ? 2 : 4) : 0;
@@ -460,12 +461,12 @@
   uint8_t* cb = base + pl->const_off;
   for (auto& bd : pl->binds) *(const void**)((char*)&k + bd.first) = cb + bd.second;
   k.ctab = (const int32_t*)(cb + pl->ctab_rel);
-  k.live = (int32_t*)(base + pl->o_live); k.ring = (int32_t*)(base + pl->o_ring); k.ring_fi = (int32_t*)(base + pl->o_ring_fi);
+  k.ring = (int32_t*)(base + pl->o_ring); k.ring_fi = (int32_t*)(base + pl->o_ring_fi);
   k.priv = (int32_t*)(base + pl->o_priv); k.rec = (int32_t*)(base + pl->o_rec); k.status = (int32_t*)(base + pl->o_status);
   k.tick = (int32_t*)(base + pl->o_tick); k.nstops = (int32_t*)(base + pl->o_nstops);
   k.order_prop = (int32_t*)(base + pl->o_order_prop); k.mt = (uint32_t*)(base + pl->o_mt);
   k.stops = (uint32_t*)(base + pl->o_stops); k.seed = (int64_t*)(base + pl->o_seed);
   k.vperiod = (int32_t*)(base + pl->o_vperiod);
-  k.hint = base + pl->o_hint; k.order = (int32_t*)(base + pl->o_order); k.sched = (int32_t*)(base + pl->o_sched);
+  k.hint = base + pl->o_hint; k.slot = base + pl->o_slot; k.order = (int32_t*)(base + pl->o_order); k.sched = (int32_t*)(base + pl->o_sched);
   k.orders = !k.pregen ? nullptr : pl->shared_orders_rel >= 0 ? (int32_t*)(cb + pl->shared_orders_rel) : (int32_t*)(base + pl->o_orders);
 }
diff --git a/maro_amd/csrc/cim_params.h b/maro_amd/csrc/cim_params.h
--- a/maro_amd/csrc/cim_params.h
+++ b/maro_amd/csrc/cim_params.h
@@ -53,14 +53,19 @@
   const int32_t* ctab;
   const uint16_t *h_tgt_off, *h_route_port, *h_v_route_base, *h_v_route_len, *h_leg_off, *h_leg_time,
       *h_rec_off, *h_v_cbase, *h_route_cidx, *h_pair_src;
-  int32_t *live, *ring, *ring_fi, *priv, *rec, *status, *tick, *nstops, *order_prop, *vperiod, *orders;
+  int32_t *ring, *ring_fi, *priv, *rec, *status, *tick, *nstops, *order_prop, *vperiod, *orders;
   uint32_t *mt, *stops;
   int64_t* seed;
   uint8_t* hint;
+  uint8_t* slot;
   int32_t* order;
   int32_t* sched;
 };
 #define MRX_ORDER_TICK 0x40000000
+#define MRX_ORDER_SLOT 0x20000000
+#define MRX_ORDER_SLOT_SHIFT 22
+#define MRX_ORDER_ENV_PACKED ((1 << MRX_ORDER_SLOT_SHIFT) - 1)
+#define MRX_ORDER_ENV_PLAIN (MRX_ORDER_SLOT - 1)
 #define MRX_PIPE_MAX_WAVES 4096
 
 #define MRX_CIM_DIM_FIELDS(X) \
diff --git a/maro_amd/csrc/cim_sampler.h b/maro_amd/csrc/cim_sampler.h
--- a/maro_amd/csrc/cim_sampler.h
+++ b/maro_amd/csrc/cim_sampler.h
@@ -30,7 +30,7 @@
     else for (int k = lane; k < R.D; k += 64) ((float*)R.c_next_state)[row + k] = ((const float*)R.c_state)[row + k];
   }
   if (!over && tick_now >= 0 && tick_now < E.frames) {
-    const int32_t* live = K.live + (size_t)e * K.FW + K.f_ports;
+    const int32_t* live = cim::live_frame(K, e, tick_now) + K.f_ports;
     int32_t* row = E.hist + ((size_t)e * E.frames + (size_t)tick_now) * 2 * K.P;
     if (lane < K.P) { row[lane] = live[PA_FULFILLMENT * K.P + lane]; row[K.P + lane] = live[PA_SHORTAGE * K.P + lane]; }
   }
diff --git a/maro_amd/csrc/cim_step_kernels.h b/maro_amd/csrc/cim_step_kernels.h
--- a/maro_amd/csrc/cim_step_kernels.h
+++ b/maro_amd/csrc/cim_step_kernels.h
@@ -30,18 +30,18 @@
     const int w = MRX_WG_WAVES > 1 ? __builtin_amdgcn_readfirstlane((int)(threadIdx.x >> 6)) : 0;                        \
     const int slot = (int)blockIdx.x * MRX_WG_WAVES + w;                                                                \
     if (MRX_WG_WAVES > 1 && slot >= K.n_envs) return;                                                                   \
-    int env = slot, path = cim::PATH_PROBE;                                                                             \
+    int env = slot, path = cim::PATH_PROBE, fslot = -1;  \
     if (sorted) {                                                                                                       \
       if (sorted == 2 && slot >= K.sched[0]) return;   \
       const int e = K.order[slot];                                                                                      \
       if (e < 0) return;                                                                                                \
-      env = e & (MRX_ORDER_TICK - 1);                                                                                   \
+      env = cim::order_env(e, fslot);                                                                                   \
       path = (e & MRX_ORDER_TICK) ? cim::PATH_FULL : cim::PATH_FAST;                                                    \
     } else if (mask && !mask[env]) {                                                                                    \
       return;                                                                                                           \
     }                                                                                                                   \
     cim::step_env<PG, OBS>(K, O, env, lds + w * KD(l_ctab), cim::step_io(K, B, env), path,                               \
-                           lds + MRX_WG_WAVES * KD(l_ctab));                                                            \
+                           lds + MRX_WG_WAVES * KD(l_ctab), fslot);                                                     \
   }
 #ifdef MRX_SPECIALIZED
 #define MRX_WANT(PG, OBS) ((PG) == (MRXC_pregen != 0) && (OBS) == ((MRXC_obs_np | MRXC_obs_nv) != 0))
```

Measured after the change: 248.4 million (median of 6 runs). 61.1% higher.
